# ebu/libear

Hardware: AMD Instinct MI355X
Metric: Msamples/s (higher is better)
Workload: dtype f32 io / f16x2-split MFMA, f32 accumulate

## Files before the change

### include/earhip.h

```cpp
#ifndef EARHIP_H
#define EARHIP_H

#include <stddef.h>
#include <stdint.h>

#ifdef __cplusplus
extern "C" {
#endif

#define EARHIP_VERSION 100

#define EARHIP_OK 0
#define EARHIP_INVALID_ARGUMENT 1
#define EARHIP_INTERNAL_ERROR 2
#define EARHIP_DEVICE_ERROR 3
#define EARHIP_NOT_IMPLEMENTED 4
#define EARHIP_UNKNOWN_LAYOUT 5
#define EARHIP_ADM_ERROR 6

int earhip_version(void);
const char *earhip_last_error(void);
int earhip_device_count(int *count);

typedef struct earhip_ctx earhip_ctx;
// ... 212 lines not shown

int earhip_conversion_to_polar(size_t n, const double *x, const double *y, const double *z,
                               const double *width, const double *height, const double *depth,
                               double *azimuth, double *elevation, double *distance,
                               double *width_out, double *height_out, double *depth_out);
int earhip_conversion_to_cartesian(size_t n, const double *azimuth, const double *elevation,
                                   const double *distance, const double *width,
                                   const double *height, const double *depth, double *x, double *y,
                                   double *z, double *width_out, double *height_out,
                                   double *depth_out);
int earhip_conversion_to_polar_device(earhip_ctx *ctx, size_t n, const double *x, const double *y,
                                      const double *z, const double *width, const double *height,
                                      const double *depth, double *azimuth, double *elevation,
                                      double *distance, double *width_out, double *height_out,
                                      double *depth_out, int *status);
int earhip_conversion_to_cartesian_device(earhip_ctx *ctx, size_t n, const double *azimuth,
                                          const double *elevation, const double *distance,
                                          const double *width, const double *height,
                                          const double *depth, double *x, double *y, double *z,
                                          double *width_out, double *height_out, double *depth_out,
                                          int *status);

typedef struct earhip_render earhip_render;

typedef struct earhip_render_config {
  int n_objects;
  int n_out;
  int block_size;
  int n_buses;
  const float *decorrelators;
  int n_taps;
  int delay;
  int max_blocks;
} earhip_render_config;

int earhip_render_create(earhip_ctx *ctx, const earhip_render_config *cfg,
                         earhip_render **out);
int earhip_render_destroy(earhip_render *r);
int earhip_render_set_object_points(earhip_render *r, int object, int npoints,
                                    const int64_t *times, const float *direct,
                                    const float *diffuse);
int earhip_render_commit(earhip_render *r);
int earhip_render_scratch_regrows(const earhip_render *r, long *count);
int earhip_render_reset(earhip_render *r, int64_t sample_time);
int earhip_render_process_device(earhip_render *r, size_t nblocks,
                                 const float *in_dev, size_t in_stride,
                                 float *out_dev, size_t out_stride);
int earhip_render_process(earhip_render *r, size_t nblocks, const float *const *in,
                          float *const *out);
typedef enum {
  EARHIP_PCM_S16 = 1,
  EARHIP_PCM_S24 = 2,
  EARHIP_PCM_S32 = 3,
  EARHIP_PCM_F32 = 4
} earhip_pcm_format;
int earhip_render_process_frames(earhip_render *r, size_t nblocks, const void *frames,
                                 earhip_pcm_format fmt, int frame_channels, int first_channel,
                                 float *const *out, int out_interleaved);
int earhip_render_process_frames_device(earhip_render *r, size_t nblocks, const void *frames_dev,
                                        earhip_pcm_format fmt, int frame_channels, int first_channel,
                                        float *out_dev, size_t out_stride, int out_interleaved);
typedef struct earhip_pcm_out {
  earhip_pcm_format format;
  int dither;
  uint32_t seed;
} earhip_pcm_out;
int earhip_render_process_frames_pcm(earhip_render *r, size_t nblocks, const void *frames,
                                     earhip_pcm_format fmt, int frame_channels, int first_channel,
                                     void *out_frames, const earhip_pcm_out *out);
int earhip_render_process_frames_pcm_device(earhip_render *r, size_t nblocks, const void *frames_dev,
                                            earhip_pcm_format fmt, int frame_channels,
                                            int first_channel, void *out_dev, size_t out_frame_bytes,
                                            size_t out_first_byte, const earhip_pcm_out *out);
int earhip_render_output_levels(earhip_render *r, float *peak, uint64_t *clipped, int reset);
int earhip_render_enable_timing(earhip_render *r, int enable);
int earhip_render_get_timing(earhip_render *r, double out[6]);
int earhip_render_gain_kernel(const earhip_render *r, int *kind);
int earhip_render_hinge_standby(earhip_render *r, int *standby);
int earhip_render_hinge_robust(earhip_render *r, int *robust);
int earhip_render_wide_form(earhip_render *r, int *wide);
int earhip_render_last_plan(const earhip_render *r, int out[4]);
int earhip_render_last_decor_plan(const earhip_render *r, int out[4]);
int earhip_render_last_list_layout(const earhip_render *r, int *paired);
int earhip_render_last_tail_blocks(const earhip_render *r, int *blocks);
int earhip_render_last_host_chunks(const earhip_render *r, int *chunks);
int earhip_render_scratch_bytes(const earhip_render *r, size_t *bytes);

typedef struct earhip_comm earhip_comm;
int earhip_comm_unique_id(void *id128);
int earhip_comm_create(earhip_ctx *ctx, int rank, int world, const void *id128, earhip_comm **out);
int earhip_comm_destroy(earhip_comm *comm);
int earhip_comm_channel_range(int n_out, int rank, int world, int *padded_rows, int *lo, int *hi);
int earhip_render_exchange_device(earhip_comm *comm, int slot, const float *partial_dev,
                                  float *owned_dev, size_t rows_per_rank, size_t row_stride);
int earhip_comm_gather_device(earhip_comm *comm, int slot, const float *owned_dev, float *full_dev,
                              size_t rows_per_rank, size_t row_stride, int root);
int earhip_comm_wait(earhip_comm *comm, int slot);
int earhip_comm_last_exchange_ms(earhip_comm *comm, int slot, double *ms);
int earhip_comm_info(earhip_comm *comm, int info[4]);
int earhip_comm_link_probe(earhip_comm *comm, size_t bytes, int shift, int reps, double *GBps);

typedef struct earhip_loudness earhip_loudness;
int earhip_loudness_create(earhip_ctx *ctx, int n_channels, int sample_rate, const double *coeffs,
                           size_t max_steps, earhip_loudness **out);
typedef struct earhip_true_peak {
  int phases;
  int taps;
  const double *coeffs;
} earhip_true_peak;
int earhip_loudness_create_tp(earhip_ctx *ctx, int n_channels, int sample_rate, const double *coeffs,
                              size_t max_steps, const earhip_true_peak *tp, earhip_loudness **out);
int earhip_loudness_destroy(earhip_loudness *m);
int earhip_loudness_reset(earhip_loudness *m);
int earhip_loudness_process_device(earhip_loudness *m, size_t nsamples, const float *rows_dev, size_t stride);
int earhip_loudness_process(earhip_loudness *m, size_t nsamples, const float *const *rows);
int earhip_loudness_num_steps(earhip_loudness *m, size_t *steps);
int earhip_loudness_steps(earhip_loudness *m, size_t first, size_t n, double *energy);
int earhip_loudness_result(earhip_loudness *m, const double *weights, double *integrated,
                           double *max_momentary, double *max_short_term);
int earhip_loudness_peaks(earhip_loudness *m, float *true_peak, float *sample_peak);
int earhip_loudness_step_peaks(earhip_loudness *m, size_t first, size_t n, float *true_peak, float *sample_peak);
int earhip_loudness_result_range(earhip_loudness *m, const double *weights, double *lra, double *low,
                                 double *high);
int earhip_loudness_gate(size_t n_steps, int n_channels, const double *energy ,
                         const double *weights, double *integrated, double *max_momentary,
                         double *max_short_term);
int earhip_loudness_layout_weights(const char *layout, double *weights);
int earhip_loudness_range(size_t n_steps, int n_channels, const double *energy ,
                          const double *weights, double *lra, double *low, double *high);
int earhip_render_attach_loudness(earhip_render *r, earhip_loudness *m);

typedef struct earhip_firmix earhip_firmix;
typedef struct earhip_firmix_config {
  int n_in;
  int n_out;
  int block_size;
  int n_taps;
  const float *taps;
  int max_blocks;
} earhip_firmix_config;
int earhip_firmix_create(earhip_ctx *ctx, const earhip_firmix_config *config, earhip_firmix **out);
int earhip_firmix_destroy(earhip_firmix *fm);
int earhip_firmix_reset(earhip_firmix *fm);
int earhip_firmix_info(const earhip_firmix *fm, int info[5]);
int earhip_firmix_process_device(earhip_firmix *fm, size_t nblocks, const float *in_dev, size_t in_stride,
                                 float *out_dev, size_t out_stride);
int earhip_firmix_process(earhip_firmix *fm, size_t nblocks, const float *const *in, float *const *out);
int earhip_firmix_create_sets(earhip_ctx *ctx, const earhip_firmix_config *config, int n_sets, earhip_firmix **out);
int earhip_firmix_load_set(earhip_firmix *fm, int set, const float *taps);
int earhip_firmix_load_set_device(earhip_firmix *fm, int set, const float *taps_dev);
int earhip_firmix_select(earhip_firmix *fm, int set, int fade_blocks);
int earhip_firmix_state(const earhip_firmix *fm, int state[4]);
int earhip_firmix_set_info(const earhip_firmix *fm, int set, int info[2]);
int earhip_render_attach_firmix(earhip_render *r, earhip_firmix *fm, float *sink_dev, size_t sink_stride,
                                size_t sink_capacity);
int earhip_render_firmix_position(earhip_render *r, size_t *samples);

typedef struct earhip_limiter earhip_limiter;
typedef struct earhip_limiter_config {
  int n_channels;
  int sample_rate;
  float ceiling;
  int lookahead;
  int hold;
  int detect;
  const earhip_true_peak *tp;
// ... 173 lines not shown
```

### libear_amd/capi.py

```python
import ctypes as C
import os

import numpy as np

from .build import lib_path

f32p = C.POINTER(C.c_float)
i64p = C.POINTER(C.c_int64)
pp_f32 = C.POINTER(f32p)

OK, INVALID_ARGUMENT, INTERNAL_ERROR, DEVICE_ERROR, NOT_IMPLEMENTED, UNKNOWN_LAYOUT, ADM_ERROR = 0, 1, 2, 3, 4, 5, 6


class EarHipError(Exception):
    def __init__(self, code, msg):
        super().__init__(msg)
        self.code = code


class InvalidArgument(EarHipError, ValueError):
    """maps to ear::invalid_argument"""


class InternalError(EarHipError, RuntimeError):
# ... 1096 lines not shown
        x = np.ascontiguousarray(x)
        _, dtype, cols = pcm_format(out_fmt)
        out = np.empty((x.shape[0], self.N * cols), dtype)
        return self.process_frames_pcm_into(x, out, fmt, first_channel, out_fmt, dither, seed)

    def process_frames_pcm_into(self, x, out, fmt, first_channel=0, out_fmt="s16", dither=False, seed=0):
        code, nblocks, channels = self._frames_shape(x, fmt)
        ocode, dtype, cols = pcm_format(out_fmt)
        assert out.dtype == dtype and out.flags["C_CONTIGUOUS"] and out.shape == (nblocks * self.B, self.N * cols), out.shape
        spec = PcmOut(ocode, int(dither), int(seed) & 0xFFFFFFFF)
        check(load().earhip_render_process_frames_pcm(self.h, C.c_size_t(nblocks), C.c_void_p(x.ctypes.data), C.c_int(code),
                                                      C.c_int(channels), C.c_int(first_channel), C.c_void_p(out.ctypes.data),
                                                      C.byref(spec)))
        return out

    def process_frames_pcm_device(self, nblocks, frames_ptr, fmt, frame_channels, first_channel, out_ptr, out_frame_bytes,
                                  out_first_byte=0, out_fmt="s16", dither=False, seed=0):
        code = pcm_format(fmt)[0] if isinstance(fmt, str) else int(fmt)
        ocode = pcm_format(out_fmt)[0] if isinstance(out_fmt, str) else int(out_fmt)
        spec = PcmOut(ocode, int(dither), int(seed) & 0xFFFFFFFF)
        check(load().earhip_render_process_frames_pcm_device(self.h, C.c_size_t(nblocks), C.c_void_p(frames_ptr), C.c_int(code),
                                                             C.c_int(frame_channels), C.c_int(first_channel), C.c_void_p(out_ptr),
                                                             C.c_size_t(out_frame_bytes), C.c_size_t(out_first_byte),
                                                             C.byref(spec)))

    def output_levels(self, reset=False):
        peak, clipped = np.zeros(self.N, np.float32), np.zeros(self.N, np.uint64)
        check(load().earhip_render_output_levels(self.h, _ptr(peak), C.c_void_p(clipped.ctypes.data), int(bool(reset))))
        return peak, clipped

    def enable_timing(self, on=True):
        check(load().earhip_render_enable_timing(self.h, int(on)))

    def get_timing(self):
        out = (C.c_double * 6)()
        check(load().earhip_render_get_timing(self.h, out))
        return {"gain_mix_ms": out[0], "gain_mix_launches": out[1], "decor_ms": out[2],
                "decor_launches": out[3], "prep_ms": out[4], "prep_launches": out[5]}

    def gain_kernel(self):
        kind = C.c_int(-1)
        check(load().earhip_render_gain_kernel(self.h, C.byref(kind)))
        return kind.value

    def hinge_standby(self):
        flag = C.c_int(0)
        check(load().earhip_render_hinge_standby(self.h, C.byref(flag)))
        return bool(flag.value)

    def hinge_robust(self):
        flag = C.c_int(0)
        check(load().earhip_render_hinge_robust(self.h, C.byref(flag)))
        return bool(flag.value)

    def wide_form(self):
        flag = C.c_int(1)
        check(load().earhip_render_wide_form(self.h, C.byref(flag)))
        return None if flag.value < 0 else bool(flag.value)

    def scratch_bytes(self):
        v = C.c_size_t(0)
        check(load().earhip_render_scratch_bytes(self.h, C.byref(v)))
        return v.value

    def scratch_regrows(self):
        v = C.c_long(0)
        check(load().earhip_render_scratch_regrows(self.h, C.byref(v)))
        return v.value

    def last_tail_blocks(self):
        v = C.c_int(0)
        check(load().earhip_render_last_tail_blocks(self.h, C.byref(v)))
        return v.value

    def last_host_chunks(self):
        v = C.c_int(0)
        check(load().earhip_render_last_host_chunks(self.h, C.byref(v)))
        return v.value

    def last_list_layout(self):
        v = C.c_int(0)
        check(load().earhip_render_last_list_layout(self.h, C.byref(v)))
        return None if v.value < 0 else bool(v.value)

    def last_plan(self):
        out = (C.c_int * 4)()
        check(load().earhip_render_last_plan(self.h, out))
        return {"kernel": out[0], "tile": out[1], "ntiles": out[2], "gsplit": out[3]}

    def last_decor_plan(self):
        out = (C.c_int * 4)()
        check(load().earhip_render_last_decor_plan(self.h, out))
        return {"Bk": out[0], "NP": out[1], "form": out[2], "run": out[3]}

    def attach_loudness(self, meter):
        check(load().earhip_render_attach_loudness(self.h, meter.h if meter is not None else None))
        self._meter = meter

    def attach_fir_matrix(self, fm, sink_ptr=None, sink_stride=0, sink_capacity=0):
        check(load().earhip_render_attach_firmix(self.h, fm.h if fm is not None else None,
                                                 C.c_void_p(sink_ptr) if sink_ptr else None, C.c_size_t(sink_stride),
                                                 C.c_size_t(sink_capacity)))
        self._fir_matrix = fm

    def fir_matrix_position(self):
        v = C.c_size_t(0)
        check(load().earhip_render_firmix_position(self.h, C.byref(v)))
        return v.value

    def attach_limiter(self, lim, sink_ptr=None, sink_stride=0, sink_capacity=0):
        check(load().earhip_render_attach_limiter(self.h, lim.h if lim is not None else None,
                                                  C.c_void_p(sink_ptr) if sink_ptr else None, C.c_size_t(sink_stride),
                                                  C.c_size_t(sink_capacity)))
        self._limiter = lim

    def limiter_position(self):
        v = C.c_size_t(0)
        check(load().earhip_render_limiter_position(self.h, C.byref(v)))
        return v.value

    def close(self):
        if self.h:
            load().earhip_render_destroy(self.h)
            self.h = C.c_void_p()



def _f64(a):
    return np.ascontiguousarray(a, dtype=np.float64)


def loudness_gate(energy, weights):
    w = _f64(weights).reshape(-1)
    e = _f64(energy).reshape(-1, w.size)
    out = [C.c_double(0) for _ in range(3)]
    check(load().earhip_loudness_gate(C.c_size_t(e.shape[0]), C.c_int(w.size), C.c_void_p(e.ctypes.data), C.c_void_p(w.ctypes.data),
                                      *[C.byref(v) for v in out]))
    return tuple(v.value for v in out)


def loudness_range(energy, weights):
    w = _f64(weights).reshape(-1)
    e = _f64(energy).reshape(-1, w.size)
    out = [C.c_double(0) for _ in range(3)]
    check(load().earhip_loudness_range(C.c_size_t(e.shape[0]), C.c_int(w.size), C.c_void_p(e.ctypes.data), C.c_void_p(w.ctypes.data),
                                       *[C.byref(v) for v in out]))
    return tuple(v.value for v in out)


class _TruePeak(C.Structure):
    _fields_ = [("phases", C.c_int), ("taps", C.c_int), ("coeffs", C.c_void_p)]


def loudness_layout_weights(layout):
    n = C.c_int(0)
    check(load().earhip_layout_num_channels(layout.encode(), C.byref(n)))
    w = np.zeros(n.value, np.float64)
    check(load().earhip_loudness_layout_weights(layout.encode(), C.c_void_p(w.ctypes.data)))
    return w


class _BusStage:
    _stem = None

    def reset(self):
        check(getattr(load(), f"earhip_{self._stem}_reset")(self.h))
# ... 442 lines not shown
```

### libear_amd/csrc/api_core.hip

```cpp
#include <cctype>
#include <cerrno>
#include <cmath>
#include <cstdlib>
#include <string>
#include <memory>
#include <mutex>
#include <type_traits>

#include "common.h"
#include "curves.h"
#include "gain_kernels.h"
#include "gain_mfma.h"
#include "gain_h2.h"
#include "gain_h2_t1.h"
#include "gain_p2.h"
#include "gain_hg.h"
#include "gain_f32g.h"

namespace earhip {

static_assert(kSplitTile == 256, "MixLaunch::tile() and tiles_aligned(256, ...) assume the 4-wave tile");

static thread_local std::string g_last_error;
void set_last_error(const std::string &msg) { g_last_error = msg; }

template <int V>
using Int = std::integral_constant<int, V>;
template <int... Vs, typename F>
static void dispatch(int v, F &&f) {
  if (!((v == Vs ? (f(Int<Vs>{}), true) : false) || ...)) fail_internal("no gain kernel instantiation for this launch plan");
}
template <int... Vs, typename F>
static void for_each(F &&f) {
  (f(Int<Vs>{}), ...);
}

template <typename F>
static void for_each_hinge_build(F &&f) {
  for_each<1, 2, 4, 8>([&](auto T) { f(T, Int<4>{}), f(T, Int<8>{}); });
}

struct CallWords {
  unsigned *level_cur = nullptr, *level_next = nullptr;
  unsigned *wide_cur = nullptr, *wide_next = nullptr;
  unsigned *gate = nullptr;
  unsigned *slow_cur = nullptr, *slow_next = nullptr;
  unsigned *obj_level = nullptr;
  bool grew = false;
};

static int grow_call_words(earhip_ctx *ctx, int M, size_t ntiles, size_t tile_cap) {
  int made = 0;
  if (M > 0 && !ctx->level.p) ctx->level.alloc_zero(4, ctx->stream), made++;
  const bool grow_obj = ctx->obj_level_cap < M, grow_tiles = ctx->tile_slow_cap < ntiles;
  if (grow_obj || grow_tiles) EARHIP_HIP(hipStreamSynchronize(ctx->stream));
  if (grow_obj) {
    ctx->obj_level_cap = M + M / 2 + 64;
    ctx->obj_level.alloc_zero(2 * (size_t)ctx->obj_level_cap, ctx->stream);
    made++;
  }
  if (grow_tiles) {
    ctx->tile_slow_cap = std::max<size_t>(tile_cap, 1024);
    ctx->tile_slow.alloc_zero(2 * ctx->tile_slow_cap, ctx->stream);
    ctx->tile_slow_idx = 0;
    made++;
  }
  return made;
}

void reserve_call_words(earhip_ctx *ctx, int M, size_t max_samples) {
  const size_t ntiles = (max_samples + 255) / 256;
  grow_call_words(ctx, M, ntiles, ntiles + ntiles / 4);
}

static CallWords acquire_call_words(earhip_ctx *ctx, const MixLaunch &ml, int M, const float *in_dev, size_t in_stride, int nsamples) {
  CallWords w;
  if (!ml.split_operands()) return w;
  const bool probe = ctx->x_scale_auto && in_stride % 4 == 0 && ((uintptr_t)in_dev & 15) == 0;
  const size_t slow_tiles = ml.kind == GainKernel::Grid ? (size_t)ml.ntiles : 0;
  if (!probe && !slow_tiles) return w;
  if ((probe && (!ctx->level.p || ctx->obj_level_cap < M)) || ctx->tile_slow_cap < slow_tiles) {
    ctx->lazy_allocs += grow_call_words(ctx, probe ? M : 0, slow_tiles, 2 * slow_tiles);
    w.grew = true;
  }
  if (slow_tiles) {
    w.slow_cur = ctx->tile_slow.p + (size_t)ctx->tile_slow_idx * ctx->tile_slow_cap;
    w.slow_next = ctx->tile_slow.p + (size_t)(ctx->tile_slow_idx ^ 1) * ctx->tile_slow_cap;
    ctx->tile_slow_idx ^= 1;
  }
  if (!probe) return w;
  w.level_cur = ctx->level.p + ctx->level_idx;
  w.level_next = ctx->level.p + (ctx->level_idx ^ 1);
  if ((size_t)ml.ntiles * ml.gsplit >= 2 * (size_t)ctx->num_cus) w.wide_cur = ctx->level.p + 2 + ctx->level_idx;
  w.wide_next = ctx->level.p + 2 + (ctx->level_idx ^ 1);
  w.gate = ctx->level.p + 2 + ctx->level_idx;
  ctx->level_idx ^= 1;
  w.obj_level = ctx->obj_level.p;
  const int v = ctx->get(OPT_PROBE_RUNS);
  const int probe_runs = v >= 1 && v <= 64 && (v & (v - 1)) == 0 ? v : 16;
  hipLaunchKernelGGL(k_level_probe, dim3((M + kProbeObjects - 1) / kProbeObjects), dim3(64 * kProbeObjects), 0, ctx->stream, in_dev,
                     in_stride, nsamples, M, w.level_cur, ctx->obj_level.p, ctx->obj_level_cap, probe_runs);
  return w;
}

struct MixCall {
  earhip_ctx *ctx;
  const CurveSet &cs;
  const MixLaunch &ml;
  const ColumnPlan &cp;
  PointStore ps;
  int M, nsamples;
  int64_t t_call;
  const float *in_dev;
  size_t in_stride;
  SegDesc *scratch;
  ScratchLayout lay;
  SlotLists sl;
  PieceLists pl;
  HingeLists hl;
  CallWords w;
  bool hg_robust = false, standby = false;
  GainMixParams P;
  hipStream_t stream() const { return ctx->stream; }
  int64_t t_end() const { return t_call + nsamples; }
  unsigned *gate_word(bool robust) const { return hg_robust == robust ? w.gate : nullptr; }
  unsigned *standby_gate() const { return ml.kind == GainKernel::Hinge ? w.gate : nullptr; }
  int piece_tile() const { return 64 * ml.pw; }
  int piece_tiles() const { return lay.piece_tiles; }
  float x_scale() const { return std::ldexp(1.0f, ctx->x_scale_log2); }
  dim3 tile_grid(int x) const { return dim3(x, ml.gsplit, cp.mnz * cp.mgroups); }
};


static void prep_hinge_lists(const MixCall &c) {
  earhip_ctx *ctx = c.ctx;
  const MixLaunch &ml = c.ml;
  const int M = c.M, nw = ml.tile() / 64;
  if (M > kMaxHingeCached || (nw != 4 && nw != 8)) fail_internal("hinge lists: object count or tile out of range");
  if (!c.ps.kink_row0) fail_internal("hinge kernel: the curve set has no kink rows");
  if (!hinge_addressable(M, c.in_stride, c.nsamples, (size_t)c.ps.kink_row0 + c.ps.rows, c.ps.row)) fail_internal("hinge kernel: buffers beyond its 32-bit offsets");
  if (c.w.gate)
    hipLaunchKernelGGL(k_hinge_gate, dim3((M + 255) / 256), dim3(256), 0, c.stream(), c.w.obj_level, ctx->obj_level_cap, M, c.w.level_cur, c.w.gate,
                       c.w.wide_cur != nullptr, c.hg_robust);
  int tpw = 1;
  const size_t cached_max = std::min((size_t)kMaxHingeCached, ctx->hinge_build_lds / sizeof(HingeCached));
  if ((size_t)M > cached_max) fail_internal("hinge lists: more objects than the builder's LDS holds on this device");
  while (tpw < 8 && ml.ntiles / (2 * tpw) >= ctx->num_cus && (size_t)M * (2 * tpw) <= cached_max) tpw *= 2;
  if (ctx->has(OPT_HBUILD_TPW)) {
    const int v = ctx->get(OPT_HBUILD_TPW);
    if ((v == 1 || v == 2 || v == 4 || v == 8) && (size_t)M * v <= cached_max) tpw = v;
  }
  HingeCached *stage = nullptr;
  if (ctx->get(OPT_BUILD_2K, 0) != 0) {
    stage = c.lay.hinge_staging(c.scratch);
    const dim3 cgrid((ml.ntiles + 63) / 64, (M + kClassifyObjects - 1) / kClassifyObjects);
    dispatch<4, 8>(nw, [&](auto NW) {
      hipLaunchKernelGGL((k_hinge_classify<decltype(NW)::value>), cgrid, dim3(64 * kClassifyObjects), 0, c.stream(), c.ps, M, ml.ntiles, c.t_call,
                         c.t_end(), stage, c.w.obj_level, c.w.level_cur, c.gate_word(false), c.gate_word(true));
    });
    if (!ctx->has(OPT_HBUILD_TPW)) {
      tpw = 1;
      while (tpw < 8 && ml.ntiles / (2 * tpw) >= 2 * ctx->num_cus) tpw *= 2;
    }
  }
  const dim3 bgrid((ml.ntiles + tpw - 1) / tpw);
  const size_t lds = stage ? 0 : sizeof(HingeCached) * (size_t)M * tpw;
  for_each_hinge_build([&](auto T, auto NW) {
    if (tpw == T && nw == NW)
      hipLaunchKernelGGL((k_hinge_build<decltype(T)::value, decltype(NW)::value>), bgrid, dim3(kHingeBuildThreads), lds, c.stream(), c.ps, M, ml.ntiles,
                         c.t_call, c.t_end(), c.hl, c.w.obj_level, c.w.level_cur, c.gate_word(false), c.gate_word(true), (const HingeCached *)stage);
  });
}

static void prep_piece_lists(const MixCall &c) {
  earhip_ctx *ctx = c.ctx;
  const MixLaunch &ml = c.ml;
  const int M = c.M, ptile = c.piece_tile(), pnt = c.piece_tiles();
  if (M > kMaxPieceObjects || ptile > kPieceMaxTile) fail_internal("piece lists: object index or tile out of range");
  int tpw = 1;
  while (tpw < 8 && pnt / (2 * tpw) >= ctx->num_cus) tpw *= 2;
  if (ctx->has(OPT_BUILD_TPW)) {
    const int v = ctx->get(OPT_BUILD_TPW);
    if (v == 1 || v == 2 || v == 4 || v == 8) tpw = v;
  }
  const PieceLists &pl = c.pl;
  PairRec *stage = nullptr;
  if (ctx->has(OPT_BUILD_2K) ? ctx->get(OPT_BUILD_2K) != 0 : ml.paired) {
    stage = c.lay.piece_staging(c.scratch);
    hipLaunchKernelGGL(k_piece_classify, dim3((pnt + 63) / 64, (M + kClassifyObjects - 1) / kClassifyObjects), dim3(64 * kClassifyObjects), 0,
                       c.stream(), c.ps, M, pnt, ptile, c.t_call, c.t_end(), pl.paired, stage, c.w.obj_level, c.w.level_cur, c.standby_gate());
  }
  dispatch<1, 2, 4, 8>(tpw, [&](auto T) {
    hipLaunchKernelGGL(k_piece_build<decltype(T)::value>, dim3((pnt + tpw - 1) / tpw), dim3(kBuildThreads), 0, c.stream(), c.ps, M, pnt, ptile, c.t_call,
                       c.t_end(), pl, c.w.obj_level, c.w.level_cur, c.standby_gate(), ctx->obj_level_cap, c.w.wide_cur, stage);
  });
}

static void prep_descriptors(const MixCall &c) {
  const MixLaunch &ml = c.ml;
  const unsigned objs = (unsigned)(c.M + 15) / 16;
  QuietMark qm;
  if (c.w.obj_level) {
// ... 54 lines not shown
  const int per_cu = ml.tile() == 512 ? 1 : (cp.nct == 1 ? 3 : 2);
  int wgs = std::max(8, (ctx->num_cus * per_cu / std::max(1, ml.gsplit * cp.mnz * cp.mgroups)) & ~7);
  if (ctx->has(OPT_H2_WGS)) wgs = std::max(1, ctx->get(OPT_H2_WGS));
  wgs = std::max(wgs, ((ml.ntiles + 63) / 64 + 7) & ~7);
  if (!h2_persistent(cp.nct, ml.tile() == 512 ? 8 : 4)) wgs = ml.ntiles;
  GainMixParams P = c.P;
  P.tile_runs = ctx->has(OPT_H2_RUNS) ? (ctx->get(OPT_H2_RUNS) != 0) : 0;
  const dim3 grid = c.tile_grid(std::min(ml.ntiles, wgs));
  const float xs = c.x_scale();
  const float *gs = c.cs.column_scales();
  const bool two_launches = ctx->get(OPT_H2_PAIR, 0) != 0;
  auto h2 = [&](auto NCT, auto NW, auto WIDE) {
    hipLaunchKernelGGL((k_gain_mix_h2<decltype(NCT)::value, decltype(NW)::value, decltype(WIDE)::value>), grid, dim3(64 * decltype(NW)::value), 0,
                       c.stream(), P, c.ps.zero_row, xs, gs, w.level_cur, w.level_next, w.slow_cur, w.slow_next, w.wide_cur, w.wide_next);
  };
  auto h2_t1 = [&](auto NCT, auto WIDE) {
    hipLaunchKernelGGL((k_gain_mix_h2_t1<decltype(NCT)::value, 4, decltype(WIDE)::value>), grid, dim3(256), 0, c.stream(), P, c.ps.zero_row, xs, gs,
                       w.level_cur, w.level_next, w.slow_cur, w.slow_next, w.wide_cur, w.wide_next);
  };
  dispatch<1, 2, 3>(cp.nct, [&](auto NCT) {
    if (ml.tile() == 512) {
      if (w.wide_cur && !two_launches) return h2(NCT, Int<8>{}, Int<2>{});
      if (w.wide_cur) h2(NCT, Int<8>{}, Int<0>{});
      h2(NCT, Int<8>{}, Int<1>{});
    } else if (NCT == 1) {
      if (w.wide_cur) h2(Int<1>{}, Int<4>{}, Int<0>{});
      h2(Int<1>{}, Int<4>{}, Int<1>{});
    } else {
      if (w.wide_cur) h2_t1(NCT, std::false_type{});
      h2_t1(NCT, std::true_type{});
    }
  });
}

static void launch_pieces(const MixCall &c) {
  earhip_ctx *ctx = c.ctx;
  const ColumnPlan &cp = c.cp;
  const MixLaunch &ml = c.ml;
  const CallWords &w = c.w;
  const int pnt = c.piece_tiles();
  int wgs = std::max(8, (ctx->num_cus * (ml.pw == 4 ? 2 : 1) / std::max(1, ml.gsplit * cp.mnz * cp.mgroups)) & ~7);
  if (ctx->has(OPT_P2_WGS)) wgs = ctx->get(OPT_P2_WGS) > 0 ? ctx->get(OPT_P2_WGS) : pnt;
  if (!p2_persistent(cp.nct, ml.pw, ml.paired)) wgs = pnt;
  const dim3 grid = c.tile_grid(std::min(pnt, wgs));
  const float xs = c.x_scale();
  const float *gs = c.cs.column_scales();
  dispatch<0, 1>(ml.paired ? 1 : 0, [&](auto PAIRED) {
    dispatch<1, 2, 3>(cp.nct, [&](auto NCT) {
      dispatch<4, 8>(ml.pw == 4 ? 4 : 8, [&](auto NW) {
        constexpr int nw = decltype(NW)::value;
        hipLaunchKernelGGL((k_gain_mix_p2<decltype(NCT)::value, nw, decltype(PAIRED)::value != 0>), grid, dim3(64 * nw), 0, c.stream(), c.P, c.pl, xs, gs,
                           w.level_cur, w.level_next, w.wide_cur, w.wide_next, c.standby_gate(), pnt);
      });
    });
  });
}

static void launch_hinge(const MixCall &c) {
  const CallWords &w = c.w;
  const float xs = c.x_scale();
  const float *gs = c.cs.column_scales();
  dispatch<1, 2, 3>(c.cp.nct, [&](auto NCT) {
    dispatch<4, 8>(c.ml.tile() == 256 ? 4 : 8, [&](auto NW) {
      constexpr int nw = decltype(NW)::value;
      hipLaunchKernelGGL((k_gain_mix_hg<decltype(NCT)::value, nw>), c.tile_grid(c.ml.ntiles), dim3(64 * nw), 0, c.stream(), c.P, c.hl, xs, gs, w.level_cur,
                         w.level_next, w.wide_cur, w.wide_next, c.gate_word(false), c.gate_word(true));
    });
  });
}

static GainMixParams mix_params(const MixCall &c, float *out_dev, size_t out_stride, size_t part_stride, unsigned *record) {
  const float *in_dev = c.in_dev;
  const size_t in_stride = c.in_stride;
  const bool valu = c.ml.kind == GainKernel::Valu;
  GainMixParams P;
  P.mode_word = c.w.gate;
  P.record = c.w.gate ? record : nullptr;
  P.sl = c.sl;
  P.in = in_dev;
  P.in_stride = in_stride;
  P.out = out_dev;
  P.out_stride = out_stride;
  P.part_stride = part_stride;
  P.desc = c.scratch;
  P.ps = c.ps;
  P.t_call = c.t_call;
  P.nsamples = c.nsamples;
  P.ntiles = c.ml.ntiles;
  P.M = c.M;
  P.ncols = c.cs.ncols();
  P.ngroups = valu ? c.cp.ngroups : c.cp.mgroups;
  P.wsplit = c.ml.wsplit;
  P.tiles_per_wg = valu ? 1 : c.ml.tpw;
  P.vec_ok = in_stride % 4 == 0 && out_stride % 4 == 0 && part_stride % 4 == 0 && ((uintptr_t)in_dev & 15) == 0 && ((uintptr_t)out_dev & 15) == 0;
  return P;
}

MixResult launch_gain_mix(earhip_ctx *ctx, const CurveSet &cs, const MixLaunch &ml, bool strict, int64_t t_call, int nsamples,
                          const float *in_dev, size_t in_stride, float *out_dev, size_t out_stride, size_t part_stride, SegDesc *desc,
                          unsigned *record, hipEvent_t *ev) {
  const GainKernel kind = ml.kind;
  MixCall c{ctx, cs, ml, cs.plan(), cs.device(), cs.M(), nsamples, t_call, in_dev, in_stride, desc, scratch_layout(cs, ml, cs.M(), nsamples)};
  if (kind == GainKernel::Slots) c.sl = c.lay.slot_lists(desc);
  if (kind == GainKernel::Pieces || kind == GainKernel::Hinge) c.pl = c.lay.piece_lists(desc, ml.paired);
  if (kind == GainKernel::Hinge) c.hl = c.lay.hinge_lists(desc);
  if (kind == GainKernel::Slots && c.M > kMaxSlotObjects) fail_internal("slot lists address objects with 16 bits");
  if (ev) EARHIP_HIP(hipEventRecord(ev[0], ctx->stream));
  c.w = acquire_call_words(ctx, ml, c.M, in_dev, in_stride, nsamples);
  c.hg_robust = kind == GainKernel::Hinge && ctx->get(OPT_HG_ROBUST, 1) != 0;
  c.standby = kind == GainKernel::Hinge && c.w.gate && !c.hg_robust;
  switch (kind) {
    case GainKernel::Hinge:
      prep_hinge_lists(c);
      if (c.standby) prep_piece_lists(c);
      break;
    case GainKernel::Pieces: prep_piece_lists(c); break;
    case GainKernel::Slots: {
      const bool own_search = (size_t)c.ps.npoints <= (size_t)8 * c.M;
      if (!own_search) prep_descriptors(c);
      prep_slot_lists(c, own_search);
      break;
    }
    default: prep_descriptors(c); break;
  }
  if (ev) EARHIP_HIP(hipEventRecord(ev[1], ctx->stream));
  c.P = mix_params(c, out_dev, out_stride, part_stride, record);
  if (ev) EARHIP_HIP(hipEventRecord(ev[2], ctx->stream));
  switch (kind) {
    case GainKernel::Valu: launch_valu(c, strict); break;
    case GainKernel::Slots: launch_slots(c); break;
    case GainKernel::F32Grid: launch_f32grid(c); break;
    case GainKernel::Grid: launch_grid(c); break;
    case GainKernel::Pieces: launch_pieces(c); break;
    case GainKernel::Hinge:
      launch_hinge(c);
      if (c.standby) launch_pieces(c);
      break;
  }
  if (ev) EARHIP_HIP(hipEventRecord(ev[3], ctx->stream));
  EARHIP_HIP(hipGetLastError());
  MixResult res;
  res.gated = kind == GainKernel::Hinge && c.w.gate;
  res.device_form = c.w.wide_cur != nullptr;
  res.hinge_robust = res.gated && c.hg_robust;
  res.grew = c.w.grew;
  return res;
}

size_t hinge_build_allow_lds(const hipDeviceProp_t &prop) {
  const size_t want = 128 * 1024, dflt = 64 * 1024;
  const size_t device_max = std::max((size_t)prop.sharedMemPerBlock, (size_t)prop.maxSharedMemoryPerMultiProcessor);
  size_t ask = std::min(want, device_max > 4096 ? device_max - 4096 : dflt);
  if (ask <= dflt) return dflt;
  bool ok = true;
  for_each_hinge_build([&](auto T, auto NW) {
    ok = ok && hipFuncSetAttribute(reinterpret_cast<const void *>(&k_hinge_build<decltype(T)::value, decltype(NW)::value>),
                                   hipFuncAttributeMaxDynamicSharedMemorySize, (int)ask) == hipSuccess;
  });
  if (!ok) (void)hipGetLastError();
  return ok ? ask : dflt;
}

struct GainStage {
  earhip_ctx *ctx;
  int n_in, n_out;
  CurveSet curves;
  DevBuf<SegDesc> desc;
  DevBuf<float> parts;
  std::vector<float> rows;
  bool force_ramp;
  GainStage(earhip_ctx *c, int ni, int no, bool ramp = false)
      : ctx(c), n_in(ni), n_out(no), curves(ni, no, 1, ramp), force_ramp(ramp) {}

  void run_device(int64_t t_call, int nsamples, const float *in_dev, size_t in_stride,
                  float *out_dev, size_t out_stride) {
    curves.commit(ctx);
    const bool strict = ctx->strict || n_in == 1 || force_ramp;
    const MixLaunch ml = plan_mix(ctx, curves.plan(), n_in, nsamples, strict, 32, curves.stats(t_call, in_stride, (size_t)nsamples, false));
    if (ml.kind == GainKernel::Hinge) curves.ensure_kinks(ctx);
    desc.reserve(scratch_units(curves, ml, n_in));
    const size_t row_stride = ((size_t)nsamples + 3) & ~(size_t)3;
    if (ml.gsplit > 1) parts.reserve(row_stride * n_out * ml.gsplit);
    launch_gain_mix_summed(ctx, curves, ml, strict, t_call, nsamples, in_dev, in_stride, out_dev, out_stride, parts.p, row_stride, desc.p,
                           nullptr, nullptr);
  }

  void run_host(int64_t t_call, const float *const *in, float *const *out, int64_t r0,
                int64_t r1) {
    const int n = (int)(r1 - r0);
    if (n <= 0) return;
    const size_t stride = ((size_t)n + 3) & ~(size_t)3;
    ctx->pin_in.reserve(stride * n_in);
    ctx->pin_out.reserve(stride * n_out);
    ctx->dev_in.reserve(stride * n_in);
    ctx->dev_out.reserve(stride * n_out);
    for (int c = 0; c < n_in; c++)
      std::memcpy(ctx->pin_in.p + c * stride, in[c] + r0, sizeof(float) * n);
    EARHIP_HIP(hipMemcpyAsync(ctx->dev_in.p, ctx->pin_in.p, sizeof(float) * stride * n_in,
                              hipMemcpyHostToDevice, ctx->stream));
    run_device(t_call, n, ctx->dev_in.p, stride, ctx->dev_out.p, stride);
    EARHIP_HIP(hipMemcpyAsync(ctx->pin_out.p, ctx->dev_out.p, sizeof(float) * stride * n_out,
                              hipMemcpyDeviceToHost, ctx->stream));
    EARHIP_HIP(hipStreamSynchronize(ctx->stream));
    for (int c = 0; c < n_out; c++)
      std::memcpy(out[c] + r0, ctx->pin_out.p + c * stride, sizeof(float) * n);
  }
};

}

using namespace earhip;

static const char *const kOptNames[OPT_COUNT] = {
    "SPL", "MFMA", "XSCALE", "WAVES", "TPW", "NRT", "H2_TILE", "H2_WGS", "H2_RUNS", "P2_TILE", "P2_PAIRS", "P2_WGS", "HINGE", "HG_TILE", "HBUILD_TPW",
    "BUILD_TPW", "K2_WG", "K2_OWN_BLOCK", "RUN", "GSPLIT", "PROBE_RUNS", "BLOCK_GROUPS", "DEBUG_TIMING", "TAILCUT", "HOST_CHUNK_MB", "HOST_THREADS", "HG_ROBUST", "BUILD_2K", "HOST_BIND", "HOST_NT", "HOST_FIRST", "H2_PAIR"};

static int parse_option_value(const std::string &key, const char *text) {
  char *end = nullptr;
  errno = 0;
  const long v = std::strtol(text, &end, 10);
  while (end && *end && std::isspace((unsigned char)*end)) end++;
  if (end == text || (end && *end) || errno == ERANGE || v < -(1L << 30) || v > (1L << 30))
    fail_invalid("option '" + key + "': '" + std::string(text) + "' is not an integer");
  return (int)v;
}

void earhip_ctx::apply_options() {
  spl = 4, use_mfma = 3, x_scale_log2 = 14, x_scale_auto = true, max_waves = 4, tiles_per_wg = 4, tiles_per_wg_forced = false, nrt = 8;
  if (has(OPT_SPL) && (get(OPT_SPL) == 2 || get(OPT_SPL) == 4)) spl = get(OPT_SPL);
  if (has(OPT_MFMA)) use_mfma = get(OPT_MFMA);
  if (has(OPT_XSCALE) && get(OPT_XSCALE) >= -64 && get(OPT_XSCALE) <= 64)
    x_scale_log2 = get(OPT_XSCALE), x_scale_auto = false;
  if (has(OPT_WAVES) && get(OPT_WAVES) >= 1 && get(OPT_WAVES) <= 8) max_waves = get(OPT_WAVES);
  if (has(OPT_TPW) && get(OPT_TPW) >= 1 && get(OPT_TPW) <= 8) tiles_per_wg = get(OPT_TPW), tiles_per_wg_forced = true;
  if (has(OPT_NRT) && (get(OPT_NRT) == 4 || get(OPT_NRT) == 8)) nrt = get(OPT_NRT);
}

struct earhip_gain_interp {
  std::unique_ptr<GainStage> stage;
};

struct PolicyCache {
  std::vector<std::unique_ptr<GainStage>> stages;
  GainStage *get(earhip_ctx *ctx, int n_in, int n_out, bool ramp) {
    for (auto &s : stages)
      if (s->n_in == n_in && s->n_out == n_out && s->force_ramp == ramp) return s.get();
    stages.emplace_back(new GainStage(ctx, n_in, n_out, ramp));
    return stages.back().get();
  }
};
static std::vector<std::pair<earhip_ctx *, std::unique_ptr<PolicyCache>>> g_policy;
static std::mutex g_policy_mutex;
static PolicyCache *policy_cache(earhip_ctx *ctx) {
  std::lock_guard<std::mutex> lock(g_policy_mutex);
  for (auto &p : g_policy)
    if (p.first == ctx) return p.second.get();
  g_policy.emplace_back(ctx, std::unique_ptr<PolicyCache>(new PolicyCache));
  return g_policy.back().second.get();
}

static __global__ void k_clock_probe(unsigned long long *out) {
  out[0] = clock64();
  out[1] = wall_clock64();
}

static __global__ void __launch_bounds__(256) k_read_linear(const f32x4 *in, float *out, size_t n4) {
  f32x4 acc = {0.0f, 0.0f, 0.0f, 0.0f};
  size_t i = (size_t)blockIdx.x * 256 + threadIdx.x;
  const size_t step = (size_t)gridDim.x * 256;
  for (; i + 3 * step < n4; i += 4 * step) {
    const f32x4 a = __builtin_nontemporal_load(in + i), b = __builtin_nontemporal_load(in + i + step);
    const f32x4 c = __builtin_nontemporal_load(in + i + 2 * step), d = __builtin_nontemporal_load(in + i + 3 * step);
    acc += (a + b) + (c + d);
  }
  for (; i < n4; i += step) acc += __builtin_nontemporal_load(in + i);
  if (acc[0] + acc[1] + acc[2] + acc[3] == 123.456f) out[0] = 1.0f;
}
static __global__ void __launch_bounds__(256) k_read_rows(const float *in, float *out, int rows, size_t stride) {
  constexpr int DEPTH = 4;
  const int lane = threadIdx.x & 63, w = threadIdx.x >> 6, li = lane & 15, kg = lane >> 4;
  const float *base = in + (size_t)blockIdx.x * 256 + w * 64 + li * 4;
  auto row = [&](int r) { return base + (size_t)min(r, rows - 1) * stride; };
  f32x4 acc = {0.0f, 0.0f, 0.0f, 0.0f};
  f32x4 ring[DEPTH][8];
#pragma unroll
  for (int d = 0; d < DEPTH; d++)
#pragma unroll
    for (int q = 0; q < 8; q++)
      ring[d][q] = __builtin_nontemporal_load((const f32x4 *)row(d * 32 + kg * 8 + q));
  for (int r0 = 0; r0 < rows; r0 += 32 * DEPTH) {
#pragma unroll
    for (int d = 0; d < DEPTH; d++) {
#pragma unroll
      for (int q = 0; q < 8; q++) acc += ring[d][q];
      const int rn = r0 + 32 * DEPTH + d * 32;
      if (rn < rows)
#pragma unroll
        for (int q = 0; q < 8; q++)
          ring[d][q] = __builtin_nontemporal_load((const f32x4 *)row(rn + kg * 8 + q));
    }
  }
  if (acc[0] + acc[1] + acc[2] + acc[3] == 123.456f) out[0] = 1.0f;
}

extern "C" {

int earhip_debug_read_bandwidth(earhip_ctx *ctx, const float *in_dev, size_t rows, size_t stride,
                                size_t nsamples, int reps, double ms[2]) {
  return guarded([&] {
    require(ctx != nullptr && in_dev != nullptr && ms != nullptr, "NULL argument");
    require(rows >= 1 && rows < ((size_t)1 << 24) && reps >= 1 && reps <= 1000, "rows / reps out of range");
    require(stride % 256 == 0 && nsamples % 256 == 0 && nsamples >= 256 && nsamples <= stride &&
                ((uintptr_t)in_dev & 15) == 0,
            "buffer must be 16-byte aligned with stride and nsamples multiples of 256");
    ctx->use();
    if (!ctx->level.p) ctx->level.alloc_zero(4, ctx->stream);
    float *sink = reinterpret_cast<float *>(ctx->level.p);
    hipEvent_t e[4];
    for (auto &x : e) EARHIP_HIP(hipEventCreate(&x));
    const size_t n4 = rows * stride / 4;
    const unsigned lin_blocks = (unsigned)std::min<size_t>((n4 + 255) / 256, (size_t)ctx->num_cus * 32);
    auto linear = [&] {
      hipLaunchKernelGGL(k_read_linear, dim3(lin_blocks), dim3(256), 0, ctx->stream,
                         reinterpret_cast<const f32x4 *>(in_dev), sink, n4);
    };
    auto pattern = [&] {
      hipLaunchKernelGGL(k_read_rows, dim3((unsigned)(nsamples / 256)), dim3(256), 0, ctx->stream, in_dev, sink,
                         (int)rows, stride);
    };
    linear();
    EARHIP_HIP(hipEventRecord(e[0], ctx->stream));
    for (int i = 0; i < reps; i++) linear();
    EARHIP_HIP(hipEventRecord(e[1], ctx->stream));
    pattern();
    EARHIP_HIP(hipEventRecord(e[2], ctx->stream));
    for (int i = 0; i < reps; i++) pattern();
    EARHIP_HIP(hipEventRecord(e[3], ctx->stream));
    EARHIP_HIP(hipGetLastError());
    EARHIP_HIP(hipEventSynchronize(e[3]));
    float t = 0.0f;
    EARHIP_HIP(hipEventElapsedTime(&t, e[0], e[1]));
    ms[0] = (double)t / reps;
    EARHIP_HIP(hipEventElapsedTime(&t, e[2], e[3]));
    ms[1] = (double)t / reps;
    for (auto &x : e) (void)hipEventDestroy(x);
  });
}

int earhip_debug_copy_bandwidth(earhip_ctx *ctx, void *host, size_t bytes, int reps, double ms[2]) {
  return guarded([&] {
    require(ctx != nullptr && host != nullptr && ms != nullptr, "NULL argument");
    require(bytes >= 4 && reps >= 1 && reps <= 1000, "bytes / reps out of range");
    ctx->use();
    DevBuf<char> dev;
    dev.alloc(bytes);
    hipEvent_t e[2];
    for (auto &x : e) EARHIP_HIP(hipEventCreate(&x));
    for (int dir = 0; dir < 2; dir++) {
      auto copy = [&] {
        if (dir == 0) EARHIP_HIP(hipMemcpyAsync(dev.p, host, bytes, hipMemcpyHostToDevice, ctx->stream));
        else EARHIP_HIP(hipMemcpyAsync(host, dev.p, bytes, hipMemcpyDeviceToHost, ctx->stream));
      };
      copy();
      EARHIP_HIP(hipEventRecord(e[0], ctx->stream));
      for (int i = 0; i < reps; i++) copy();
      EARHIP_HIP(hipEventRecord(e[1], ctx->stream));
      EARHIP_HIP(hipEventSynchronize(e[1]));
      float t = 0.0f;
      EARHIP_HIP(hipEventElapsedTime(&t, e[0], e[1]));
      ms[dir] = (double)t / reps;
    }
    for (auto &x : e) (void)hipEventDestroy(x);
    EARHIP_HIP(hipStreamSynchronize(ctx->stream));
  });
}

int earhip_debug_hg_prof(earhip_ctx *ctx, unsigned long long *out128) {
  return guarded([&] {
    require(ctx != nullptr && out128 != nullptr, "NULL argument");
#ifdef EARHIP_HG_PROF
    ctx->use();
    EARHIP_HIP(hipStreamSynchronize(ctx->stream));
    EARHIP_HIP(hipMemcpyFromSymbol(out128, HIP_SYMBOL(g_hg_prof), sizeof(unsigned long long) * 128));
#else
    fail_invalid("this build has no hinge-kernel phase sums (-DEARHIP_HG_PROF)");
#endif
  });
}

int earhip_debug_build_prof(earhip_ctx *ctx, unsigned long long *out64) {
  return guarded([&] {
    require(ctx != nullptr && out64 != nullptr, "NULL argument");
#ifdef EARHIP_BUILD_PROF
    ctx->use();
    EARHIP_HIP(hipStreamSynchronize(ctx->stream));
    EARHIP_HIP(hipMemcpyFromSymbol(out64, HIP_SYMBOL(g_build_prof), sizeof(unsigned long long) * 64));
#else
    fail_invalid("this build has no list-builder phase stamps (-DEARHIP_BUILD_PROF)");
#endif
// ... 305 lines not shown
```

### libear_amd/csrc/api_render.hip

```cpp
#include <cmath>
#include <cstdlib>
#include <chrono>
#include <memory>
#include <vector>

#include "bus_stage.h"
#include "curves.h"
#include "decor_stage.h"
#include "host_pipeline.h"
#include "pcm_frames.h"

using namespace earhip;

struct CallReport {
  int kind = -1;
  int plan[3] = {0, 0, 0};
  int paired = -1;
  size_t scratch_bytes = 0;
  bool gated = false;
  bool device_form = false;
  bool hg_robust = false;
  int tail_blocks = 0;
};

struct earhip_render {
  earhip_ctx *ctx = nullptr;
  int M = 0, N = 0, B = 0, K = 1, T = 0;
  std::unique_ptr<CurveSet> curves;
  int64_t t = 0;
  CallReport report;
  long scratch_regrows = 0;
  DevBuf<unsigned> rec;

  DevBuf<SegDesc> desc;
  DevBuf<float> bus;
  int max_gsplit = 1;
  DecorStage decor;
  DevBuf<float> d_in, d_out;
  PinBuf<float> p_in, p_out;
  std::unique_ptr<GatherPool> gather;
  StreamPipe pipe;
  int last_host_chunks = 0;
  PinBuf<unsigned char> p_bytes;
  DevBuf<unsigned char> d_bytes;
  DevBuf<float> d_ilv, d_rows, d_rows_out;
  DevBuf<unsigned char> d_pcm;
  PinBuf<unsigned char> p_pcm;
  PcmLevels levels;
  bool timing = false;
  bool last_timed = false;
  int timing_every = 1;
  long timing_calls = 0;
  hipEvent_t ev[6] = {nullptr, nullptr, nullptr, nullptr, nullptr, nullptr};
  struct Pending { hipEvent_t e[6]; bool has_k2; bool continues; };
  std::vector<Pending> pending;
  std::vector<hipEvent_t> pool;
  double acc_ms[3] = {0, 0, 0};
  double acc_n[3] = {0, 0, 0};

  ~earhip_render() {
    for (auto &p : pending)
      for (auto e : p.e)
        if (e) (void)hipEventDestroy(e);
    for (auto e : pool) (void)hipEventDestroy(e);
  }

  unsigned mode_word() {
    ctx->use();
    unsigned word = 0;
    EARHIP_HIP(hipMemcpyAsync(&word, rec.p, sizeof(word), hipMemcpyDeviceToHost, ctx->stream));
    EARHIP_HIP(hipStreamSynchronize(ctx->stream));
    if (!(word & kModeRecorded)) fail_internal("no gain kernel recorded the call's mode word");
    return word;
  }

  hipEvent_t get_event() {
    if (!pool.empty()) {
      hipEvent_t e = pool.back();
      pool.pop_back();
      return e;
    }
    hipEvent_t e;
    EARHIP_HIP(hipEventCreate(&e));
    return e;
  }

  void drain_timing() {
    EARHIP_HIP(hipStreamSynchronize(ctx->stream));
    for (auto &p : pending) {
      float ms = 0;
      const double one = p.continues ? 0.0 : 1.0;
      EARHIP_HIP(hipEventElapsedTime(&ms, p.e[0], p.e[1]));
      acc_ms[2] += ms; acc_n[2] += one;
      EARHIP_HIP(hipEventElapsedTime(&ms, p.e[2], p.e[3]));
      acc_ms[0] += ms; acc_n[0] += one;
      if (p.has_k2) {
        EARHIP_HIP(hipEventElapsedTime(&ms, p.e[4], p.e[5]));
        acc_ms[1] += ms; acc_n[1] += one;
      }
      for (auto e : p.e)
        if (e) pool.push_back(e);
    }
    pending.clear();
  }

  size_t direct_stride(const float *const *ch, int count, size_t n) const {
    if (ctx->host_ranges.empty() || count < 1) return 0;
    const uintptr_t a0 = (uintptr_t)ch[0];
    const uintptr_t step = count > 1 ? (uintptr_t)ch[1] - a0 : sizeof(float) * n;
    if ((a0 & 15) != 0 || step % 16 != 0 || step < sizeof(float) * n || step > ((uintptr_t)1 << 40)) return 0;
    for (int c = 1; c < count; c++)
      if ((uintptr_t)ch[c] - (uintptr_t)ch[c - 1] != step) return 0;
    return ctx->host_reachable(ch[0], step * (count - 1) + sizeof(float) * n) ? (size_t)(step / sizeof(float)) : 0;
  }

  size_t frames_to_device_rows(size_t nblocks, const void *frames_dev, int fmt, int frame_channels, int first_channel, bool with_out) {
    ctx->use();
    const size_t S = (size_t)pcm_sample_bytes(fmt), n = nblocks * (size_t)B, cap = (size_t)T * B;
    if (d_rows.n < cap * M || (with_out && d_rows_out.n < cap * N)) {
      EARHIP_HIP(hipStreamSynchronize(ctx->stream));
      d_rows.reserve(cap * M);
      if (with_out) d_rows_out.reserve(cap * N);
    }
    launch_pcm_to_rows(fmt, frames_dev, (size_t)frame_channels * S, (size_t)first_channel * S, M, n, d_rows.p, n, ctx->stream);
    return n;
  }
  void reserve_pcm_out(size_t bytes, bool pinned) {
    levels.reserve(N, ctx->stream);
    d_pcm.reserve(bytes);
    if (pinned) p_pcm.reserve(bytes);
  }

  HostChunkPlan host_plan(size_t nblocks, bool direct) const {
    return plan_host_chunks(nblocks, B, M, direct, ctx->has(OPT_HOST_CHUNK_MB), ctx->get(OPT_HOST_CHUNK_MB), ctx->get(OPT_HOST_FIRST, 0));
  }
  hipError_t chunk_rows_d2h(float *out0, size_t out_st, size_t at, size_t len) {
    const float *dout = d_out.p + (size_t)N * at;
    if (out_st)
      return hipMemcpy2DAsync(out0 + at, sizeof(float) * out_st, dout, sizeof(float) * len, sizeof(float) * len, N, hipMemcpyDeviceToHost, pipe.out);
    return hipMemcpyAsync(p_out.p + (size_t)N * at, dout, sizeof(float) * len * N, hipMemcpyDeviceToHost, pipe.out);
  }
  void chunk_rows_scatter(float *const *out, size_t at, size_t len) const {
    for (int ch = 0; ch < N; ch++) std::memcpy(out[ch] + at, p_out.p + (size_t)N * at + (size_t)ch * len, sizeof(float) * len);
  }
  void process_short_call(size_t nblocks, float *out0, size_t out_st) {
    const size_t n = nblocks * (size_t)B;
    const bool direct_out = decor.NP <= 1;
    process_device(nblocks, d_in.p, n, out_st ? out0 : direct_out ? p_out.p : d_out.p, out_st ? out_st : n);
    if (!out_st && !direct_out) EARHIP_HIP(hipMemcpyAsync(p_out.p, d_out.p, sizeof(float) * n * N, hipMemcpyDeviceToHost, ctx->stream));
  }
  GatherPool &staging_threads() {
    if (!gather) {
      gather.reset(new GatherPool);
      const int want = ctx->get(OPT_HOST_THREADS, 0);
      gather->start(want >= 1 && want <= 64 ? want : default_staging_threads());
    }
    return *gather;
  }

  MixLaunch plan_call(size_t nblocks, size_t in_stride) {
    const int nsamples = (int)(nblocks * (size_t)B);
    MixLaunch ml = plan_mix(ctx, curves->plan(), M, nsamples, ctx->strict, max_gsplit, curves->stats(t, in_stride, (size_t)nsamples, true));
    const size_t bus_stride = ((size_t)nsamples + 3) & ~(size_t)3;
    while (ml.gsplit > 1 && bus_stride * K * N * ml.gsplit > bus.n) ml.gsplit /= 2;
    return ml;
  }

  size_t last_in_stride = 0;
  void reserve_for_curves() {
    size_t need = 0;
    bool hinge = false;
    const size_t lens[3] = {(size_t)T, (size_t)std::max(1, T / 2), (size_t)1};
    for (size_t nb : lens) {
      const MixLaunch ml = plan_call(nb, last_in_stride ? last_in_stride : nb * (size_t)B);
      need = std::max(need, scratch_units(*curves, ml, M));
      hinge = hinge || ml.kind == GainKernel::Hinge;
    }
    if (hinge) curves->ensure_kinks(ctx);
    if (need > desc.n) {
      EARHIP_HIP(hipStreamSynchronize(ctx->stream));
      desc.reserve(need + need / 4);
    }
  }

  int resident_workgroups(const MixLaunch &ml) const {
    if (!ml.split_operands()) return 0;
    return ctx->num_cus * (ml.tile() >= 512 ? 1 : 2);
  }

  struct BusTap {
    BusStage *stage = nullptr;
    float *sink = nullptr;
    size_t stride = 0, cap = 0, pos = 0;
  };
  enum { TAP_METER, TAP_MATRIX, TAP_LIMITER, TAP_COUNT };
  BusTap taps[TAP_COUNT];
  bool tapped() const {
    for (const BusTap &t : taps)
      if (t.stage) return true;
    return false;
  }
  void attach(int which, BusStage *stage, const char *rows_words, bool writes, float *sink_dev, size_t sink_stride,
              size_t sink_capacity) {
    if (stage) {
      const std::string the = std::string("the ") + stage->noun;
      if (stage->ctx != ctx) fail_invalid(the + " must belong to the renderer's context");
      require(stage->n_in == N, rows_words);
      if (stage->block != 1 && stage->block != B) fail_invalid(the + " must have the renderer's block size");
      if (writes) {
        require(sink_dev != nullptr, "sink_dev must not be NULL");
        require(sink_stride >= sink_capacity, "sink_stride must be >= sink_capacity");
      }
    }
    taps[which] = stage && writes ? BusTap{stage, sink_dev, sink_stride, sink_capacity, 0} : BusTap{stage};
  }
  void check_taps(size_t nblocks) const {
    const size_t n = nblocks * (size_t)B;
    for (const BusTap &t : taps) {
      if (!t.stage) continue;
      t.stage->check_room(n / (size_t)t.stage->block);
      if (t.sink && t.pos + n > t.cap)
        fail_invalid(std::string("the call would pass the ") + t.stage->noun + "'s sink_capacity (nothing was rendered)");
    }
  }
  void feed_taps(size_t nblocks, const float *out_dev, size_t out_stride) {
    const size_t n = nblocks * (size_t)B;
    for (BusTap &t : taps) {
      if (!t.stage) continue;
      t.stage->feed(n / (size_t)t.stage->block, out_dev, out_stride, t.sink ? t.sink + t.pos : nullptr, t.stride);
      if (t.sink) t.pos += n;
    }
  }
  void process_device(size_t nblocks, const float *in_dev, size_t in_stride, float *out_dev, size_t out_stride) {
    if (!tapped()) return render_spans(nblocks, in_dev, in_stride, out_dev, out_stride);
    check_taps(nblocks);
    render_spans(nblocks, in_dev, in_stride, out_dev, out_stride);
    feed_taps(nblocks, out_dev, out_stride);
  }
  void render_spans(size_t nblocks, const float *in_dev, size_t in_stride, float *out_dev, size_t out_stride) {
    MixLaunch whole;
    bool have_plan = false;
    if (!ctx->strict && ctx->get(OPT_TAILCUT, 1) != 0 && nblocks >= 2) {
      last_in_stride = in_stride;
      if (curves->dirty()) {
        curves->commit(ctx);
        reserve_for_curves();
      }
      const MixLaunch ml = whole = plan_call(nblocks, in_stride);
      have_plan = true;
      const int W = resident_workgroups(ml);
      if (W > 0 && ml.gsplit == 1 && ml.ntiles > W) {
        const size_t tile = (size_t)ml.tile();
        const size_t full = (size_t)ml.ntiles / (size_t)W, rest = (size_t)ml.ntiles % (size_t)W;
        const size_t main_samples = full * (size_t)W * tile;
        const size_t eighths = (size_t)std::min(std::max(ctx->get(OPT_TAILCUT, 2), 0), 7);
        if (rest > 0 && rest <= (size_t)W * eighths / 8 && main_samples % (size_t)B == 0) {
          const size_t main_blocks = main_samples / (size_t)B;
          process_span(main_blocks, in_dev, in_stride, out_dev, out_stride, false);
          const CallReport main = report;
          process_span(nblocks - main_blocks, in_dev + main_samples, in_stride, out_dev + main_samples, out_stride, true);
          report = main;
          report.tail_blocks = (int)(nblocks - main_blocks);
          return;
        }
      }
    }
    report.tail_blocks = 0;
    process_span(nblocks, in_dev, in_stride, out_dev, out_stride, false, have_plan ? &whole : nullptr);
  }

  void process_span(size_t nblocks, const float *in_dev, size_t in_stride, float *out_dev,
                    size_t out_stride, bool continues, const MixLaunch *planned = nullptr) {
    const int nsamples = (int)(nblocks * (size_t)B);
    last_in_stride = in_stride;
    if (curves->dirty()) {
      curves->commit(ctx);
      reserve_for_curves();
    }
    const bool strict = ctx->strict;
    MixLaunch ml = planned ? *planned : plan_call(nblocks, in_stride);
    if (ml.kind == GainKernel::Hinge) curves->ensure_kinks(ctx);

    report.kind = (int)ml.kind;
    {
      const size_t need = scratch_units(*curves, ml, M);
      if (need > desc.n) {
        EARHIP_HIP(hipStreamSynchronize(ctx->stream));
        desc.reserve(need + need / 2);
        scratch_regrows++;
      }
      report.scratch_bytes = need * 16;
    }
    const size_t bus_stride = ((size_t)nsamples + 3) & ~(size_t)3;
    const size_t part_stride = bus_stride * K * N;
    if (part_stride * ml.gsplit > bus.n) fail_internal("bus buffer too small for this launch plan");
    report.paired = (ml.kind == GainKernel::Pieces || ml.kind == GainKernel::Hinge) ? (ml.paired ? 1 : 0) : -1;
    report.plan[0] = ml.tile();
    report.plan[1] = ml.ntiles;
    report.plan[2] = ml.gsplit;
    Pending pd;
    hipEvent_t *evp = nullptr;
    const bool timed = timing && (continues ? last_timed : (timing_calls++ % timing_every) == 0);
    last_timed = timed;
    if (timed) {
      for (int i = 0; i < 6; i++) pd.e[i] = get_event();
      pd.has_k2 = K == 2;
      pd.continues = continues;
      evp = pd.e;
    }
    unsigned *const record = rec.p + (continues ? 1 : 0);
    MixResult mix;
    if (K == 1) {
      mix = launch_gain_mix_summed(ctx, *curves, ml, strict, t, nsamples, in_dev, in_stride, out_dev, out_stride, bus.p, bus_stride, desc.p,
                                   record, evp);
    } else {
      mix = launch_gain_mix(ctx, *curves, ml, strict, t, nsamples, in_dev, in_stride, bus.p, bus_stride, part_stride, desc.p, record, evp);
      decor.run(ctx, nblocks, nsamples, bus.p, bus_stride, part_stride, ml.gsplit, out_dev, out_stride, evp);
    }
    if (timed) pending.push_back(pd);
    report.gated = mix.gated, report.device_form = mix.device_form, report.hg_robust = mix.hinge_robust;
    if (mix.grew) scratch_regrows++;
    t += nsamples;
  }
};

extern "C" {

int earhip_render_create(earhip_ctx *ctx, const earhip_render_config *cfg, earhip_render **out) {
  return guarded([&] {
    require(ctx != nullptr && cfg != nullptr && out != nullptr, "NULL argument");
    require(cfg->n_objects >= 1 && cfg->n_out >= 1, "n_objects and n_out must be >= 1");
    require(cfg->n_buses == 1 || cfg->n_buses == 2, "n_buses must be 1 or 2");
    FftShape shape;
    require(cfg->block_size >= 16 && cfg->block_size <= 4096 && fft_make_shape(2 * cfg->block_size, &shape),
            "block_size must be in [16, 4096]");
    require(cfg->max_blocks >= 1, "max_blocks must be >= 1");
    require((int64_t)cfg->max_blocks * cfg->block_size < ((int64_t)1 << 30),
            "max_blocks * block_size too large");
    require(cfg->delay >= 0, "delay must be >= 0");
    if (cfg->n_buses == 2) {
      require(cfg->decorrelators != nullptr && cfg->n_taps >= 1,
              "n_buses == 2 needs decorrelator filters");
      require((cfg->n_taps + cfg->block_size - 1) / cfg->block_size <= 64,
              "decorrelator filters of more than 64 blocks are not supported by the fused render "
              "(use BlockConvolver)");
    } else {
      require(cfg->delay == 0, "delay needs n_buses == 2");
    }
    ctx->use();
    std::unique_ptr<earhip_render> r(new earhip_render);
    r->ctx = ctx;
    r->M = cfg->n_objects;
    r->N = cfg->n_out;
    r->B = cfg->block_size;
    r->K = cfg->n_buses;
    r->T = cfg->max_blocks;
    r->curves.reset(new CurveSet(r->M, r->K * r->N, r->K, false));
    const size_t max_samples = (size_t)r->T * r->B;
    reserve_call_words(ctx, r->M, max_samples);
    r->rec.alloc_zero(2, ctx->stream);
    const size_t min_tile = (size_t)std::min(16 * ctx->nrt, std::min(64 * ctx->spl, 256));
    const size_t max_tiles = (max_samples + min_tile - 1) / min_tile;
    r->desc.alloc((size_t)r->M * ((max_samples + 255) / 256) + 1);
    (void)max_tiles;
    r->max_gsplit = 16;
    if (ctx->has(OPT_GSPLIT)) {
      const int v = ctx->get(OPT_GSPLIT);
      if (v >= 1 && v <= 32) r->max_gsplit = v;
    }
    r->bus.alloc_zero((size_t)r->K * r->N * bus_samples_bound(ctx, max_samples, r->max_gsplit), ctx->stream);
    if (r->K == 2) r->decor.create(ctx, *cfg, r->B);
    EARHIP_HIP(hipStreamSynchronize(ctx->stream));
    *out = r.release();
  });
}

int earhip_render_destroy(earhip_render *r) {
  return guarded([&] {
    if (!r) return;
    (void)hipSetDevice(r->ctx->device);
    (void)hipStreamSynchronize(r->ctx->stream);
    delete r;
  });
}

int earhip_render_set_object_points(earhip_render *r, int object, int npoints,
                                    const int64_t *times, const float *direct,
                                    const float *diffuse) {
  return guarded([&] {
    require(r != nullptr, "render must not be NULL");
    require(npoints >= 1, "interp_points must not be empty");
    require(times != nullptr && direct != nullptr, "times/direct must not be NULL");
    require(r->K == 1 || diffuse != nullptr, "diffuse gains must not be NULL when n_buses == 2");
    const int N = r->N, cols = r->K * N;
    std::vector<float> rows((size_t)npoints * cols);
    for (int k = 0; k < npoints; k++) {
      std::memcpy(&rows[(size_t)k * cols], direct + (size_t)k * N, sizeof(float) * N);
      if (r->K == 2)
        std::memcpy(&rows[(size_t)k * cols + N], diffuse + (size_t)k * N, sizeof(float) * N);
    }
    r->curves->set_object(object, npoints, times, rows.data());
  });
}
// ... 326 lines not shown
    r->ctx->use();
    if (r->timing) r->drain_timing();
    r->timing = enable != 0;
    r->timing_every = enable > 1 ? enable : 1;
    r->timing_calls = 0;
    for (int i = 0; i < 3; i++) r->acc_ms[i] = r->acc_n[i] = 0;
  });
}

int earhip_render_get_timing(earhip_render *r, double out[6]) {
  return guarded([&] {
    require(r != nullptr && out != nullptr, "NULL argument");
    r->ctx->use();
    r->drain_timing();
    out[0] = r->acc_ms[0]; out[1] = r->acc_n[0];
    out[2] = r->acc_ms[1]; out[3] = r->acc_n[1];
    out[4] = r->acc_ms[2]; out[5] = r->acc_n[2];
  });
}

int earhip_render_gain_kernel(const earhip_render *r, int *kind) {
  return guarded([&] {
    require(r != nullptr && kind != nullptr, "NULL argument");
    *kind = r->report.kind;
  });
}

int earhip_render_hinge_standby(earhip_render *r, int *standby) {
  return guarded([&] {
    require(r != nullptr && standby != nullptr, "NULL argument");
    *standby = 0;
    if (r->report.kind != 5 || !r->report.gated || r->report.hg_robust) return;
    *standby = (r->mode_word() & kGateHingeUnsafe) ? 1 : 0;
  });
}

int earhip_render_hinge_robust(earhip_render *r, int *robust) {
  return guarded([&] {
    require(r != nullptr && robust != nullptr, "NULL argument");
    *robust = 0;
    if (r->report.kind != 5 || !r->report.hg_robust) return;
    *robust = hinge_span_exceeded(r->mode_word(), r->M) ? 1 : 0;
  });
}

int earhip_render_wide_form(earhip_render *r, int *wide) {
  return guarded([&] {
    require(r != nullptr && wide != nullptr, "NULL argument");
    *wide = 1;
    if (r->report.kind < 3) *wide = -1;
    if (r->report.kind < 3 || !r->report.device_form) return;
    *wide = (r->mode_word() & 1u) ? 1 : 0;
  });
}

int earhip_render_scratch_bytes(const earhip_render *r, size_t *bytes) {
  return guarded([&] {
    require(r != nullptr && bytes != nullptr, "NULL argument");
    *bytes = r->report.scratch_bytes;
  });
}

int earhip_render_scratch_regrows(const earhip_render *r, long *count) {
  return guarded([&] {
    require(r != nullptr && count != nullptr, "NULL argument");
    *count = r->scratch_regrows;
  });
}

int earhip_render_last_tail_blocks(const earhip_render *r, int *blocks) {
  return guarded([&] {
    require(r != nullptr && blocks != nullptr, "NULL argument");
    *blocks = r->report.tail_blocks;
  });
}

int earhip_render_last_host_chunks(const earhip_render *r, int *chunks) {
  return guarded([&] {
    require(r != nullptr && chunks != nullptr, "NULL argument");
    *chunks = r->last_host_chunks;
  });
}

int earhip_render_last_list_layout(const earhip_render *r, int *paired) {
  return guarded([&] {
    require(r != nullptr && paired != nullptr, "NULL argument");
    *paired = r->report.paired;
  });
}

int earhip_render_last_plan(const earhip_render *r, int out[4]) {
  return guarded([&] {
    require(r != nullptr && out != nullptr, "NULL argument");
    out[0] = r->report.kind;
    for (int i = 0; i < 3; i++) out[1 + i] = r->report.plan[i];
  });
}

int earhip_render_last_decor_plan(const earhip_render *r, int out[4]) {
  return guarded([&] {
    require(r != nullptr && out != nullptr, "NULL argument");
    for (int i = 0; i < 4; i++) out[i] = 0;
    if (r->K != 2) return;
    out[0] = r->decor.Bk;
    out[1] = r->decor.NP;
    out[2] = r->decor.last_form;
    out[3] = r->decor.last_R;
  });
}

}
```

### libear_amd/csrc/common.h

```cpp
#pragma once

#include <hip/hip_runtime.h>

#include <cstdint>
#include <cstdio>
#include <string>
#include <vector>

#include "../../include/earhip.h"

namespace earhip {

struct Error {
  int code;
  std::string msg;
};

void set_last_error(const std::string &msg);

template <typename F>
int guarded(F &&f) {
  try {
    f();
    return EARHIP_OK;
// ... 15 lines not shown
[[noreturn]] inline void fail_internal(const std::string &m) {
  throw Error{EARHIP_INTERNAL_ERROR, "internal error: " + m};
}
inline void require(bool ok, const char *m) {
  if (!ok) fail_invalid(m);
}

#define EARHIP_HIP(expr)                                                        \
  do {                                                                          \
    hipError_t e_ = (expr);                                                     \
    if (e_ != hipSuccess)                                                       \
      throw ::earhip::Error{EARHIP_DEVICE_ERROR,                                \
                            std::string("internal error: HIP: ") +              \
                                hipGetErrorString(e_) + " in " #expr};          \
  } while (0)

inline bool is_pow2(size_t v) { return v && !(v & (v - 1)); }

template <typename T>
struct DevBuf {
  T *p = nullptr;
  size_t n = 0;
  DevBuf() = default;
  DevBuf(const DevBuf &) = delete;
  DevBuf &operator=(const DevBuf &) = delete;
  ~DevBuf() { release(); }
  void release() {
    if (p) (void)hipFree(p);
    p = nullptr;
    n = 0;
  }
  void alloc(size_t count) {
    release();
    if (count == 0) count = 1;
    EARHIP_HIP(hipMalloc((void **)&p, count * sizeof(T)));
    n = count;
  }
  void alloc_zero(size_t count, hipStream_t s) {
    alloc(count);
    EARHIP_HIP(hipMemsetAsync(p, 0, n * sizeof(T), s));
  }
  void reserve(size_t count) {
    if (count > n) alloc(count);
  }
  void upload(const std::vector<T> &v) {
    alloc(v.size());
    if (!v.empty()) EARHIP_HIP(hipMemcpy(p, v.data(), sizeof(T) * v.size(), hipMemcpyHostToDevice));
  }
};

template <typename T>
struct PinBuf {
  T *p = nullptr;
  size_t n = 0;
  PinBuf() = default;
  PinBuf(const PinBuf &) = delete;
  PinBuf &operator=(const PinBuf &) = delete;
  ~PinBuf() {
    if (p) (void)hipHostFree(p);
  }
  void reserve(size_t count) {
    if (count <= n) return;
    if (p) (void)hipHostFree(p);
    p = nullptr;
    n = 0;
    EARHIP_HIP(hipHostMalloc((void **)&p, count * sizeof(T), hipHostMallocDefault));
    n = count;
  }
};

}

struct earhip_vbs;
namespace earhip {
void vbs_orphan(earhip_vbs *v);
}

namespace earhip {
enum Opt {
  OPT_SPL, OPT_MFMA, OPT_XSCALE, OPT_WAVES, OPT_TPW, OPT_NRT,
  OPT_H2_TILE, OPT_H2_WGS, OPT_H2_RUNS, OPT_P2_TILE, OPT_P2_PAIRS, OPT_P2_WGS, OPT_HINGE, OPT_HG_TILE, OPT_HBUILD_TPW, OPT_BUILD_TPW,
  OPT_K2_WG, OPT_K2_OWN_BLOCK, OPT_RUN, OPT_GSPLIT,
  OPT_PROBE_RUNS, OPT_BLOCK_GROUPS, OPT_DEBUG_TIMING, OPT_TAILCUT, OPT_HOST_CHUNK_MB, OPT_HOST_THREADS, OPT_HG_ROBUST, OPT_BUILD_2K,
  OPT_HOST_BIND, OPT_HOST_NT, OPT_HOST_FIRST, OPT_H2_PAIR, OPT_COUNT
};
struct OptVal {
  bool set = false;
  int v = 0;
};
}

struct earhip_ctx {
  earhip::OptVal opt[earhip::OPT_COUNT];
  bool has(earhip::Opt o) const { return opt[o].set; }
  int get(earhip::Opt o, int dflt = 0) const { return opt[o].set ? opt[o].v : dflt; }
  void apply_options();
  int device = 0;
  hipStream_t stream = nullptr;
  bool own_stream = false;
  bool strict = false;
  int spl = 4;
  int use_mfma = 3;
  int x_scale_log2 = 14;
  bool x_scale_auto = true;
  earhip::DevBuf<unsigned> level;
  int level_idx = 0;
  earhip::DevBuf<unsigned> tile_slow;
  size_t tile_slow_cap = 0;
  int tile_slow_idx = 0;
  earhip::DevBuf<unsigned> obj_level;
  int obj_level_cap = 0;
  long lazy_allocs = 0;
  int max_waves = 4;
  int tiles_per_wg = 4;
  bool tiles_per_wg_forced = false;
  int nrt = 8;
  int num_cus = 256;
  size_t hinge_build_lds = 64 * 1024;
  struct HostRange {
    const char *base;
    size_t bytes;
    bool owned;
  };
  std::vector<HostRange> host_ranges;
  std::vector<earhip_vbs *> pinned_adapters;
  bool host_reachable(const void *p, size_t bytes) const {
    const char *c = static_cast<const char *>(p);
    for (const auto &r : host_ranges)
      if (c >= r.base && c + bytes <= r.base + r.bytes) return true;
    return false;
  }
  earhip::PinBuf<float> pin_in, pin_out;
  earhip::DevBuf<float> dev_in, dev_out, dev_pts;
  void use() const { EARHIP_HIP(hipSetDevice(device)); }
};

namespace earhip {
int panner_create(earhip_ctx *ctx, const char *layout, int n_channels, const double *azimuth, const double *elevation,
                  earhip_panner **out, bool with_extent);
struct PanParams;
const PanParams &panner_params(const earhip_panner *p);
std::vector<double> panner_pan_points(earhip_panner *p, size_t npos, const double *xyz, unsigned *missed);
std::vector<double> tdesign_directions(size_t extra_rows = 0);
}
```

### libear_amd/csrc/curves.h

```cpp
#pragma once

#include <chrono>
#include <cmath>
#include <cstdio>
#include <cstdlib>

#include <algorithm>
#include <cstring>
#include <vector>

#include "common.h"
#include "gain_kernels.h"
#include "gain_p2.h"
#include "gain_hg.h"
#include "gain_f32g.h"

namespace earhip {

struct ColumnPlan {
  int nout = 24;
  int ngroups = 1;
  int nz = 1;
  int nct = 1;
  int mgroups = 1;
  int mnz = 1;
  int row = 24;
  static ColumnPlan make(int ncols) {
    ColumnPlan p;
    int groups = (ncols + 23) / 24;
    const int per = (ncols + groups - 1) / groups;
    p.nout = per <= 8 ? 8 : per <= 16 ? 16 : 24;
    groups = (ncols + p.nout - 1) / p.nout;
    p.ngroups = std::min(groups, 8);
    p.nz = (groups + p.ngroups - 1) / p.ngroups;
    int mg = (ncols + 47) / 48;
    p.nct = mg > 1 ? 3 : (ncols + 15) / 16;
    p.mgroups = std::min(mg, 8);
    p.mnz = (mg + p.mgroups - 1) / p.mgroups;
    p.row = std::max(p.nz * p.ngroups * p.nout, p.mnz * p.mgroups * p.nct * 16);
    return p;
  }
};

struct CurveImage {
  ObjHdr *hdr;
  int32_t *off, *cnt;
  int64_t *time;
  uint8_t *flat;
  PointRec *rec;
  float *gain;
};
static __global__ void __launch_bounds__(256)
k_curve_upload(CurveImage src, CurveImage dst, const int32_t *changed, int row) {
  const int m = changed[blockIdx.x];
  const int off = src.off[m], n = src.cnt[m];
  if (threadIdx.x == 0) dst.off[m] = off, dst.cnt[m] = n, dst.hdr[m] = src.hdr[m];
  for (int i = threadIdx.x; i < n; i += 256) {
    dst.time[off + i] = src.time[off + i];
    dst.flat[off + i] = src.flat[off + i];
    dst.rec[off + i] = src.rec[off + i];
  }
  const size_t g0 = (size_t)off * row, gn = (size_t)n * row;
  const float4 *sg = reinterpret_cast<const float4 *>(src.gain + g0);
  float4 *dg = reinterpret_cast<float4 *>(dst.gain + g0);
  for (size_t i = threadIdx.x; i < gn / 4; i += 256) dg[i] = sg[i];
}

struct CurveStats {
  int aligned_tile = 0;
  double ramp_share = 1.0;
  float gain_scale = 0.0f;
  double point_density = 0.0;
  double pair_waste256 = 1.0;
  double pair_waste512 = 1.0;
  double hinge_exact_share = 2.0;
  bool grid512_strict = false;
  double deltas256 = 0.0;
};

class CurveSet {
 public:
  CurveSet(int M, int ncols, int nbus = 1, bool force_ramp = false)
      : M_(M), ncols_(ncols), nbus_(nbus), force_ramp_(force_ramp), plan_(ColumnPlan::make(ncols)), obj_(M) {
    for (int m = 0; m < M; m++) {
      obj_[m].t.assign(1, 0);
      obj_[m].g.assign(plan_.row, 0.0f);
      obj_[m].flat.assign(1, 0);
      obj_[m].dirty = true;
      dirty_list_.push_back(m);
    }
    cmax_.assign(plan_.row, 0.0f);
    obj_cmax_.assign((size_t)M * plan_.row, 0.0f);
    cm_scratch_.assign(plan_.row, 0.0f);
    shrunk_cols_.assign(plan_.row, 0);
    dirty_list_.reserve(M);
    for (auto &p : phases_) p.items.reserve(M);
  }
  ~CurveSet() {
    if (staged_) (void)hipEventDestroy(staged_);
  }
  int M() const { return M_; }
  int ncols() const { return ncols_; }
  const ColumnPlan &plan() const { return plan_; }

  void set_object(int m, int npoints, const int64_t *times, const float *rows,
                  const uint8_t *flat_override = nullptr) {
    if (m < 0 || m >= M_) fail_invalid("object index out of range");
    if (npoints < 1) fail_invalid("interp_points must not be empty");
    if (npoints > kMaxPointsPerObject) fail_invalid("too many interpolation points for one object");
    for (int k = 1; k < npoints; k++) {
      if (times[k] < times[k - 1]) fail_invalid("interpolation points are not sorted");
      if (times[k] - times[k - 1] > (int64_t)0x7fffffff)
        fail_invalid("interpolation ramp longer than 2^31-1 samples is not supported");
    }
    Obj &o = obj_[m];
    const size_t row = (size_t)plan_.row;
    o.t.assign(times, times + npoints);
    o.g.assign((size_t)npoints * row, 0.0f);
    for (int k = 0; k < npoints; k++)
      std::memcpy(&o.g[(size_t)k * row], rows + (size_t)k * ncols_, sizeof(float) * ncols_);
    o.flat.assign(npoints, 0);
    const int bc = ncols_ / nbus_;
    for (int k = 1; k < npoints; k++) {
      if (flat_override) {
        o.flat[k] = flat_override[k];
        continue;
      }
      for (int b = 0; b < nbus_; b++) {
        bool same = true;
        for (int c = b * bc; same && c < (b + 1) * bc; c++)
          same = rows[(size_t)(k - 1) * ncols_ + c] == rows[(size_t)k * ncols_ + c];
        if (same) o.flat[k] |= (uint8_t)(1 << b);
      }
    }
    {
      int w = 1;
      for (int k = 1; k < npoints; k++) {
        const bool repeat = o.t[k] == o.t[w - 1] && std::memcmp(&o.g[(size_t)k * row], &o.g[(size_t)(w - 1) * row], sizeof(float) * row) == 0;
        if (repeat) continue;
        if (w != k) {
          o.t[w] = o.t[k];
          o.flat[w] = o.flat[k];
          std::memmove(&o.g[(size_t)w * row], &o.g[(size_t)k * row], sizeof(float) * row);
        }
        w++;
      }
      o.t.resize(w);
      o.flat.resize(w);
      o.g.resize((size_t)w * row);
    }
    if (!o.dirty) o.dirty = true, dirty_list_.push_back(m);
  }

  void commit(earhip_ctx *ctx) {
    if (dirty_list_.empty()) return;
#ifdef EARHIP_COMMIT_TIMING
    static double acc[6] = {0, 0, 0, 0, 0, 0};
    static long ncalls = 0;
    auto now = [] { return std::chrono::duration<double, std::micro>(std::chrono::steady_clock::now().time_since_epoch()).count(); };
    double tq = now();
    auto lap = [&](int i) { const double t = now(); acc[i] += t - tq; tq = t; };
    struct Print { ~Print() { if (ncalls) fprintf(stderr, "commit timing (us/call over %ld): sync %.2f regions %.2f mirror+stats %.2f finish %.2f upload %.2f tail %.2f\n", ncalls, acc[0]/ncalls, acc[1]/ncalls, acc[2]/ncalls, acc[3]/ncalls, acc[4]/ncalls, acc[5]/ncalls); } };
    static Print printer;
    ncalls++;
#define EARHIP_LAP(i) lap(i)
#else
#define EARHIP_LAP(i)
#endif
    const size_t row = (size_t)plan_.row;
    if (staged_) EARHIP_HIP(hipEventSynchronize(staged_));
    EARHIP_LAP(0);
    bool full_upload = !uploaded_once_;
    for (int m : dirty_list_) {
      Obj &o = obj_[m];
      const int n = (int)o.t.size();
      if (n > o.cap) {
        abandoned_ += (size_t)o.cap;
        o.cap = std::max(16, n + n / 2);
// ... 41 lines not shown
      arena_cap_ = cap;
      full_upload = true;
    }
    if (!h_off_.p) {
      h_off_.reserve(M_), h_cnt_.reserve(M_), h_changed_.reserve(M_), h_gcol_.reserve(row), h_hdr_.reserve(M_);
      d_off_.alloc(M_), d_cnt_.alloc(M_), d_gcol_.alloc(row), d_hdr_.alloc(M_);
    }
    EARHIP_LAP(1);
    const float old_scale = gain_scale();
    bool cmax_shrunk = false;
    for (int m : dirty_list_) {
      Obj &o = obj_[m];
      const int n = (int)o.t.size();
      h_off_.p[m] = o.off;
      h_cnt_.p[m] = n;
      h_hdr_.p[m] = ObjHdr{o.off, n, o.t[0], o.t[n - 1], 0};
      std::memcpy(h_time_.p + o.off, o.t.data(), (size_t)n * sizeof(int64_t));
      std::memcpy(h_flat_.p + o.off, o.flat.data(), (size_t)n);
      std::memcpy(h_gain_.p + (size_t)o.off * row, o.g.data(), (size_t)n * row * sizeof(float));
      for (int k = 0; k < n; k++) {
        PointRec &r = h_rec_.p[o.off + k];
        r.time = o.t[k];
        const int64_t len = k ? o.t[k] - o.t[k - 1] : 0;
        r.scale = len > 0 ? 1.0f / (float)len : 0.0f;
        r.flat = o.flat[k];
      }
      float *cm = obj_cmax_.data() + (size_t)m * row;
      if (o.has_stats) cmax_shrunk = retire(o.st, cm) || cmax_shrunk;
      o.st = stats_of(o, cm);
      admit(o.st, cm);
      o.has_stats = true;
    }
    if (cmax_shrunk) {
      for (size_t c = 0; c < row; c++) {
        if (!shrunk_cols_[c]) continue;
        shrunk_cols_[c] = 0;
        float v = 0.0f;
        for (int m = 0; m < M_; m++) {
          const float a = obj_cmax_[(size_t)m * row + c];
          v = a <= v ? v : a;
        }
        cmax_[c] = v;
      }
    }
    EARHIP_LAP(2);
    finish_stats();
    const float set_scale = gain_scale();
    bool gcol_changed = !uploaded_once_ || set_scale != old_scale;
    for (size_t c = 0; c < row; c++) {
      const float cm = cmax_[c];
      int e;
      std::frexp(cm, &e);
      const float v = (cm >= 1e-30f && cm < 1e30f) ? std::ldexp(1.0f, 14 - e) : (set_scale > 0.0f ? set_scale : 1.0f);
      gcol_changed = gcol_changed || v != h_gcol_.p[c];
      h_gcol_.p[c] = v;
    }
    EARHIP_LAP(3);
    if (gcol_changed) EARHIP_HIP(hipMemcpyAsync(d_gcol_.p, h_gcol_.p, row * sizeof(float), hipMemcpyHostToDevice, ctx->stream));
    if (full_upload || dirty_list_.size() > (size_t)M_ / 4) {
      EARHIP_HIP(hipMemcpyAsync(d_off_.p, h_off_.p, M_ * sizeof(int32_t), hipMemcpyHostToDevice, ctx->stream));
      EARHIP_HIP(hipMemcpyAsync(d_cnt_.p, h_cnt_.p, M_ * sizeof(int32_t), hipMemcpyHostToDevice, ctx->stream));
      EARHIP_HIP(hipMemcpyAsync(d_hdr_.p, h_hdr_.p, M_ * sizeof(ObjHdr), hipMemcpyHostToDevice, ctx->stream));
      EARHIP_HIP(hipMemcpyAsync(d_time_.p, h_time_.p, arena_used_ * sizeof(int64_t), hipMemcpyHostToDevice, ctx->stream));
      EARHIP_HIP(hipMemcpyAsync(d_flat_.p, h_flat_.p, arena_used_, hipMemcpyHostToDevice, ctx->stream));
      EARHIP_HIP(hipMemcpyAsync(d_rec_.p, h_rec_.p, arena_used_ * sizeof(PointRec), hipMemcpyHostToDevice, ctx->stream));
      EARHIP_HIP(hipMemcpyAsync(d_gain_.p, h_gain_.p, arena_used_ * row * sizeof(float), hipMemcpyHostToDevice, ctx->stream));
    } else {
      for (size_t i = 0; i < dirty_list_.size(); i++) h_changed_.p[i] = dirty_list_[i];
      CurveImage src{h_hdr_.p, h_off_.p, h_cnt_.p, h_time_.p, h_flat_.p, h_rec_.p, h_gain_.p};
      CurveImage dst{d_hdr_.p, d_off_.p, d_cnt_.p, d_time_.p, d_flat_.p, d_rec_.p, d_gain_.p};
      hipLaunchKernelGGL(k_curve_upload, dim3((unsigned)dirty_list_.size()), dim3(256), 0, ctx->stream, src, dst, h_changed_.p,
                         (int)row);
      EARHIP_HIP(hipGetLastError());
    }
    EARHIP_LAP(4);
    if (kinks_) {
      const bool all = full_upload || gcol_changed || dirty_list_.size() > (size_t)M_ / 4;
      if (!all)
        for (size_t i = 0; i < dirty_list_.size(); i++) h_changed_.p[i] = dirty_list_[i];
      derive_kinks(ctx, all ? nullptr : h_changed_.p, all ? M_ : (int)dirty_list_.size());
    }
    if (!staged_) EARHIP_HIP(hipEventCreateWithFlags(&staged_, hipEventDisableTiming));
    EARHIP_HIP(hipEventRecord(staged_, ctx->stream));
    for (int m : dirty_list_) obj_[m].dirty = false;
    dirty_list_.clear();
    uploaded_once_ = true;
    EARHIP_LAP(5);
  }
#undef EARHIP_LAP

  void ensure_kinks(earhip_ctx *ctx) {
    if (kinks_) return;
    kinks_ = true;
    const size_t row = (size_t)plan_.row;
    EARHIP_HIP(hipStreamSynchronize(ctx->stream));
    d_gain_.alloc(arena_cap_ * row * 2);
    EARHIP_HIP(hipMemcpyAsync(d_gain_.p, h_gain_.p, arena_used_ * row * sizeof(float), hipMemcpyHostToDevice, ctx->stream));
    derive_kinks(ctx, nullptr, M_);
    if (!staged_) EARHIP_HIP(hipEventCreateWithFlags(&staged_, hipEventDisableTiming));
    EARHIP_HIP(hipEventRecord(staged_, ctx->stream));
  }
  bool has_kinks() const { return kinks_; }
  bool dirty() const { return !dirty_list_.empty(); }

  bool tiles_aligned(int tile, int64_t t_call) const {
    const int64_t d = t_call >= t_ref_ ? t_call - t_ref_ : t_ref_ - t_call;
    return d % tile == 0 && grid_ % (uint64_t)tile == 0;
  }

  int aligned_tile(int64_t t_call) const {
    const int grids[2] = {512, 256};
    for (int gi = 0; gi < 2; gi++) {
      const int64_t G = grids[gi];
      const int si = 1 - gi;
      int off_grid_limit = M_ / 64;
      if (ramp_share() < 0.5) {
        const double deltas = deltas_per_pair(si ? 512 : 256);
        off_grid_limit = (int)(M_ * std::min(1.0 / 64, deltas / 200.0));
      }
      if (tiles_aligned((int)G, t_call)) return (int)G;
      if (grid_off_[gi] <= off_grid_limit && (((t_call - grid_phase_[gi]) % G) + G) % G == 0) return (int)G;
    }
    return 0;
  }

  double deltas_per_pair(int tile) const {
    const int gi = tile >= 512 ? 1 : 0;
    return tot_.tiles[gi] > 0 ? tot_.incid[gi] / tot_.tiles[gi] * moving_share() : 0.0;
  }
  double moving_share() const { return M_ > 0 ? (double)tot_.moving / M_ : 0.0; }
  double point_density_all() const { return point_density() * moving_share(); }
  double ramp_share() const { return tot_.span > 0 ? tot_.ramp / tot_.span : 0.0; }
  double point_density() const { return tot_.span > 0 ? tot_.npts / tot_.span : 0.0; }
  double pair_waste(int tile) const {
    const int gi = tile >= 512 ? 1 : 0;
    return (tot_.incid[gi] - tot_.touched[gi]) / std::max(1.0, tot_.tiles[gi] + tot_.incid[gi]);
  }
  double hinge_exact_share(size_t in_stride, size_t nsamples) const {
    if (force_ramp_ || !hinge_addressable((size_t)M_, in_stride, nsamples, 2 * arena_cap_, (size_t)plan_.row)) return 2.0;
    return tot_.span > 0 ? std::min(1.0, tot_.bad / std::max(1.0, tot_.span / kHingeTile)) : 0.0;
  }

  int piece_cap(int tile, bool paired) const {
    const int gi = tile >= 512 ? 1 : 0;
    const long slots = paired ? (long)((M_ + 63) & ~63) + 2 * tot_.sum_r7[gi] : (long)M_ + tot_.sum_r15[gi];
    return (int)std::min<long>(slots + 128, (long)kPieceCapPerObject * M_ + 128);
  }

  float gain_scale() const {
    if (!(gain_max_ < 1e30f)) return 0.0f;
    if (gain_max_ < 1e-18f) return 1.0f;
    int e;
    std::frexp(gain_max_, &e);
    return std::ldexp(1.0f, 14 - e);
  }

  CurveStats stats(int64_t t_call, size_t in_stride, size_t nsamples, bool grid512) const {
    CurveStats s;
    s.aligned_tile = aligned_tile(t_call);
    s.ramp_share = ramp_share();
    s.gain_scale = gain_scale();
    s.point_density = point_density_all();
    s.pair_waste256 = pair_waste(256);
    s.pair_waste512 = pair_waste(512);
    s.hinge_exact_share = hinge_exact_share(in_stride, nsamples);
    s.grid512_strict = grid512 && tiles_aligned(kF32GridTile, t_call);
    s.deltas256 = deltas_per_pair(256);
    return s;
  }

  const float *column_scales() const { return d_gcol_.p; }

  PointStore device() const {
    PointStore ps;
    ps.hdr = d_hdr_.p;
    ps.off = d_off_.p;
    ps.cnt = d_cnt_.p;
    ps.time = d_time_.p;
    ps.flat = d_flat_.p;
    ps.rec = d_rec_.p;
    ps.gain = d_gain_.p;
    ps.row = plan_.row;
    ps.bus_cols = ncols_ / nbus_;
    ps.nbus = nbus_;
    ps.zero_row = 0;
    ps.npoints = (int)tot_.points;
    ps.rows = (int)arena_used_;
    ps.kink_row0 = kinks_ ? (int)arena_cap_ : 0;
    ps.force_ramp = force_ramp_ ? 1 : 0;
    return ps;
  }

 private:
  void derive_kinks(earhip_ctx *ctx, const int32_t *objects, int count) {
    const size_t row = (size_t)plan_.row;
    uint32_t *kink = reinterpret_cast<uint32_t *>(d_gain_.p + arena_cap_ * row);
    EARHIP_HIP(hipMemsetAsync(kink, 0, 2 * row * sizeof(uint32_t), ctx->stream));
    hipLaunchKernelGGL(k_kink_rows, dim3((unsigned)count), dim3(256), 0, ctx->stream, d_off_.p, d_cnt_.p, d_rec_.p, d_gain_.p, kink,
                       d_gcol_.p, objects, (int)row, nbus_);
    EARHIP_HIP(hipGetLastError());
  }
  struct ObjStats {
    uint64_t gcd = 0;
    int64_t first = 0;
    int64_t phase[2] = {-1, -1};
    double span = 0, ramp = 0, npts = 0, bad = 0, points = 0;
    double incid[2] = {0, 0}, touched[2] = {0, 0}, tiles[2] = {0, 0};
    int maxr[2] = {0, 0};
  };
  struct Obj {
    std::vector<int64_t> t;
    std::vector<float> g;
    std::vector<uint8_t> flat;
    int off = 0, cap = 0;
    bool dirty = false, has_stats = false;
    ObjStats st;
  };

  ObjStats stats_of(const Obj &o, float *cm) const {
    ObjStats s;
    const auto &t = o.t;
    const size_t row = (size_t)plan_.row, n = t.size();
    const int allflat = (1 << nbus_) - 1;
    s.first = t[0];
    s.points = (double)n;
    for (size_t k = 1; k < n && s.gcd != 1; k++) {
      uint64_t a = (uint64_t)(t[k] - t[k - 1]), b = s.gcd;
      while (a) {
        const uint64_t r = b % a;
        b = a;
        a = r;
      }
      s.gcd = b;
    }
    const int64_t grids[2] = {512, 256};
    for (int gi = 0; gi < 2; gi++) {
      const int64_t G = grids[gi];
      const int64_t p0 = ((t[0] % G) + G) % G;
      bool same = s.gcd % (uint64_t)G == 0;
      s.phase[gi] = same ? p0 : -1;
    }
    for (size_t k = 1; k < n; k++) {
      const int64_t len = t[k] - t[k - 1];
      const bool is_ramp = (o.flat[k] & allflat) != allflat;
      s.span += (double)len;
      if (is_ramp) s.ramp += (double)len;
      if (len < kHingeMinLen) s.bad += is_ramp ? 1.0 + (double)len / kHingeTile : 0.5;
    }
    if (n > 1) s.npts = (double)(n - 1);
    for (int gi = 0; gi < 2; gi++) {
      const int64_t T = gi ? 512 : 256;
      auto tile_of = [T](int64_t a) { return a >= 0 ? a / T : -((-a + T - 1) / T); };
      if (n > 1) s.tiles[gi] = (double)(t.back() - t.front()) / (double)T;
      int64_t last_tile = INT64_MIN;
      for (size_t k = 1; k < n; k++) {
        if ((o.flat[k] & allflat) == allflat) continue;
        const int64_t a = t[k] > t[k - 1] ? t[k - 1] : t[k] - 1, b = t[k];
        const int64_t ta = tile_of(a), tb = tile_of(b - 1);
        s.incid[gi] += (double)(tb - ta + 1);
        s.touched[gi] += (double)(tb - ta + 1) - (ta == last_tile ? 1.0 : 0.0);
        last_tile = tb;
      }
    }
    for (int gi = 0; gi < 2; gi++) {
      const int64_t T = gi ? 512 : 256;
      auto is_r = [&](size_t k) { return (o.flat[k] & allflat) != allflat; };
      auto ra = [&](size_t k) { return t[k] > t[k - 1] ? t[k - 1] : t[k] - 1; };
      int best = 0, inside = 0;
      size_t j = 1;
      for (size_t i = 1; i < n; i++) {
        if (!is_r(i)) continue;
        if (j < i) j = i, inside = 0;
        while (j < n && (!is_r(j) || ra(j) < t[i] - 1 + T)) {
          if (is_r(j)) inside++;
          j++;
        }
        best = std::max(best, inside);
        inside--;
      }
      s.maxr[gi] = force_ramp_ ? 1 : best;
    }
    for (size_t c = 0; c < row; c++) cm[c] = 0.0f;
    for (size_t k = 0; k < n; k++) {
      const float *g = o.g.data() + k * row;
      for (size_t c = 0; c < row; c++) {
        const float a = std::fabs(g[c]);
        cm[c] = a <= cm[c] ? cm[c] : a;
      }
    }
    return s;
  }
  bool retire(const ObjStats &s, const float *cm) {
    tot_.span -= s.span, tot_.ramp -= s.ramp, tot_.npts -= s.npts, tot_.bad -= s.bad, tot_.points -= s.points;
    tot_.moving -= s.npts > 0 ? 1 : 0;
    for (int gi = 0; gi < 2; gi++) {
      tot_.incid[gi] -= s.incid[gi], tot_.touched[gi] -= s.touched[gi], tot_.tiles[gi] -= s.tiles[gi];
      tot_.sum_r15[gi] -= std::min(s.maxr[gi], kPieceMaxPerObject), tot_.sum_r7[gi] -= std::min(s.maxr[gi], kPairMaxPerObject);
      if (s.phase[gi] >= 0) phases_[gi].add(s.phase[gi], -1);
// ... 20 lines not shown
  void finish_stats() {
    if (grid_stale_) {
      t_ref_ = obj_[0].st.first;
      uint64_t g = 0;
      auto fold = [&g](uint64_t a) {
        uint64_t b = g;
        while (a) {
          const uint64_t r = b % a;
          b = a;
          a = r;
        }
        g = b;
      };
      for (int m = 0; m < M_ && g != 1; m++) {
        const ObjStats &s = obj_[m].st;
        fold(s.gcd);
        fold((uint64_t)(s.first >= t_ref_ ? s.first - t_ref_ : t_ref_ - s.first));
      }
      grid_ = g;
      grid_stale_ = false;
    }
    for (int gi = 0; gi < 2; gi++) {
      int64_t best = 0;
      int best_n = 0;
      for (const auto &kv : phases_[gi].items)
        if (kv.second > best_n) best_n = kv.second, best = kv.first;
      grid_phase_[gi] = best;
      grid_off_[gi] = M_ - best_n;
    }
    float gmax = 0.0f;
    for (float v : cmax_) gmax = v <= gmax ? gmax : v;
    gain_max_ = gmax;
  }

  int M_, ncols_, nbus_;
  bool force_ramp_;
  ColumnPlan plan_;
  std::vector<Obj> obj_;
  std::vector<int> dirty_list_;
  bool uploaded_once_ = false;
  size_t arena_used_ = 2, arena_cap_ = 0, abandoned_ = 0;
  struct Totals {
    double span = 0, ramp = 0, npts = 0, bad = 0, points = 0;
    long moving = 0;
    double incid[2] = {0, 0}, touched[2] = {0, 0}, tiles[2] = {0, 0};
    long sum_r15[2] = {0, 0}, sum_r7[2] = {0, 0};
  } tot_;
  struct PhaseCounts {
    std::vector<std::pair<int64_t, int>> items;
    void add(int64_t phase, int d) {
      for (size_t i = 0; i < items.size(); i++)
        if (items[i].first == phase) {
          items[i].second += d;
          if (items[i].second <= 0) items[i] = items.back(), items.pop_back();
          return;
        }
      if (d > 0) items.emplace_back(phase, d);
    }
  } phases_[2];
  std::vector<float> obj_cmax_;
  std::vector<float> cm_scratch_;
  std::vector<uint8_t> shrunk_cols_;
  bool grid_stale_ = true;
  int64_t t_ref_ = 0;
  uint64_t grid_ = 0;
  int64_t grid_phase_[2] = {0, 0};
  int grid_off_[2] = {0, 0};
  std::vector<float> cmax_;
  float gain_max_ = 0;
  DevBuf<int32_t> d_off_, d_cnt_;
  DevBuf<ObjHdr> d_hdr_;
  PinBuf<ObjHdr> h_hdr_;
  DevBuf<int64_t> d_time_;
  DevBuf<uint8_t> d_flat_;
  DevBuf<PointRec> d_rec_;
  DevBuf<float> d_gcol_, d_gain_;
  bool kinks_ = false;
  PinBuf<float> h_gcol_, h_gain_;
  PinBuf<int32_t> h_off_, h_cnt_, h_changed_;
  PinBuf<int64_t> h_time_;
  PinBuf<uint8_t> h_flat_;
  PinBuf<PointRec> h_rec_;
  hipEvent_t staged_ = nullptr;
};

enum class GainKernel : int {
  Valu = 0,
  Slots = 1,
  F32Grid = 2,
  Grid = 3,
  Pieces = 4,
  Hinge = 5
};

struct MixLaunch {
  GainKernel kind = GainKernel::Valu;
  bool wide = false;
  int pw = 2;
  bool paired = false;
  int hinge_tile = 512;
  int spl;
  int nrt;
  int ntiles, wsplit, gsplit;
  int tpw = 1;
  bool split_operands() const { return kind == GainKernel::Grid || kind == GainKernel::Pieces || kind == GainKernel::Hinge; }
  int tile() const {
    switch (kind) {
      case GainKernel::Valu: return 64 * spl;
      case GainKernel::Slots: return 16 * nrt;
      case GainKernel::F32Grid: return kF32GridTile;
      case GainKernel::Grid: return wide ? 512 : 256;
      case GainKernel::Pieces: return 64 * pw;
      case GainKernel::Hinge: return hinge_tile;
    }
    return 0;
  }
};

inline MixLaunch plan_mix(const earhip_ctx *ctx, const ColumnPlan &cp, int M, int nsamples, bool strict, int max_gsplit,
                          const CurveStats &st) {
  const int aligned_tile = st.aligned_tile;
  const double ramp_share = st.ramp_share, point_density = st.point_density, pair_waste256 = st.pair_waste256,
               pair_waste512 = st.pair_waste512, hinge_exact_share = st.hinge_exact_share, deltas256 = st.deltas256;
  const float gain_scale = st.gain_scale;
  const bool aligned = aligned_tile >= 256;
  MixLaunch L;
  const bool mfma = !strict && ctx->use_mfma;
  bool split = mfma && M >= 32 && gain_scale > 0.0f && ctx->use_mfma != 5 && ctx->use_mfma != 6 &&
               (ctx->use_mfma == 4 || (ctx->use_mfma == 3 && aligned));
  auto object_splits = [&](int ntiles) {
    int g = 1;
    const int nz = cp.mnz * cp.mgroups;
    while (g < max_gsplit && ntiles * nz * g < 2 * ctx->num_cus && M / (g * 2) >= 64) g *= 2;
    return g;
  };
  if (split && !aligned && M / object_splits((nsamples + 255) / 256) > 1024) split = false;
  const int forced = ctx->get(OPT_H2_TILE);
  bool pieces = mfma && !split && M >= 32 && M <= kMaxPieceObjects && gain_scale > 0.0f &&
                (ctx->use_mfma == 3 || ctx->use_mfma == 5 || ctx->use_mfma == 6);
  bool hinge = false;
  if (pieces) {
    const int ptile = ctx->get(OPT_P2_TILE);
    const double kPairWaste = 0.06;
    const double kMostlyRamping = cp.nct == 3 && M <= 1024 ? 0.7 : 0.5;
    const bool paired_by_rule = pair_waste256 < kPairWaste && ramp_share < kMostlyRamping;
    L.paired = paired_by_rule;
    if (ctx->has(OPT_P2_PAIRS)) L.paired = ctx->get(OPT_P2_PAIRS) != 0;
    const bool long_call = nsamples / 512 >= 2 * ctx->num_cus;
    L.pw = ptile == 512 ? 8 : ptile == 256 ? 4 : (L.paired && long_call && pair_waste512 < kPairWaste) ? 8 : 4;
    const double kHingeExact = 0.005, kHingeRamps = 0.5;
    const int hinge_max = (int)std::min((size_t)kMaxHingeCached, ctx->hinge_build_lds / 16);
    hinge = M <= hinge_max && hinge_exact_share <= kHingeExact && ramp_share >= kHingeRamps && !(paired_by_rule && L.paired);
    if (ctx->has(OPT_HINGE)) hinge = ctx->get(OPT_HINGE) != 0 && M <= hinge_max && hinge_exact_share <= 1.0;
    if (ctx->use_mfma == 6) hinge = M <= hinge_max && hinge_exact_share <= 1.0;
    if (ctx->use_mfma == 5) hinge = false;
    if (hinge && !ctx->has(OPT_HINGE) && ctx->use_mfma == 3 && cp.nct == 3 && deltas256 > 0.0 && point_density > 0.0) {
      const double hinge_est = 0.56 + 0.077 * (point_density * 512.0), lists_est = 0.151 + 0.238 * (1.0 + deltas256);
      if (lists_est < 0.97 * hinge_est) hinge = false;
    }
    if (hinge) {
      if (ctx->has(OPT_HG_TILE)) L.hinge_tile = ctx->get(OPT_HG_TILE) == 256 ? 256 : 512;
      pieces = false, L.paired = false, L.pw = 4;
    }
  }
  L.wide = split && aligned_tile >= 512 && forced != 256 && (forced == 512 || nsamples / 512 >= 2 * ctx->num_cus);
  const bool f32grid = mfma && !split && !pieces && !hinge && ctx->use_mfma == 1 && st.grid512_strict && gain_scale > 0.0f &&
// ... 42 lines not shown
void reserve_call_words(earhip_ctx *ctx, int M, size_t max_samples);

struct ScratchLayout {
  struct Region {
    size_t at = 0, units = 0;
  };
  Region desc;
  Region slots;
  Region pieces;
  Region piece_stage;
  Region hinge;
  Region hinge_stage;
  size_t total = 0;
  int M = 0, ntiles = 0, piece_tiles = 0, piece_slots = 0;

  SlotLists slot_lists(SegDesc *base) const {
    SlotLists sl;
    sl.slots = reinterpret_cast<Slot *>(base + slots.at);
    sl.count = reinterpret_cast<int *>(sl.slots + (size_t)kTileSlots * M * ntiles);
    sl.ovf = sl.count + (size_t)4 * ntiles;
    sl.M = M;
    return sl;
  }
  PieceLists piece_lists(SegDesc *base, bool paired) const {
    PieceLists pl;
    pl.pieces = reinterpret_cast<Piece *>(base + pieces.at);
    pl.M = M;
    pl.paired = paired ? 1 : 0;
    pl.slots = piece_slots;
    pl.count = reinterpret_cast<int *>(pl.pieces + (size_t)pl.cap() * piece_tiles);
    pl.ovf = pl.count + (size_t)8 * piece_tiles;
    return pl;
  }
  PairRec *piece_staging(SegDesc *base) const { return reinterpret_cast<PairRec *>(base + piece_stage.at); }
  HingeLists hinge_lists(SegDesc *base) const { return earhip::hinge_lists(base + hinge.at, M, ntiles); }
  HingeCached *hinge_staging(SegDesc *base) const { return reinterpret_cast<HingeCached *>(base + hinge_stage.at); }
};
static_assert(sizeof(Slot) == 16 && sizeof(Piece) == 16 && sizeof(PairRec) == 16 && sizeof(HingeCached) == 16 && sizeof(SegDesc) == 16,
              "the scratch buffer is laid out in 16-byte units");

inline ScratchLayout scratch_layout(GainKernel kind, size_t M, size_t ntiles, size_t piece_tiles, size_t piece_slots) {
  ScratchLayout L;
  L.M = (int)M, L.ntiles = (int)ntiles, L.piece_tiles = (int)piece_tiles, L.piece_slots = (int)piece_slots;
  auto behind = [](const ScratchLayout::Region &r, size_t units) { return ScratchLayout::Region{r.at + r.units, units}; };
  switch (kind) {
    case GainKernel::Valu:
    case GainKernel::F32Grid:
    case GainKernel::Grid:
      L.desc = {0, M * ntiles + 1};
      L.total = L.desc.units;
      break;
    case GainKernel::Slots:
      L.desc = {0, M * ntiles};
      L.slots = behind(L.desc, desc_units(M, ntiles) - M * ntiles);
      L.total = L.slots.at + L.slots.units;
      break;
    case GainKernel::Hinge:
      L.hinge = {0, hinge_units(M, ntiles)};
      L.hinge_stage = behind(L.hinge, M * ntiles);
      [[fallthrough]];
    case GainKernel::Pieces:
      L.pieces = {0, piece_units(M, piece_tiles, piece_slots)};
      L.piece_stage = behind(L.pieces, M * piece_tiles);
      L.total = std::max(L.hinge_stage.at + L.hinge_stage.units, L.piece_stage.at + L.piece_stage.units);
      break;
  }
  return L;
}

inline ScratchLayout scratch_layout(const CurveSet &cs, const MixLaunch &ml, int M, int nsamples = 0) {
  const int ptile = 64 * ml.pw;
  const size_t ptiles = nsamples > 0 ? (size_t)(nsamples + ptile - 1) / ptile
                                     : (size_t)ml.ntiles * (ml.kind == GainKernel::Hinge ? (size_t)std::max(1, ml.tile() / ptile) : 1);
  const bool lists = ml.kind == GainKernel::Pieces || ml.kind == GainKernel::Hinge;
  return scratch_layout(ml.kind, (size_t)M, (size_t)ml.ntiles, lists ? ptiles : 0, lists ? (size_t)cs.piece_cap(ptile, ml.paired) : 0);
}
inline size_t scratch_units(const CurveSet &cs, const MixLaunch &ml, int M) { return scratch_layout(cs, ml, M).total; }

struct MixResult {
  bool gated = false;
  bool device_form = false;
  bool hinge_robust = false;
  bool grew = false;
};

MixResult launch_gain_mix(earhip_ctx *ctx, const CurveSet &cs, const MixLaunch &ml, bool strict,
                          int64_t t_call, int nsamples, const float *in_dev, size_t in_stride,
                          float *out_dev, size_t out_stride, size_t part_stride, SegDesc *desc, unsigned *record,
                          hipEvent_t *ev );

inline MixResult launch_gain_mix_summed(earhip_ctx *ctx, const CurveSet &cs, const MixLaunch &ml, bool strict, int64_t t_call, int nsamples,
                                        const float *in_dev, size_t in_stride, float *out_dev, size_t out_stride, float *parts,
                                        size_t row_stride, SegDesc *desc, unsigned *record, hipEvent_t *ev) {
  if (ml.gsplit == 1) return launch_gain_mix(ctx, cs, ml, strict, t_call, nsamples, in_dev, in_stride, out_dev, out_stride, 0, desc, record, ev);
  const int ncols = cs.ncols();
  const size_t part_stride = row_stride * ncols;
  const MixResult res = launch_gain_mix(ctx, cs, ml, strict, t_call, nsamples, in_dev, in_stride, parts, row_stride, part_stride, desc, record, ev);
  hipLaunchKernelGGL(k_sum_parts, dim3((nsamples + 255) / 256, ncols), dim3(256), 0, ctx->stream, parts, part_stride, ml.gsplit, row_stride,
                     ncols, nsamples, out_dev, out_stride);
  EARHIP_HIP(hipGetLastError());
  return res;
}

}
```

### libear_amd/csrc/gain_h2.h

```cpp
#pragma once

#include <hip/hip_runtime.h>

#include <type_traits>

#include "gain_kernels.h"
#include "gain_mfma.h"
#include "gain_split.h"

namespace earhip {

typedef const SegDesc __attribute__((address_space(4))) *ConstDesc;
template <int NQ>
struct ChunkDesc {
  SegDesc d[NQ];
};
template <int NQ>
struct ChunkCoef {
  float p0[NQ], scale[NQ];
};
template <int NQ>
__device__ __forceinline__ ChunkDesc<NQ> load_desc(const SegDesc *dtile, int m0) {
  ConstDesc dp = (ConstDesc)(dtile + m0);
  ChunkDesc<NQ> D;
#pragma unroll
  for (int q = 0; q < NQ; q++) {
    D.d[q].row = dp[q].row;
    D.d[q].d0 = dp[q].d0;
    D.d[q].scale = dp[q].scale;
    D.d[q].info = dp[q].info;
  }
  return D;
}
template <int NQ, int TILE>
__device__ __forceinline__ void load_gains(const ChunkDesc<NQ> &R, int m0, int m_new, int zero_row, const float *__restrict__ gain,
                                           unsigned rowlen, unsigned bcol_e, ChunkCoef<NQ> &D, float (&S)[NQ], float (&E)[NQ]) {
#pragma unroll
  for (int q = 0; q < NQ; q++) {
    const SegDesc d = R.d[q];
    const bool valid = m0 + q >= m_new && !(d.info & (kSegMulti | kSegQuiet));
    const unsigned rs = (unsigned)(valid ? d.row : zero_row);
    const unsigned re = (valid && (d.info & kSegRamp)) ? (unsigned)d.row + 1u : rs;
    D.p0[q] = d.scale != 0.0f ? (float)(d.d0 + TILE / 2) * d.scale : 0.0f;
    D.scale[q] = d.scale;
    const float *rps = gain + (size_t)rs * rowlen, *rpe = gain + (size_t)re * rowlen;
    S[q] = rps[bcol_e];
    E[q] = rpe[bcol_e];
  }
}
template <int NQ, bool WIDE>
__device__ __forceinline__ void store_b(const ChunkCoef<NQ> &D, const float (&S)[NQ], const float (&E)[NQ], float g_scale, u32x4 *f,
                                        int w, int part) {
  uint32_t h[NQ / 2], l[NQ / 2], hs[NQ / 2];
#pragma unroll
  for (int i = 0; i < NQ / 2; i++) {
    float v[2];
#pragma unroll
    for (int j = 0; j < 2; j++) {
      const int q = 2 * i + j;
      v[j] = (part == 0 ? __builtin_fmaf(1.0f - D.p0[q], S[q], D.p0[q] * E[q]) : D.scale[q] * (E[q] - S[q])) *
             g_scale;
    }
    const uint32_t H = pack_f16(v[0], v[1]);
    h[i] = H;
    l[i] = pack_f16(sub_f16_lo(v[0], H), sub_f16_hi(v[1], H));
    hs[i] = WIDE ? scale_f16x2_down(H) : 0u;
  }
  if constexpr (NQ == 8) {
    f[0] = u32x4{h[0], h[1], h[2], h[3]};
    f[64] = u32x4{l[0], l[1], l[2], l[3]};
    if constexpr (WIDE) f[128] = u32x4{hs[0], hs[1], hs[2], hs[3]};
  } else {
    typedef uint32_t u32x2 __attribute__((ext_vector_type(2)));
    u32x2 *g = reinterpret_cast<u32x2 *>(f) + (w & 1);
    g[0] = u32x2{h[0], h[1]};
    g[128] = u32x2{l[0], l[1]};
    if constexpr (WIDE) g[256] = u32x2{hs[0], hs[1]};
  }
}
template <int NCT, bool WIDE, typename RequestX, typename Convert>
__device__ __forceinline__ void chunk_mfmas(const u32x4 (*bf)[64], int lane, const u32x4 (&ah)[kSplitRowTiles],
                                            const u32x4 (&al)[kSplitRowTiles], f32x4 (&tot0)[kSplitRowTiles][NCT],
                                            f32x4 (&tot1)[kSplitRowTiles][NCT], RequestX request_x, Convert convert) {
  constexpr int NRT = kSplitRowTiles;
  constexpr int XB = 2 * NCT >= 4 ? 4 : 2 * NCT;
  constexpr int NBLK = 2 * NCT;
  u32x4 b[2][2], b2;
  auto load_b = [&](int blk, u32x4 (&bb)[2]) {
#pragma unroll
    for (int q = 0; q < 2; q++) bb[q] = bf[((blk & 1) * NCT + (blk >> 1)) * 3 + q][lane];
  };
  load_b(0, b[0]);
  __builtin_amdgcn_sched_group_barrier(0x100, 2, 0);
#pragma unroll
  for (int blk = 0; blk < NBLK; blk++) {
    u32x4(&bc)[2] = b[blk & 1];
    const int ct = blk >> 1;
    if constexpr (WIDE) b2 = bf[((blk & 1) * NCT + (blk >> 1)) * 3 + 2][lane];
    if (blk + 1 < NBLK) load_b(blk + 1, b[(blk + 1) & 1]);
    f32x4(&tt)[NRT][NCT] = (blk & 1) == 0 ? tot0 : tot1;
    if constexpr (WIDE) {
#pragma unroll
      for (int r = 0; r < NRT; r++) tt[r][ct] = mfma_f16(ah[r], bc[1], tt[r][ct]);
#pragma unroll
      for (int r = 0; r < NRT; r++) tt[r][ct] = mfma_f16(al[r], b2, tt[r][ct]);
    } else {
#pragma unroll
      for (int r = 0; r < NRT; r++) tt[r][ct] = mfma_f16(al[r], bc[0], tt[r][ct]);
#pragma unroll
      for (int r = 0; r < NRT; r++) tt[r][ct] = mfma_f16(ah[r], bc[1], tt[r][ct]);
    }
#pragma unroll
    for (int r = 0; r < NRT; r++) tt[r][ct] = mfma_f16(ah[r], bc[0], tt[r][ct]);
    if (blk < XB) request_x(blk * (8 / XB), 8 / XB);
    const bool conv0 = blk == NBLK - 2, conv1 = blk == NBLK - 1;
    if (conv0) convert(0);
    if (conv1) convert(1);
    if constexpr (WIDE) {
      if (blk + 1 < NBLK) __builtin_amdgcn_sched_group_barrier(0x100, 3, 0);
      else __builtin_amdgcn_sched_group_barrier(0x100, 1, 0);
    } else {
      if (blk + 1 < NBLK) __builtin_amdgcn_sched_group_barrier(0x100, 2, 0);
    }
    if (conv0 || conv1) {
#pragma unroll
      for (int k = 0; k < 12; k++) {
        __builtin_amdgcn_sched_group_barrier(0x008, 1, 0);
        __builtin_amdgcn_sched_group_barrier(0x002, 5, 0);
      }
    } else if (blk < XB) {
#pragma unroll
      for (int k = 0; k < 8 / XB; k++) {
        __builtin_amdgcn_sched_group_barrier(0x008, 12 / (8 / XB), 0);
        __builtin_amdgcn_sched_group_barrier(0x002, 2, 0);
        __builtin_amdgcn_sched_group_barrier(0x020, 1, 0);
      }
    } else {
      __builtin_amdgcn_sched_group_barrier(0x008, 12, 0);
    }
  }
}


constexpr bool h2_persistent(int nct, int nw) { return nw == 8 || nct == 1; }
template <int NCT, int NW, int FORM>
__global__ void __launch_bounds__(64 * NW, NCT == 1 && NW == 8 ? 2 : (NW == 4 ? 2 : 1))
k_gain_mix_h2(GainMixParams P, int zero_row, float x_scale, const float *__restrict__ gcol, const unsigned *level_cur,
              unsigned *level_next, const unsigned *slow_cur, unsigned *slow_next, const unsigned *wide_cur, unsigned *wide_next) {
  if (FORM != 2 && wide_cur && ((*wide_cur & 1u) != 0u) != (FORM == 1)) return;
  constexpr int NRT = 4, TS = 16 * NRT, CH = kSplitChunk;
  constexpr int NQ = CH / NW;
  constexpr int NFRAG = 2 * NCT * 3;
  __shared__ u32x4 bfrag[2][NFRAG + 6][64];
  constexpr int OP = kSplitOutPitch;
  __shared__ __attribute__((aligned(16))) float otile[NW][16 * OP];
  __shared__ float inv_gcol[16 * NCT];
  __shared__ unsigned long long redo_tiles[NW];
  auto body = [&](auto wide_tag) __attribute__((always_inline)) {
  constexpr bool WIDE = decltype(wide_tag)::value;
  if (threadIdx.x < 16 * NCT) inv_gcol[threadIdx.x] = 1.0f / gcol[blockIdx.z * 16 * NCT + threadIdx.x];
  __syncthreads();
  const int lane = threadIdx.x & 63;
  const int w = __builtin_amdgcn_readfirstlane(threadIdx.x >> 6);
  const int li = lane & 15, kg = lane >> 4;
  const int ntl = P.ntiles, gx = gridDim.x;
  const bool runs = P.tile_runs != 0;
  const int run_first = (int)(((int64_t)ntl * blockIdx.x) / gx), run_end = (int)(((int64_t)ntl * (blockIdx.x + 1)) / gx);
  const int vb0 = runs ? run_first : (int)blockIdx.x, vstep = runs ? 1 : gx;
  const int vb_last = runs ? max(run_end - 1, run_first) : ntl - 1;
  const int my_tiles = runs ? run_end - run_first : (ntl - (int)blockIdx.x + gx - 1) / gx;
  auto tile_at = [&](int vb) { return runs ? min(vb, ntl - 1) : xcd_tile(vb, ntl); };
  if (blockIdx.x == 0 && blockIdx.y == 0 && blockIdx.z == 0 && threadIdx.x == 0) {
    if (wide_next) *wide_next = 0u;
    record_mode(P, wide_cur != nullptr);
  }
  if (level_cur) {
    x_scale = probed_input_scale(level_cur, x_scale);
    if (blockIdx.x == 0 && blockIdx.y == 0 && blockIdx.z == 0 && threadIdx.x == 0) *level_next = 0;
  }
  const int nparts = gridDim.y;
  const int part = blockIdx.y;
  const int m_lo = (int)(((int64_t)P.M * part) / nparts);
  const int m_hi = (int)(((int64_t)P.M * (part + 1)) / nparts);
  const int col0 = blockIdx.z * 16 * NCT;
  const float *__restrict__ gain = P.ps.gain;
  const unsigned rowlen = (unsigned)P.ps.row;
  auto tile_first = [&](int t) { return t * (TS * NW) + w * TS; };
  auto tile_length = [&](int t) { return max(0, min(TS, P.nsamples - tile_first(t))); };
  auto opaque_lane = [&]() __attribute__((always_inline)) {
    int l = lane;
    asm volatile("" : "+v"(l));
    return l;
  };

  f32x4 tot0[NRT][NCT], tot1[NRT][NCT];
  auto clear_totals = [&]() {
#pragma unroll
    for (int r = 0; r < NRT; r++)
#pragma unroll
      for (int c = 0; c < NCT; c++) tot0[r][c] = tot1[r][c] = f32x4{0.0f, 0.0f, 0.0f, 0.0f};
  };
  clear_totals();

  auto single_object = [&](int t, int m, float sx, bool sg, int khint = -1) __attribute__((always_inline)) {
    const int tile_s0 = tile_first(t), tile_len = tile_length(t);
    if (tile_len <= 0) return;
    const int64_t tile_t0 = P.t_call + tile_s0, tile_t1 = tile_t0 + tile_len;
    const int ol = opaque_lane(), li = ol & 15, kg = ol >> 4;
    float gsc[NCT];
#pragma unroll
    for (int c = 0; c < NCT; c++) gsc[c] = sg ? gcol[col0 + c * 16 + li] : 1.0f;
    const int base = P.ps.off[m], n = P.ps.cnt[m];
    const float *row = P.in + (size_t)m * P.in_stride + tile_s0;
    int k;
    if (khint >= 0) {
      k = min(khint, n);
      while (k < n && P.ps.time[base + k] <= tile_t0) k++;
    } else {
      k = upper_bound_time(P.ps.time + base, n, tile_t0);
    }
    exact_segments<NCT>(P.ps, base, n, k, row, tile_t0, tile_t1, tile_len, li, kg, gsc, sx, col0, tot0);
  };

  const int nobj = m_hi - m_lo;
  const int nch = (P.vec_ok && nobj >= CH) ? (nobj + CH - 1) / CH : 0;
  auto flush_tile = [&](int t, float inv_x, bool col_scaled) __attribute__((always_inline)) {
    const int tile_s0 = tile_first(t), tile_len = tile_length(t);
    if (tile_len > 0) {
      const int ol = opaque_lane(), li = ol & 15, kg = ol >> 4;
      const float wf0 = (float)(w * TS + kg * 16 - (TS * NW) / 2);
      float inv_gc[NCT];
#pragma unroll
      for (int c = 0; c < NCT; c++) inv_gc[c] = col_scaled ? inv_gcol[c * 16 + li] : 1.0f;
      float *op = P.out + (size_t)blockIdx.y * P.part_stride + tile_s0;
      write_tile<NCT>(tot0, tot1, wf0, inv_x, inv_gc, otile[w], op, P.out_stride, col0, P.ncols, li, kg, tile_len, P.vec_ok);
    }
    clear_totals();
  };

  if (lane == 0) redo_tiles[w] = 0ull;
  if (nch > 0) {
    const int nvec = (P.nsamples + 3) & ~3;
    const unsigned xrow = (unsigned)(kg * 8) * (unsigned)P.in_stride * 4u;
    const int xsl = w * TS + li * NRT;
    struct Stage {
      int tile, c;
    };
    int left = my_tiles * nch;
    int vb_c = vb0;
    auto next_stage = [&](const Stage &s) __attribute__((always_inline)) {
      Stage n;
      const bool wrap = s.c + 1 == nch;
      n.c = wrap ? 0 : s.c + 1;
      if (wrap) vb_c = min(vb_c + vstep, vb_last);
      n.tile = wrap ? tile_at(vb_c) : s.tile;
      return n;
    };
    const unsigned bcol_e = (unsigned)(col0 + min(lane, 16 * NCT - 1));
    const float g_scale = gcol[bcol_e];
    const int blane = (w * NQ / 8) * 16 + (lane & 15);
    const int bfr = lane < 16 * NCT ? (lane >> 4) * 3 : NFRAG;
    const int bfr1 = lane < 16 * NCT ? NCT * 3 : 3;
    auto chunk_base = [&](int c) { return min(m_lo + c * CH, m_hi - CH); };

    auto load_x_part = [&](const Stage &st, bool live, f32x4 (&x)[8], int q0, int n) {
      const int ts0 = st.tile * (TS * NW);
      const char *bp = reinterpret_cast<const char *>(P.in + (live ? (size_t)chunk_base(st.c) * P.in_stride + ts0 : 0));
      const size_t rstride = live ? P.in_stride * sizeof(float) : 0;
      const unsigned xo = live ? xrow + 4u * (unsigned)min(xsl, nvec - 4 - ts0) : 0u;
#pragma unroll
      for (int q = 0; q < 8; q++)
        if (q >= q0 && q < q0 + n)
          x[q] = __builtin_nontemporal_load(reinterpret_cast<const f32x4 *>(bp + (size_t)q * rstride + xo));
    };
    auto load_x = [&](const Stage &st, bool live, f32x4 (&x)[8]) { load_x_part(st, live, x, 0, 8); };
    auto stage_desc = [&](const Stage &st) { return load_desc<NQ>(P.desc + (size_t)st.tile * P.M, chunk_base(st.c) + w * NQ); };
    auto chunk_gains = [&](const ChunkDesc<NQ> &R, int cc, ChunkCoef<NQ> &D, float (&S)[NQ], float (&E)[NQ]) {
      load_gains<NQ, TS * NW>(R, chunk_base(cc) + w * NQ, m_lo + cc * CH, zero_row, gain, rowlen, bcol_e, D, S, E);
    };
    auto convert = [&](const ChunkCoef<NQ> &D, const float (&S)[NQ], const float (&E)[NQ], int buf, int part) {
      store_b<NQ, WIDE>(D, S, E, g_scale, &bfrag[buf][bfr][blane] + (part ? bfr1 * 64 : 0), w, part);
    };

    f32x4 X0[8], X1[8];
    ChunkDesc<NQ> L;
    Stage sa, sb, sc;
    sa.tile = tile_at(vb_c);
    sa.c = 0;
    sb = next_stage(sa);
    sc = next_stage(sb);
    int ka = 0;
    {
      float S[NQ], E[NQ];
      ChunkCoef<NQ> D;
      L = stage_desc(sa);
      chunk_gains(L, 0, D, S, E);
      load_x(sa, true, X0);
      load_x(sb, left > 1, X1);
      convert(D, S, E, 0, 0);
      convert(D, S, E, 0, 1);
      L = stage_desc(sb);
    }
    auto chunk = [&](int buf, f32x4 (&xc)[8]) __attribute__((always_inline)) {
      __syncthreads();
      float S[NQ], E[NQ];
      ChunkCoef<NQ> D;
      chunk_gains(L, sb.c, D, S, E);
      L = stage_desc(sc);
      __builtin_amdgcn_sched_barrier(0);

      u32x4 ah[NRT], al[NRT];
      split_inputs<WIDE>(xc, x_scale, ah, al);
      __builtin_amdgcn_sched_barrier(0);
      chunk_mfmas<NCT, WIDE>(bfrag[buf], lane, ah, al, tot0, tot1,
                             [&](int q0, int n) __attribute__((always_inline)) { load_x_part(sc, left > 2, xc, q0, n); },
                             [&](int part) __attribute__((always_inline)) { convert(D, S, E, buf ^ 1, part); });
    };
    auto tile_end = [&](int t) __attribute__((always_inline)) {
      {
        typedef const unsigned __attribute__((address_space(4))) *ConstWord;
        const bool any_slow = !slow_cur || ((ConstWord)slow_cur)[t] != 0u;
        if (slow_next && blockIdx.y == 0 && blockIdx.z == 0 && threadIdx.x == 0) slow_next[t] = 0u;
        for (int b0 = 0; any_slow && b0 < nobj; b0 += 64) {
          const int ol = opaque_lane();
          const SegDesc db = (P.desc + (size_t)t * P.M)[min(m_lo + b0 + ol, m_hi - 1)];
          unsigned long long multi = __ballot((db.info & (kSegMulti | kSegQuiet)) && b0 + ol < nobj);
          while (multi) {
            const int j = __builtin_ctzll(multi);
            multi &= multi - 1;
            single_object(t, m_lo + b0 + j, x_scale, true, seg_k(__shfl(db.info, j)));
          }
        }
        if (__ballot(totals_not_finite<NCT>(tot0, tot1))) {
          if (lane == 0) redo_tiles[w] |= 1ull << ka;
          clear_totals();
        } else {
          flush_tile(t, 1.0f / x_scale, true);
        }
        ka++;
      }
    };
    auto advance = [&]() __attribute__((always_inline)) {
      if (sa.c == nch - 1) tile_end(sa.tile);
      sa = sb;
      sb = sc;
      sc = next_stage(sc);
      left--;
    };
#pragma unroll 1
    while (left > 0) {
      chunk(0, X0);
      advance();
      if (left <= 0) break;
      chunk(1, X1);
      advance();
    }
  }
  for (int k = 0; k < my_tiles; k++) {
    if (nch > 0 && !((redo_tiles[w] >> (k & 63)) & 1ull)) continue;
    const int t = tile_at(vb0 + k * vstep);
    if (nch == 0 && slow_next && blockIdx.y == 0 && blockIdx.z == 0 && threadIdx.x == 0) slow_next[t] = 0u;
    for (int m = m_lo; m < m_hi; m++) single_object(t, m, 1.0f, false);
    flush_tile(t, 1.0f, false);
  }
  };
  if constexpr (FORM == 2) {
    if (!wide_cur || (*wide_cur & 1u) != 0u) body(std::true_type{});
    else body(std::false_type{});
  } else {
    body(std::integral_constant<bool, FORM == 1>{});
  }
}

}
```

### libear_amd/csrc/gain_h2_t1.h

```cpp
#pragma once

#include "gain_h2.h"

namespace earhip {

template <int NCT, int NW, bool WIDE>
__global__ void __launch_bounds__(64 * NW, 2)
k_gain_mix_h2_t1(GainMixParams P, int zero_row, float x_scale, const float *__restrict__ gcol, const unsigned *level_cur,
              unsigned *level_next, const unsigned *slow_cur, unsigned *slow_next, const unsigned *wide_cur, unsigned *wide_next) {
  if (wide_cur && ((*wide_cur & 1u) != 0u) != WIDE) return;
  constexpr int NRT = 4, TS = 16 * NRT, CH = kSplitChunk;
  constexpr int NQ = CH / NW;
  constexpr int NFRAG = 2 * NCT * 3;
  __shared__ u32x4 bfrag[2][NFRAG + 6][64];
  constexpr int OP = kSplitOutPitch;
  __shared__ __attribute__((aligned(16))) float otile[NW][16 * OP];
  __shared__ float inv_gcol[16 * NCT];
  if (threadIdx.x < 16 * NCT) inv_gcol[threadIdx.x] = 1.0f / gcol[blockIdx.z * 16 * NCT + threadIdx.x];
  __syncthreads();
  const int lane = threadIdx.x & 63;
  const int w = __builtin_amdgcn_readfirstlane(threadIdx.x >> 6);
  const int li = lane & 15, kg = lane >> 4;
  const int wgtile = xcd_tile(blockIdx.x, gridDim.x);
  if (blockIdx.x == 0 && blockIdx.y == 0 && blockIdx.z == 0 && threadIdx.x == 0) {
    if (wide_next) *wide_next = 0u;
    record_mode(P, wide_cur != nullptr);
  }
  if (level_cur) {
    x_scale = probed_input_scale(level_cur, x_scale);
    if (blockIdx.x == 0 && blockIdx.y == 0 && blockIdx.z == 0 && threadIdx.x == 0) *level_next = 0;
  }
  const bool any_slow = !slow_cur || slow_cur[wgtile] != 0u;
  if (slow_next && blockIdx.y == 0 && blockIdx.z == 0 && threadIdx.x == 0) slow_next[wgtile] = 0u;
  const int nparts = gridDim.y;
  const int part = blockIdx.y;
  const int m_lo = (int)(((int64_t)P.M * part) / nparts);
  const int m_hi = (int)(((int64_t)P.M * (part + 1)) / nparts);
  const int col0 = blockIdx.z * 16 * NCT;
  const int tile_s0 = wgtile * (TS * NW) + w * TS;
  const int tile_len = max(0, min(TS, P.nsamples - tile_s0));
  const int64_t tile_t0 = P.t_call + tile_s0;
  const int64_t tile_t1 = tile_t0 + tile_len;
  const SegDesc *__restrict__ dtile = P.desc + (size_t)wgtile * P.M;
  const float *__restrict__ gain = P.ps.gain;
  const unsigned rowlen = (unsigned)P.ps.row;

  f32x4 tot0[NRT][NCT], tot1[NRT][NCT];
  auto clear_totals = [&]() {
#pragma unroll
    for (int r = 0; r < NRT; r++)
#pragma unroll
      for (int c = 0; c < NCT; c++) tot0[r][c] = tot1[r][c] = f32x4{0.0f, 0.0f, 0.0f, 0.0f};
  };
  clear_totals();

  auto single_object = [&](int m, float sx, bool sg, int khint = -1) {
    if (tile_len <= 0) return;
    float gsc[NCT];
#pragma unroll
    for (int c = 0; c < NCT; c++) gsc[c] = sg ? gcol[col0 + c * 16 + li] : 1.0f;
    const int base = P.ps.off[m], n = P.ps.cnt[m];
    const float *row = P.in + (size_t)m * P.in_stride + tile_s0;
    int k;
    if (khint >= 0) {
      k = min(khint, n);
      while (k < n && P.ps.time[base + k] <= tile_t0) k++;
    } else {
      k = upper_bound_time(P.ps.time + base, n, tile_t0);
    }
    exact_segments<NCT>(P.ps, base, n, k, row, tile_t0, tile_t1, tile_len, li, kg, gsc, sx, col0, tot0);
  };

  const int nobj = m_hi - m_lo;
  const int nch = (P.vec_ok && nobj >= CH) ? (nobj + CH - 1) / CH : 0;
  float inv_x = 1.0f / x_scale;
  bool col_scaled = true;

  if (nch > 0) {
    const int nvec = (P.nsamples + 3) & ~3;
    const unsigned xs = (unsigned)min(tile_s0 + li * NRT, nvec - 4);
    const unsigned xlane = ((unsigned)(kg * 8) * (unsigned)P.in_stride + xs) * 4u;
    const unsigned bcol_e = (unsigned)(col0 + min(lane, 16 * NCT - 1));
    const float g_scale = gcol[bcol_e];
    const int blane = (w * NQ / 8) * 16 + (lane & 15);
    const int bfr = lane < 16 * NCT ? (lane >> 4) * 3 : NFRAG;
    const int bfr1 = lane < 16 * NCT ? NCT * 3 : 3;
    auto chunk_base = [&](int c) { return min(m_lo + c * CH, m_hi - CH); };

    auto load_x_part = [&](int c, f32x4 (&x)[8], int q0, int n) {
      const bool live = c < nch;
      const char *bp = reinterpret_cast<const char *>(P.in + (live ? (size_t)chunk_base(c) * P.in_stride : 0));
      const size_t rstride = live ? P.in_stride * sizeof(float) : 0;
      const unsigned xo = live ? xlane : 0u;
#pragma unroll
      for (int q = 0; q < 8; q++)
        if (q >= q0 && q < q0 + n)
          x[q] = __builtin_nontemporal_load(reinterpret_cast<const f32x4 *>(bp + (size_t)q * rstride + xo));
    };
    auto load_x = [&](int c, f32x4 (&x)[8]) { load_x_part(c, x, 0, 8); };
    auto chunk_desc = [&](int c) { return load_desc<NQ>(dtile, chunk_base(min(c, nch - 1)) + w * NQ); };
    auto chunk_gains = [&](const ChunkDesc<NQ> &R, int c, ChunkCoef<NQ> &D, float (&S)[NQ], float (&E)[NQ]) {
      const int cc = min(c, nch - 1);
      load_gains<NQ, TS * NW>(R, chunk_base(cc) + w * NQ, m_lo + cc * CH, zero_row, gain, rowlen, bcol_e, D, S, E);
    };
    auto convert = [&](const ChunkCoef<NQ> &D, const float (&S)[NQ], const float (&E)[NQ], int buf, int part) {
      store_b<NQ, WIDE>(D, S, E, g_scale, &bfrag[buf][bfr][blane] + (part ? bfr1 * 64 : 0), w, part);
    };

    f32x4 X0[8], X1[8];
    ChunkDesc<NQ> L;
    {
      float S[NQ], E[NQ];
      ChunkCoef<NQ> D;
      L = chunk_desc(0);
      chunk_gains(L, 0, D, S, E);
      load_x(0, X0);
      load_x(1, X1);
      convert(D, S, E, 0, 0);
      convert(D, S, E, 0, 1);
      L = chunk_desc(1);
    }
    auto chunk = [&](int c, int buf, f32x4 (&xc)[8]) {
      __syncthreads();
      float S[NQ], E[NQ];
      ChunkCoef<NQ> D;
      chunk_gains(L, c + 1, D, S, E);
      L = chunk_desc(c + 2);
      __builtin_amdgcn_sched_barrier(0);

      u32x4 ah[NRT], al[NRT];
      split_inputs<WIDE>(xc, x_scale, ah, al);
      __builtin_amdgcn_sched_barrier(0);
      chunk_mfmas<NCT, WIDE>(bfrag[buf], lane, ah, al, tot0, tot1,
                             [&](int q0, int n) __attribute__((always_inline)) { load_x_part(c + 2, xc, q0, n); },
                             [&](int part) __attribute__((always_inline)) { convert(D, S, E, buf ^ 1, part); });
    };
#pragma unroll 1
    for (int c = 0; c < nch; c += 2) {
      chunk(c, 0, X0);
      if (c + 1 < nch) chunk(c + 1, 1, X1);
    }

    for (int b0 = 0; any_slow && b0 < nobj; b0 += 64) {
      const SegDesc db = dtile[min(m_lo + b0 + lane, m_hi - 1)];
      unsigned long long multi = __ballot((db.info & (kSegMulti | kSegQuiet)) && b0 + lane < nobj);
      while (multi) {
        const int j = __builtin_ctzll(multi);
        multi &= multi - 1;
        single_object(m_lo + b0 + j, x_scale, true, seg_k(__shfl(db.info, j)));
      }
    }
    if (__ballot(totals_not_finite<NCT>(tot0, tot1))) {
      clear_totals();
      inv_x = 1.0f;
      col_scaled = false;
      for (int m = m_lo; m < m_hi; m++) single_object(m, 1.0f, false);
    }
  } else {
    inv_x = 1.0f;
    col_scaled = false;
    for (int m = m_lo; m < m_hi; m++) single_object(m, 1.0f, false);
  }

  if (tile_len <= 0) return;
  const float wf0 = (float)(w * TS + kg * 16 - (TS * NW) / 2);
  float inv_gc[NCT];
#pragma unroll
  for (int c = 0; c < NCT; c++) inv_gc[c] = col_scaled ? inv_gcol[c * 16 + li] : 1.0f;
  float *op = P.out + (size_t)blockIdx.y * P.part_stride + tile_s0;
  write_tile<NCT>(tot0, tot1, wf0, inv_x, inv_gc, otile[w], op, P.out_stride, col0, P.ncols, li, kg, tile_len, P.vec_ok);
}

}
```

### libear_amd/csrc/gain_kernels.h

```cpp
#pragma once

#include <hip/hip_runtime.h>

#include <cstdint>

#include "search.h"

namespace earhip {

struct PointRec {
  int64_t time;
  float scale;
  uint32_t flat;
};
static_assert(sizeof(PointRec) == 16, "PointRec is loaded as one dwordx4");

struct ObjHdr {
  int32_t off, cnt;
  int64_t first, last;
  int64_t reserved;
};
static_assert(sizeof(ObjHdr) == 32, "an object's header is two dwordx4 loads");
struct PointStore {
  const ObjHdr *hdr;
// ... 23 lines not shown

constexpr int kSegRamp = 1;
constexpr int kSegMulti = 2;
constexpr int kSegQuiet = (int)0x80000000u;
constexpr int kMaxPointsPerObject = (1 << 18) - 1;
static_assert((((unsigned)kMaxPointsPerObject << 13) & (unsigned)kSegQuiet) == 0u, "the segment index must not reach the quiet flag");
__host__ __device__ __forceinline__ int seg_r1(int info) { return (info >> 4) & 0x1ff; }
__host__ __device__ __forceinline__ int seg_k(int info) { return (info >> 13) & 0x3ffff; }


__device__ __forceinline__ int xcd_tile(int b, int n) {
  const int per = n >> 3;
  if (b >= per * 8) return b;
  return (b & 7) * per + (b >> 3);
}

__device__ __forceinline__ SegDesc describe_segment(const PointStore &ps, int base,
                                                    int n, int k, int64_t t0,
                                                    int64_t t_end) {
  SegDesc d;
  if (ps.force_ramp) k = 1;
  const int allflat = (1 << ps.nbus) - 1;
  const int fb = (k > 0 && k < n) ? (ps.flat[base + k] & allflat) : allflat;
  const bool ramp = ps.force_ramp || fb != allflat;
  const bool multi = !ps.force_ramp && k < n && ps.time[base + k] < t_end;
  const int r1 = min((int)((multi ? ps.time[base + k] : t_end) - t0), 511);
  d.info = (k << 13) | (r1 << 4) | (fb << 2) | (multi ? kSegMulti : 0) | (ramp ? kSegRamp : 0);
  if (ramp) {
    const int64_t start = ps.time[base + k - 1], end = ps.time[base + k];
    d.row = base + k - 1;
    d.d0 = (int32_t)(t0 - start);
    d.scale = 1.0f / (float)(end - start);
  } else {
    d.row = base + (k == n ? k - 1 : k);
    d.d0 = 0;
    d.scale = 0.0f;
  }
  return d;
}

__device__ __forceinline__ SegDesc describe_segment_rec(const PointStore &ps, int base, int n, int k, int64_t t0,
                                                        int64_t t_end) {
  if (ps.force_ramp) return describe_segment(ps, base, n, k, t0, t_end);
  const int allflat = (1 << ps.nbus) - 1;
  PointRec r, q;
  r.time = t_end;
  r.scale = 0.0f;
  r.flat = (uint32_t)allflat;
  q = r;
  if (k < n) r = ps.rec[base + k];
  if (k > 0) q = ps.rec[base + k - 1];
  const int fb = (k > 0 && k < n) ? ((int)r.flat & allflat) : allflat;
  const bool ramp = fb != allflat;
  const bool multi = k < n && r.time < t_end;
  const int r1 = min((int)((multi ? r.time : t_end) - t0), 511);
  SegDesc d;
  d.info = (k << 13) | (r1 << 4) | (fb << 2) | (multi ? kSegMulti : 0) | (ramp ? kSegRamp : 0);
  if (ramp) {
    d.row = base + k - 1;
    d.d0 = (int32_t)(t0 - q.time);
    d.scale = r.scale;
  } else {
    d.row = base + (k == n ? k - 1 : k);
    d.d0 = 0;
    d.scale = 0.0f;
  }
  return d;
}

struct LevelProbe {
  const float *in = nullptr;
  size_t in_stride = 0;
  int nsamples = 0;
  int every = 1;
  unsigned *level = nullptr;
  unsigned *obj_level = nullptr;
};
constexpr int kQuietBinades = 20;
constexpr int kPlainBinades = 8;
__host__ __device__ __forceinline__ bool level_is_quiet(unsigned obj_level, unsigned call_level) {
  return obj_level != 0u && call_level != 0u && (int)(obj_level >> 23) < (int)(call_level >> 23) - kQuietBinades;
}
constexpr int kProbeInstants = 64, kProbeObjects = 16;
static __global__ void __launch_bounds__(64 * kProbeObjects)
k_level_probe(const float *in, size_t in_stride, int nsamples, int M, unsigned *level, unsigned *obj_level, int cap, int nruns) {
  __shared__ unsigned wmax[kProbeObjects];
  const int lane = threadIdx.x & 63, wv = threadIdx.x >> 6, m = blockIdx.x * kProbeObjects + wv;
  const int nvec = nsamples >> 2, ninst = min(kProbeInstants, nvec);
  unsigned v = 0u;
  if (m < M && lane < ninst) {
    const unsigned sh = (unsigned)__builtin_ctz((unsigned)nruns), per = 64u >> sh;
    const unsigned nrun = max((unsigned)ninst / per, 1u), g = min((unsigned)lane / per, nrun - 1u), sub = (unsigned)lane & (per - 1u);
    const unsigned stretch = (unsigned)nvec / nrun;
    const unsigned h = ((unsigned)m * 2654435761u) ^ (g * 40503u);
    const unsigned room = stretch > per ? stretch - per + 1u : 1u;
    const int at = (int)min(g * stretch + __umulhi(h, room) + sub, (unsigned)nvec - 1u);
    const float4 px = *reinterpret_cast<const float4 *>(in + (size_t)m * in_stride + 4 * (size_t)at);
    v = max(max(__float_as_uint(px.x) & 0x7fffffffu, __float_as_uint(px.y) & 0x7fffffffu),
            max(__float_as_uint(px.z) & 0x7fffffffu, __float_as_uint(px.w) & 0x7fffffffu));
  }
  unsigned hi_v = v, lo_v = v ? v : 0xffffffffu;
#pragma unroll
  for (int d = 32; d >= 1; d >>= 1) {
    hi_v = max(hi_v, (unsigned)__shfl_xor((int)hi_v, d));
    lo_v = min(lo_v, (unsigned)__shfl_xor((int)lo_v, d));
  }
  if (lane == 0) {
    wmax[wv] = hi_v;
    if (m < M) {
      obj_level[m] = hi_v;
      obj_level[cap + m] = lo_v == 0xffffffffu ? 0u : lo_v;
    }
  }
  __syncthreads();
  if (threadIdx.x == 0) {
    unsigned he = 0u;
#pragma unroll
    for (int i = 0; i < kProbeObjects; i++) he = max(he, wmax[i]);
    he &= 0x7f800000u;
    if (he != 0 && he > __atomic_load_n(level, __ATOMIC_RELAXED)) atomicMax(level, he);
  }
}

constexpr int kHingeSpreadBinades = 16;
constexpr unsigned kGateHingeUnsafe = 2u;
constexpr int kGateQuietShift = 8;
__host__ __device__ __forceinline__ bool hinge_span_exceeded(unsigned word, int M) {
  const int limit = M / 64 > 4 ? M / 64 : 4;
  return (word & kGateHingeUnsafe) != 0u || (int)(word >> kGateQuietShift) > limit;
}
static __global__ void __launch_bounds__(256)
k_hinge_gate(const unsigned *obj_level, int cap, int M, const unsigned *level_cur, unsigned *gate, bool wide, bool count_quiet) {
  const int m = blockIdx.x * 256 + threadIdx.x;
  bool unsafe = false, quiet = false;
  if (m < M) {
    const unsigned hi = obj_level[m], lo = obj_level[cap + m], call = *level_cur;
    const bool exact_anyway = hi != 0u && call != 0u && (int)(hi >> 23) < (int)(call >> 23) - kHingeSpreadBinades;
    unsafe = !exact_anyway && lo != 0u && call != 0u && (int)(lo >> 23) < (int)(call >> 23) - kHingeSpreadBinades;
    quiet = exact_anyway;
  }
  if (__syncthreads_or(unsafe ? 1 : 0) && threadIdx.x == 0) atomicOr(gate, kGateHingeUnsafe);
  if (count_quiet) {
    const int nq = __syncthreads_count(quiet ? 1 : 0);
    if (nq > 0 && threadIdx.x == 0) atomicAdd(gate, (unsigned)nq << kGateQuietShift);
  }
  if (wide) {
    bool wd = false;
    if (m < M) {
      const unsigned lo = obj_level[cap + m], call = *level_cur;
      wd = lo != 0u && call != 0u && (int)(lo >> 23) < (int)(call >> 23) - kPlainBinades;
    }
    if (__syncthreads_or(wd ? 1 : 0) && threadIdx.x == 0) atomicOr(gate, 1u);
  }
}

struct QuietMark {
  const unsigned *obj_level = nullptr;
  int cap = 0;
  const unsigned *level = nullptr;
  unsigned *wide = nullptr;
};
template <int kPrepRun>
static __global__ void __launch_bounds__(256)
k_seg_prep(PointStore ps, int M, int ntiles, int tile_samples, int64_t t_call, int64_t t_call_end,
           SegDesc *desc, QuietMark qm, unsigned *tile_slow = nullptr) {
  __shared__ SegDesc sh[16 * kPrepRun][17];
  const int ti = threadIdx.x & 15, oi = threadIdx.x >> 4;
  const int tile0 = (blockIdx.x * 16 + ti) * kPrepRun, m = blockIdx.y * 16 + oi;
  bool quiet = false;
  if (qm.obj_level && m < M) {
    const unsigned call = *qm.level, lv = qm.obj_level[m], lo = qm.obj_level[qm.cap + m];
    quiet = level_is_quiet(lv, call);
    if (qm.wide && blockIdx.x == 0 && ti == 0 && lo != 0u && call != 0u && (int)(lo >> 23) < (int)(call >> 23) - kPlainBinades)
      atomicOr(qm.wide, 1u);
  }
  if (tile0 < ntiles && m < M) {
    const ObjHdr hd = ps.hdr[m];
    const int base = hd.off, n = hd.cnt;
    int k = 0;
#pragma unroll
    for (int j = 0; j < kPrepRun; j++) {
      const int tile = tile0 + j;
      if (tile >= ntiles) break;
      const int64_t t0 = t_call + (int64_t)tile * tile_samples;
      int64_t t_end = t0 + tile_samples;
      if (t_end > t_call_end) t_end = t_call_end;
      if (j == 0) {
        k = upper_bound_rec_window(ps.rec + base, n, hd.first, hd.last, t0);
      } else {
        while (k < n && ps.rec[base + k].time <= t0) k++;
      }
      SegDesc d = describe_segment_rec(ps, base, n, k, t0, t_end);
      if (quiet) d.info |= kSegQuiet;
      sh[ti * kPrepRun + j][oi] = d;
      if (tile_slow && (quiet || (d.info & kSegMulti))) atomicOr(&tile_slow[tile], 1u);
    }
  }
  __syncthreads();
#pragma unroll
  for (int j = 0; j < kPrepRun; j++) {
    const int to = (threadIdx.x >> 4) + 16 * j, oo = threadIdx.x & 15;
    const int tile_o = blockIdx.x * 16 * kPrepRun + to, m_o = blockIdx.y * 16 + oo;
    if (tile_o < ntiles && m_o < M) desc[(size_t)tile_o * M + m_o] = sh[to][oo];
  }
}

struct Slot {
  uint32_t mr;
  int32_t row;
  float alpha, beta;
};
static_assert(sizeof(Slot) == 16, "Slot is loaded as one dwordx4");
constexpr int kMaxSlotObjects = 1 << 16;
constexpr int kPlainSlots = 2;
constexpr int kMaskedSlots = 6;
constexpr int kTileSlots = kPlainSlots + kMaskedSlots;
struct SlotLists {
  Slot *slots;
  int *count;
  int *ovf;
  int M;
};
__host__ __device__ inline size_t desc_units(size_t M, size_t ntiles) {
  return (1 + kTileSlots) * M * ntiles + (16 * ntiles + 4 * M * ntiles + 15) / 16 + 1;
}

static __global__ void __launch_bounds__(256)
k_slot_list(PointStore ps, int M, int tile_samples, int64_t t_call, int64_t t_call_end,
            const SegDesc *desc, SlotLists sl) {
  __shared__ unsigned wsum[4];
  __shared__ int base_p, base_m, base_o, written_m, any_over;
  const int tile = blockIdx.x, tid = threadIdx.x, lane = tid & 63, wv = tid >> 6;
  const int64_t t0 = t_call + (int64_t)tile * tile_samples;
  int64_t t_end = t0 + tile_samples;
  if (t_end > t_call_end) t_end = t_call_end;
  Slot *plain = sl.slots + (size_t)tile * kTileSlots * M;
  Slot *masked = plain + kPlainSlots * (size_t)M;
  int *ovf = sl.ovf + (size_t)tile * M;
  if (tid == 0) {
    base_p = 0;
    base_m = 0;
    base_o = 0;
    written_m = 0;
  }
  __syncthreads();
  auto walk = [&](int m, SegDesc dk, Slot *op, Slot *om, int &cp, int &cm, SegDesc (&nx)[2], bool fill) {
    int base = 0, n = 0;
    if (dk.info & kSegMulti) {
      base = ps.off[m];
      n = ps.cnt[m];
    }
    int k = seg_k(dk.info), cur = 0, step = 0;
    cp = 0;
    cm = 0;
    for (;;) {
      const int r1 = seg_r1(dk.info);
      if (r1 > cur) {
        const bool ramp = dk.info & kSegRamp;
        const bool whole = cur == 0 && r1 == tile_samples;
        Slot a;
        a.mr = (uint32_t)m | ((uint32_t)cur << 16) | ((uint32_t)(r1 - 1) << 24);
        a.row = dk.row;
        const float p0 = (float)dk.d0 * dk.scale;
        a.alpha = ramp ? 1.0f - p0 : 1.0f;
        a.beta = ramp ? -dk.scale : 0.0f;
        Slot *o = whole ? op : om;
        int &c = whole ? cp : cm;
        if (o) o[c] = a;
        c++;
        if (ramp) {
          Slot b = a;
          b.row = dk.row + 1;
          b.alpha = p0;
          b.beta = dk.scale;
          if (o) o[c] = b;
          c++;
        }
        cur = r1;
      }
      if (!(dk.info & kSegMulti)) break;
      k++;
      if (step < 2 && !fill) {
        dk = nx[step];
      } else {
        dk = describe_segment(ps, base, n, k, t0, t_end);
        if (step < 2) nx[step] = dk;
// ... 10 lines not shown
    if (lane == 63) wsum[wv] = v;
    __syncthreads();
    unsigned pre = 0, tot = 0;
#pragma unroll
    for (int w = 0; w < 4; w++) {
      const unsigned x = wsum[w];
      if (w < wv) pre += x;
      tot += x;
    }
    __syncthreads();
    total = tot;
    return v + pre;
  };
  for (int mb = 0; mb < M; mb += 256) {
    const int m = mb + tid;
    SegDesc d, nx[2];
    d.info = 0;
    int cp = 0, cm = 0;
    if (m < M) {
      if (desc) {
        d = desc[(size_t)tile * M + m];
      } else {
        const int base = ps.off[m], n = ps.cnt[m];
        d = describe_segment(ps, base, n, upper_bound_time_window(ps.time + base, n, t0), t0, t_end);
      }
      walk(m, d, nullptr, nullptr, cp, cm, nx, true);
    }
    unsigned last;
    const unsigned incl = block_scan((unsigned)cp | ((unsigned)cm << 10), last);
    const int off_p = base_p + (int)(incl & 1023u) - cp;
    const int off_m = base_m + (int)(incl >> 10) - cm;
    const bool over = cm > 0 && off_m + cm > kMaskedSlots * M;
    if (tid == 0) any_over = 0;
    __syncthreads();
    if (over) any_over = 1;
    __syncthreads();
    unsigned oincl = 0, olast = 0;
    if (any_over) oincl = block_scan(over ? 1u : 0u, olast);
    if (m < M) {
      if (over) {
        ovf[base_o + (int)oincl - 1] = m;
      } else if (cp + cm > 0) {
        int a, b;
        walk(m, d, plain + off_p, masked + off_m, a, b, nx, false);
        if (cm > 0) atomicMax(&written_m, off_m + cm);
      }
    }
    __syncthreads();
    if (tid == 0) {
      base_p += (int)(last & 1023u);
      base_m += (int)(last >> 10);
      base_o += (int)olast;
    }
    __syncthreads();
  }
  if (tid == 0) {
    sl.count[tile * 4 + 0] = base_p;
    sl.count[tile * 4 + 1] = written_m;
    sl.count[tile * 4 + 2] = base_o;
  }
}

struct GainMixParams {
  const float *in;
  size_t in_stride;
  float *out;
  size_t out_stride;
  size_t part_stride;
  const SegDesc *desc;
  PointStore ps;
  int64_t t_call;
  int nsamples;
  int ntiles;
  int M;
  int ncols;
  int ngroups;
  int wsplit;
  int tiles_per_wg;
  int vec_ok;
  SlotLists sl;
  int tile_runs = 0;
  const unsigned *mode_word = nullptr;
  unsigned *record = nullptr;
};
constexpr unsigned kModeRecorded = 4u;
__device__ __forceinline__ void record_mode(const GainMixParams &P, bool device_form) {
  if (P.record) *P.record = (P.mode_word ? *P.mode_word : 0u) | (device_form ? 0u : 1u) | kModeRecorded;
}

template <int NOUT, int SPL, bool STRICT, bool PARTIAL>
__device__ __forceinline__ void accumulate_piece(float (&acc)[NOUT][SPL], const float (&xs)[SPL], const bool (&on)[SPL],
                                                 const SegDesc d, const float *__restrict__ rows,
                                                 int rowlen, int lane, int col0, int bus_cols) {
  const bool ramp = d.info & kSegRamp;
  const float *__restrict__ S = rows;
  const float *__restrict__ E = rows + (ramp ? rowlen : 0);
  float p[SPL], q[SPL];
#pragma unroll
  for (int i = 0; i < SPL; i++) {
    p[i] = (float)(d.d0 + lane * SPL + i) * d.scale;
    q[i] = 1.0f - p[i];
  }
  if (STRICT) {
#pragma unroll
    for (int j = 0; j < NOUT; j++) {
      const float s = S[j], e = E[j];
      const bool cflat = !ramp || ((d.info >> (2 + (col0 + j >= bus_cols ? 1 : 0))) & 1);
#pragma unroll
      for (int i = 0; i < SPL; i++) {
        const float g = cflat ? e : q[i] * s + p[i] * e;
        const float v = acc[j][i] + xs[i] * g;
        acc[j][i] = !PARTIAL || on[i] ? v : acc[j][i];
      }
    }
  } else {
    float a[SPL], b[SPL];
#pragma unroll
    for (int i = 0; i < SPL; i++) {
      a[i] = ramp ? xs[i] * q[i] : xs[i];
      b[i] = xs[i] * p[i];
    }
#pragma unroll
    for (int j = 0; j < NOUT; j++) {
      const float s = S[j];
#pragma unroll
      for (int i = 0; i < SPL; i++) acc[j][i] = __builtin_fmaf(a[i], s, acc[j][i]);
    }
    if (ramp) {
#pragma unroll
      for (int j = 0; j < NOUT; j++) {
        const float e = E[j];
#pragma unroll
        for (int i = 0; i < SPL; i++) acc[j][i] = __builtin_fmaf(b[i], e, acc[j][i]);
      }
    }
  }
}

template <int NOUT, int SPL, bool STRICT>
__global__ void __launch_bounds__(512) k_gain_mix(GainMixParams P) {
  constexpr int TS = 64 * SPL;
  typedef float vec_t __attribute__((ext_vector_type(SPL)));
  extern __shared__ __attribute__((aligned(16))) float lds[];
  const int lane = threadIdx.x & 63;
  const int wave = __builtin_amdgcn_readfirstlane(threadIdx.x >> 6);
  const int g = wave % P.ngroups;
  const int ws = wave / P.ngroups;
  const int tile = blockIdx.x;
  const int nparts = P.wsplit * gridDim.y;
  const int part = blockIdx.y * P.wsplit + ws;
  const int m_lo = (int)(((int64_t)P.M * part) / nparts);
  const int m_hi = (int)(((int64_t)P.M * (part + 1)) / nparts);
  const int col0 = (blockIdx.z * P.ngroups + g) * NOUT;

  const int s0 = tile * TS + lane * SPL;
  const int64_t tile_t0 = P.t_call + (int64_t)tile * TS;
  int64_t tile_t1 = tile_t0 + TS;
  if (tile_t1 > P.t_call + P.nsamples) tile_t1 = P.t_call + P.nsamples;
  const bool full = P.vec_ok && s0 + SPL - 1 < P.nsamples;

  float acc[NOUT][SPL];
#pragma unroll
  for (int j = 0; j < NOUT; j++)
#pragma unroll
    for (int i = 0; i < SPL; i++) acc[j][i] = 0.0f;

// ... 111 lines not shown
```

Before: 1.160 million.

## Precompute per-tile segment descriptor tables across calls for grid gain kernel

Adds a persistent per-tile segment descriptor table, built once from the curve points and updated incrementally for changed objects, so grid-kernel calls index into it instead of running the per-call descriptor prep kernel. Per-call quiet state is moved out of the descriptors into a separate per-object mark array. The level probe now fills that array in its last block, using a ticket counter, and sets an any-quiet mode bit. Gain kernels are specialised to OR in these marks only when some object is quiet. This removes a per-call kernel launch and its descriptor writes, at the cost of extra device memory, table rebuilds when curves change, and more complex cross-kernel synchronisation.

```diff
diff --git a/include/earhip.h b/include/earhip.h
--- a/include/earhip.h
+++ b/include/earhip.h
@@ -318,6 +318,7 @@
 int earhip_render_last_plan(const earhip_render *r, int out[4]);
 int earhip_render_last_decor_plan(const earhip_render *r, int out[4]);
 int earhip_render_last_list_layout(const earhip_render *r, int *paired);
+int earhip_render_last_desc_source(const earhip_render *r, int *src);
 int earhip_render_last_tail_blocks(const earhip_render *r, int *blocks);
 int earhip_render_last_host_chunks(const earhip_render *r, int *chunks);
 int earhip_render_scratch_bytes(const earhip_render *r, size_t *bytes);
diff --git a/libear_amd/capi.py b/libear_amd/capi.py
--- a/libear_amd/capi.py
+++ b/libear_amd/capi.py
@@ -1202,6 +1202,11 @@
         v = C.c_int(0)
         check(load().earhip_render_last_list_layout(self.h, C.byref(v)))
         return None if v.value < 0 else bool(v.value)
+
+    def last_desc_source(self):
+        v = C.c_int(0)
+        check(load().earhip_render_last_desc_source(self.h, C.byref(v)))
+        return v.value
 
     def last_plan(self):
         out = (C.c_int * 4)()
diff --git a/libear_amd/csrc/api_core.hip b/libear_amd/csrc/api_core.hip
--- a/libear_amd/csrc/api_core.hip
+++ b/libear_amd/csrc/api_core.hip
@@ -46,17 +46,18 @@
   unsigned *gate = nullptr;
   unsigned *slow_cur = nullptr, *slow_next = nullptr;
   unsigned *obj_level = nullptr;
+  const unsigned *qmark = nullptr;
   bool grew = false;
 };
 
 static int grow_call_words(earhip_ctx *ctx, int M, size_t ntiles, size_t tile_cap) {
   int made = 0;
-  if (M > 0 && !ctx->level.p) ctx->level.alloc_zero(4, ctx->stream), made++;
+  if (M > 0 && !ctx->level.p) ctx->level.alloc_zero(8, ctx->stream), made++;
   const bool grow_obj = ctx->obj_level_cap < M, grow_tiles = ctx->tile_slow_cap < ntiles;
   if (grow_obj || grow_tiles) EARHIP_HIP(hipStreamSynchronize(ctx->stream));
   if (grow_obj) {
     ctx->obj_level_cap = M + M / 2 + 64;
-    ctx->obj_level.alloc_zero(2 * (size_t)ctx->obj_level_cap, ctx->stream);
+    ctx->obj_level.alloc_zero(3 * (size_t)ctx->obj_level_cap, ctx->stream);
     made++;
   }
   if (grow_tiles) {
@@ -73,16 +74,19 @@
   grow_call_words(ctx, M, ntiles, ntiles + ntiles / 4);
 }
 
-static CallWords acquire_call_words(earhip_ctx *ctx, const MixLaunch &ml, int M, const float *in_dev, size_t in_stride, int nsamples) {
+static CallWords acquire_call_words(earhip_ctx *ctx, const MixLaunch &ml, int M, const float *in_dev, size_t in_stride, int nsamples,
+                                    const unsigned *tab_multi) {
   CallWords w;
   if (!ml.split_operands()) return w;
   const bool probe = ctx->x_scale_auto && in_stride % 4 == 0 && ((uintptr_t)in_dev & 15) == 0;
-  const size_t slow_tiles = ml.kind == GainKernel::Grid ? (size_t)ml.ntiles : 0;
-  if (!probe && !slow_tiles) return w;
+  const bool grid = ml.kind == GainKernel::Grid;
+  const size_t slow_tiles = grid && !tab_multi ? (size_t)ml.ntiles : 0;
+  if (!probe && !grid) return w;
   if ((probe && (!ctx->level.p || ctx->obj_level_cap < M)) || ctx->tile_slow_cap < slow_tiles) {
     ctx->lazy_allocs += grow_call_words(ctx, probe ? M : 0, slow_tiles, 2 * slow_tiles);
     w.grew = true;
   }
+  if (tab_multi) w.slow_cur = const_cast<unsigned *>(tab_multi);
   if (slow_tiles) {
     w.slow_cur = ctx->tile_slow.p + (size_t)ctx->tile_slow_idx * ctx->tile_slow_cap;
     w.slow_next = ctx->tile_slow.p + (size_t)(ctx->tile_slow_idx ^ 1) * ctx->tile_slow_cap;
@@ -98,8 +102,16 @@
   w.obj_level = ctx->obj_level.p;
   const int v = ctx->get(OPT_PROBE_RUNS);
   const int probe_runs = v >= 1 && v <= 64 && (v & (v - 1)) == 0 ? v : 16;
+  QuietOut qo;
+  if (tab_multi) {
+    qo.mark = ctx->obj_level.p + 2 * (size_t)ctx->obj_level_cap;
+    qo.mode = w.gate;
+    qo.ticket = ctx->level.p + 4;
+    qo.wide = w.wide_cur != nullptr;
+    w.qmark = qo.mark;
+  }
   hipLaunchKernelGGL(k_level_probe, dim3((M + kProbeObjects - 1) / kProbeObjects), dim3(64 * kProbeObjects), 0, ctx->stream, in_dev,
-                     in_stride, nsamples, M, w.level_cur, ctx->obj_level.p, ctx->obj_level_cap, probe_runs);
+                     in_stride, nsamples, M, w.level_cur, ctx->obj_level.p, ctx->obj_level_cap, probe_runs, qo);
   return w;
 }
 
@@ -118,6 +130,7 @@
   SlotLists sl;
   PieceLists pl;
   HingeLists hl;
+  DescTableView tab;
   CallWords w;
   bool hg_robust = false, standby = false;
   GainMixParams P;
@@ -338,7 +351,8 @@
   P.out = out_dev;
   P.out_stride = out_stride;
   P.part_stride = part_stride;
-  P.desc = c.scratch;
+  P.desc = c.tab.desc ? c.tab.desc : c.scratch;
+  P.qmark = c.w.qmark;
   P.ps = c.ps;
   P.t_call = c.t_call;
   P.nsamples = c.nsamples;
@@ -362,7 +376,8 @@
   if (kind == GainKernel::Hinge) c.hl = c.lay.hinge_lists(desc);
   if (kind == GainKernel::Slots && c.M > kMaxSlotObjects) fail_internal("slot lists address objects with 16 bits");
   if (ev) EARHIP_HIP(hipEventRecord(ev[0], ctx->stream));
-  c.w = acquire_call_words(ctx, ml, c.M, in_dev, in_stride, nsamples);
+  if (kind == GainKernel::Grid && ctx->get(OPT_DESC_TABLE, 1) != 0) c.tab = cs.desc_table(ml.tile(), t_call, nsamples);
+  c.w = acquire_call_words(ctx, ml, c.M, in_dev, in_stride, nsamples, c.tab.multi);
   c.hg_robust = kind == GainKernel::Hinge && ctx->get(OPT_HG_ROBUST, 1) != 0;
   c.standby = kind == GainKernel::Hinge && c.w.gate && !c.hg_robust;
   switch (kind) {
@@ -377,7 +392,9 @@
       prep_slot_lists(c, own_search);
       break;
     }
-    default: prep_descriptors(c); break;
+    default:
+      if (!c.tab.desc) prep_descriptors(c);
+      break;
   }
   if (ev) EARHIP_HIP(hipEventRecord(ev[1], ctx->stream));
   c.P = mix_params(c, out_dev, out_stride, part_stride, record);
@@ -400,6 +417,7 @@
   res.device_form = c.w.wide_cur != nullptr;
   res.hinge_robust = res.gated && c.hg_robust;
   res.grew = c.w.grew;
+  res.desc_table = c.tab.desc != nullptr;
   return res;
 }
 
@@ -469,7 +487,7 @@
 
 static const char *const kOptNames[OPT_COUNT] = {
     "SPL", "MFMA", "XSCALE", "WAVES", "TPW", "NRT", "H2_TILE", "H2_WGS", "H2_RUNS", "P2_TILE", "P2_PAIRS", "P2_WGS", "HINGE", "HG_TILE", "HBUILD_TPW",
-    "BUILD_TPW", "K2_WG", "K2_OWN_BLOCK", "RUN", "GSPLIT", "PROBE_RUNS", "BLOCK_GROUPS", "DEBUG_TIMING", "TAILCUT", "HOST_CHUNK_MB", "HOST_THREADS", "HG_ROBUST", "BUILD_2K", "HOST_BIND", "HOST_NT", "HOST_FIRST", "H2_PAIR"};
+    "BUILD_TPW", "K2_WG", "K2_OWN_BLOCK", "RUN", "GSPLIT", "PROBE_RUNS", "BLOCK_GROUPS", "DEBUG_TIMING", "TAILCUT", "HOST_CHUNK_MB", "HOST_THREADS", "HG_ROBUST", "BUILD_2K", "HOST_BIND", "HOST_NT", "HOST_FIRST", "H2_PAIR", "DESC_TABLE"};
 
 static int parse_option_value(const std::string &key, const char *text) {
   char *end = nullptr;
@@ -570,7 +588,7 @@
                 ((uintptr_t)in_dev & 15) == 0,
             "buffer must be 16-byte aligned with stride and nsamples multiples of 256");
     ctx->use();
-    if (!ctx->level.p) ctx->level.alloc_zero(4, ctx->stream);
+    if (!ctx->level.p) ctx->level.alloc_zero(8, ctx->stream);
     float *sink = reinterpret_cast<float *>(ctx->level.p);
     hipEvent_t e[4];
     for (auto &x : e) EARHIP_HIP(hipEventCreate(&x));
diff --git a/libear_amd/csrc/api_render.hip b/libear_amd/csrc/api_render.hip
--- a/libear_amd/csrc/api_render.hip
+++ b/libear_amd/csrc/api_render.hip
@@ -21,6 +21,7 @@
   bool device_form = false;
   bool hg_robust = false;
   int tail_blocks = 0;
+  bool desc_table = false;
 };
 
 struct earhip_render {
@@ -167,15 +168,23 @@
   }
 
   size_t last_in_stride = 0;
+  size_t desc_table_units(int tile) const { return kDescTableCalls * ((size_t)M * (((size_t)T * B + tile - 1) / tile) + 1); }
+  void sync_desc_tables(const bool (&want)[2]) {
+    const size_t units[2] = {desc_table_units(256), desc_table_units(512)};
+    curves->sync_desc_tables(ctx, want, units);
+  }
   void reserve_for_curves() {
     size_t need = 0;
     bool hinge = false;
+    bool table[2] = {false, false};
     const size_t lens[3] = {(size_t)T, (size_t)std::max(1, T / 2), (size_t)1};
     for (size_t nb : lens) {
       const MixLaunch ml = plan_call(nb, last_in_stride ? last_in_stride : nb * (size_t)B);
       need = std::max(need, scratch_units(*curves, ml, M));
       hinge = hinge || ml.kind == GainKernel::Hinge;
-    }
+      if (ml.kind == GainKernel::Grid && ctx->get(OPT_DESC_TABLE, 1) != 0) table[ml.tile() >= 512 ? 1 : 0] = true;
+    }
+    sync_desc_tables(table);
     if (hinge) curves->ensure_kinks(ctx);
     if (need > desc.n) {
       EARHIP_HIP(hipStreamSynchronize(ctx->stream));
@@ -282,6 +291,11 @@
     if (ml.kind == GainKernel::Hinge) curves->ensure_kinks(ctx);
 
     report.kind = (int)ml.kind;
+    if (ml.kind == GainKernel::Grid && ctx->get(OPT_DESC_TABLE, 1) != 0 && curves->desc_table_pending(ml.tile())) {
+      bool table[2] = {ml.tile() < 512, ml.tile() >= 512};
+      sync_desc_tables(table);
+      scratch_regrows++;
+    }
     {
       const size_t need = scratch_units(*curves, ml, M);
       if (need > desc.n) {
@@ -319,6 +333,7 @@
     }
     if (timed) pending.push_back(pd);
     report.gated = mix.gated, report.device_form = mix.device_form, report.hg_robust = mix.hinge_robust;
+    report.desc_table = mix.desc_table;
     if (mix.grew) scratch_regrows++;
     t += nsamples;
   }
@@ -811,6 +826,13 @@
   });
 }
 
+int earhip_render_last_desc_source(const earhip_render *r, int *src) {
+  return guarded([&] {
+    require(r != nullptr && src != nullptr, "NULL argument");
+    *src = r->report.desc_table ? 1 : 0;
+  });
+}
+
 int earhip_render_last_list_layout(const earhip_render *r, int *paired) {
   return guarded([&] {
     require(r != nullptr && paired != nullptr, "NULL argument");
diff --git a/libear_amd/csrc/common.h b/libear_amd/csrc/common.h
--- a/libear_amd/csrc/common.h
+++ b/libear_amd/csrc/common.h
@@ -121,7 +121,7 @@
   OPT_H2_TILE, OPT_H2_WGS, OPT_H2_RUNS, OPT_P2_TILE, OPT_P2_PAIRS, OPT_P2_WGS, OPT_HINGE, OPT_HG_TILE, OPT_HBUILD_TPW, OPT_BUILD_TPW,
   OPT_K2_WG, OPT_K2_OWN_BLOCK, OPT_RUN, OPT_GSPLIT,
   OPT_PROBE_RUNS, OPT_BLOCK_GROUPS, OPT_DEBUG_TIMING, OPT_TAILCUT, OPT_HOST_CHUNK_MB, OPT_HOST_THREADS, OPT_HG_ROBUST, OPT_BUILD_2K,
-  OPT_HOST_BIND, OPT_HOST_NT, OPT_HOST_FIRST, OPT_H2_PAIR, OPT_COUNT
+  OPT_HOST_BIND, OPT_HOST_NT, OPT_HOST_FIRST, OPT_H2_PAIR, OPT_DESC_TABLE, OPT_COUNT
 };
 struct OptVal {
   bool set = false;
diff --git a/libear_amd/csrc/curves.h b/libear_amd/csrc/curves.h
--- a/libear_amd/csrc/curves.h
+++ b/libear_amd/csrc/curves.h
@@ -10,6 +10,7 @@
 #include <vector>
 
 #include "common.h"
+#include "desc_table.h"
 #include "gain_kernels.h"
 #include "gain_p2.h"
 #include "gain_hg.h"
@@ -78,6 +79,11 @@
   double deltas256 = 0.0;
 };
 
+struct DescTableView {
+  const SegDesc *desc = nullptr;
+  const unsigned *multi = nullptr;
+};
+
 class CurveSet {
  public:
   CurveSet(int M, int ncols, int nbus = 1, bool force_ramp = false)
@@ -94,6 +100,7 @@
     cm_scratch_.assign(plan_.row, 0.0f);
     shrunk_cols_.assign(plan_.row, 0);
     dirty_list_.reserve(M);
+    tab_changed_.reserve(M);
     for (auto &p : phases_) p.items.reserve(M);
   }
   ~CurveSet() {
@@ -301,6 +308,10 @@
     }
     if (!staged_) EARHIP_HIP(hipEventCreateWithFlags(&staged_, hipEventDisableTiming));
     EARHIP_HIP(hipEventRecord(staged_, ctx->stream));
+    tab_synced_ = false;
+    if (tab_[0].tried || tab_[1].tried)
+      for (int m : dirty_list_)
+        if (!obj_[m].tab_stale) obj_[m].tab_stale = true, tab_changed_.push_back(m);
     for (int m : dirty_list_) obj_[m].dirty = false;
     dirty_list_.clear();
     uploaded_once_ = true;
@@ -320,6 +331,71 @@
     EARHIP_HIP(hipEventRecord(staged_, ctx->stream));
   }
   bool has_kinks() const { return kinks_; }
+
+  void sync_desc_tables(earhip_ctx *ctx, const bool (&want)[2], const size_t (&max_units)[2]) {
+    if (!dirty_list_.empty()) fail_internal("descriptor tables: uncommitted curves");
+    int64_t first = obj_[0].t.front(), last = obj_[0].t.back();
+    for (int m = 1; m < M_; m++) first = std::min(first, obj_[m].t.front()), last = std::max(last, obj_[m].t.back());
+    const PointStore ps = device();
+    bool list_staged = false;
+    for (int gi = 0; gi < 2; gi++) {
+      DescTable &T = tab_[gi];
+      if (!want[gi] && !T.tried) continue;
+      if (want[gi]) T.max_units = max_units[gi];
+      const int tile = gi ? 512 : 256;
+      DescTableRange range;
+      if (!force_ramp_) range = desc_table_range(true, first, last, tile, (size_t)M_, T.max_units);
+      if (range.n >= ((int64_t)1 << 30)) range = DescTableRange{};
+      const bool all = !T.tried || !(range == T.range) || tab_changed_.size() > (size_t)M_ / 4;
+      T.tried = true;
+      T.range = range;
+      if (range.n == 0 || (!all && tab_changed_.empty())) continue;
+      const size_t units = (size_t)range.n * M_;
+      if (units > T.desc.n || (size_t)range.n > T.multi.n) {
+        EARHIP_HIP(hipStreamSynchronize(ctx->stream));
+        const size_t cap = std::max(units, std::min(T.max_units, units + units / 2));
+        T.desc.alloc(cap);
+        T.multi.alloc(cap / M_ + 1);
+      }
+      const int nt = (int)range.n, run = nt >= 2048 ? 4 : 2;
+      const int32_t *objects = nullptr;
+      int count = M_;
+      if (all) {
+        EARHIP_HIP(hipMemsetAsync(T.multi.p, 0, (size_t)nt * sizeof(unsigned), ctx->stream));
+      } else {
+        if (!list_staged) {
+          if (staged_) EARHIP_HIP(hipEventSynchronize(staged_));
+          h_tab_changed_.reserve(M_);
+          for (size_t i = 0; i < tab_changed_.size(); i++) h_tab_changed_.p[i] = tab_changed_[i];
+          list_staged = true;
+        }
+        objects = h_tab_changed_.p;
+        count = (int)tab_changed_.size();
+      }
+      const dim3 grid((nt + 16 * run - 1) / (16 * run), (count + 15) / 16);
+      if (run == 4)
+        hipLaunchKernelGGL(k_desc_table<4>, grid, dim3(256), 0, ctx->stream, ps, M_, objects, count, nt, tile, range.lo, T.desc.p, T.multi.p, all);
+      else
+        hipLaunchKernelGGL(k_desc_table<2>, grid, dim3(256), 0, ctx->stream, ps, M_, objects, count, nt, tile, range.lo, T.desc.p, T.multi.p, all);
+      EARHIP_HIP(hipGetLastError());
+    }
+    for (int m : tab_changed_) obj_[m].tab_stale = false;
+    tab_changed_.clear();
+    tab_synced_ = true;
+    if (list_staged) EARHIP_HIP(hipEventRecord(staged_, ctx->stream));
+  }
+  bool desc_table_pending(int tile) const { return !force_ramp_ && (!tab_[tile >= 512 ? 1 : 0].tried || !tab_synced_); }
+  DescTableView desc_table(int tile, int64_t t_call, int nsamples) const {
+    DescTableView v;
+    const int gi = tile >= 512 ? 1 : 0;
+    const DescTable &T = tab_[gi];
+    if (!tab_synced_ || !dirty_list_.empty()) return v;
+    if (!desc_table_usable(T.range, gi ? 512 : 256, true, force_ramp_, t_call, nsamples, tile)) return v;
+    const int64_t i0 = desc_table_index(T.range, t_call, tile);
+    v.desc = T.desc.p + (size_t)i0 * M_;
+    v.multi = T.multi.p + i0;
+    return v;
+  }
   bool dirty() const { return !dirty_list_.empty(); }
 
   bool tiles_aligned(int tile, int64_t t_call) const {
@@ -433,6 +509,7 @@
     std::vector<uint8_t> flat;
     int off = 0, cap = 0;
     bool dirty = false, has_stats = false;
+    bool tab_stale = false;
     ObjStats st;
   };
 
@@ -619,6 +696,16 @@
   PinBuf<uint8_t> h_flat_;
   PinBuf<PointRec> h_rec_;
   hipEvent_t staged_ = nullptr;
+  struct DescTable {
+    DevBuf<SegDesc> desc;
+    DevBuf<unsigned> multi;
+    DescTableRange range;
+    size_t max_units = 0;
+    bool tried = false;
+  } tab_[2];
+  std::vector<int> tab_changed_;
+  PinBuf<int32_t> h_tab_changed_;
+  bool tab_synced_ = false;
 };
 
 enum class GainKernel : int {
@@ -827,6 +914,7 @@
   bool device_form = false;
   bool hinge_robust = false;
   bool grew = false;
+  bool desc_table = false;
 };
 
 MixResult launch_gain_mix(earhip_ctx *ctx, const CurveSet &cs, const MixLaunch &ml, bool strict,
diff --git a/libear_amd/csrc/desc_table.h b/libear_amd/csrc/desc_table.h
--- /dev/null
+++ b/libear_amd/csrc/desc_table.h
@@ -0,0 +1,41 @@
+#pragma once
+
+#include <cstddef>
+#include <cstdint>
+
+namespace earhip {
+
+inline int64_t floor_div(int64_t a, int64_t b) { return a >= 0 ? a / b : -((-a + b - 1) / b); }
+
+constexpr size_t kDescTableCalls = 2;
+
+struct DescTableRange {
+  int64_t lo = 0;
+  int64_t n = 0;
+  bool operator==(const DescTableRange &o) const { return lo == o.lo && n == o.n; }
+};
+
+inline DescTableRange desc_table_range(bool have_points, int64_t first, int64_t last, int tile, size_t M, size_t max_units) {
+  DescTableRange r;
+  if (!have_points || tile <= 0 || M == 0 || last < first) return r;
+  if (first < INT64_MIN / 2 || last > INT64_MAX / 2) return r;
+  const int64_t lo = floor_div(first, tile) - 1;
+  const int64_t hi = floor_div(last + tile - 1, tile) + 1;
+  const int64_t n = hi - lo;
+  if (n <= 0 || (uint64_t)n > max_units / M) return r;
+  r.lo = lo;
+  r.n = n;
+  return r;
+}
+
+inline int64_t desc_table_index(const DescTableRange &r, int64_t t_call, int tile) { return floor_div(t_call, tile) - r.lo; }
+
+inline bool desc_table_usable(const DescTableRange &r, int table_tile, bool grid_kind, bool force_ramp, int64_t t_call, int64_t nsamples,
+                              int tile) {
+  if (r.n <= 0 || !grid_kind || force_ramp || tile <= 0 || tile != table_tile || nsamples <= 0) return false;
+  if (t_call % tile != 0 || nsamples % tile != 0) return false;
+  const int64_t i0 = desc_table_index(r, t_call, tile), nt = nsamples / tile;
+  return i0 >= 0 && nt <= r.n && i0 <= r.n - nt;
+}
+
+}
diff --git a/libear_amd/csrc/gain_h2.h b/libear_amd/csrc/gain_h2.h
--- a/libear_amd/csrc/gain_h2.h
+++ b/libear_amd/csrc/gain_h2.h
@@ -19,16 +19,19 @@
 struct ChunkCoef {
   float p0[NQ], scale[NQ];
 };
-template <int NQ>
-__device__ __forceinline__ ChunkDesc<NQ> load_desc(const SegDesc *dtile, int m0) {
+typedef const unsigned __attribute__((address_space(4))) *ConstWord;
+template <int NQ, bool MARKS>
+__device__ __forceinline__ ChunkDesc<NQ> load_desc(const SegDesc *dtile, const unsigned *qmark, int m0) {
   ConstDesc dp = (ConstDesc)(dtile + m0);
+  ConstWord qp = (ConstWord)(qmark + (MARKS ? m0 : 0));
   ChunkDesc<NQ> D;
 #pragma unroll
   for (int q = 0; q < NQ; q++) {
     D.d[q].row = dp[q].row;
     D.d[q].d0 = dp[q].d0;
     D.d[q].scale = dp[q].scale;
-    D.d[q].info = dp[q].info;
+    if constexpr (MARKS) D.d[q].info = dp[q].info | (int)qp[q];
+    else D.d[q].info = dp[q].info;
   }
   return D;
 }
@@ -156,8 +159,8 @@
   __shared__ __attribute__((aligned(16))) float otile[NW][16 * OP];
   __shared__ float inv_gcol[16 * NCT];
   __shared__ unsigned long long redo_tiles[NW];
-  auto body = [&](auto wide_tag) __attribute__((always_inline)) {
-  constexpr bool WIDE = decltype(wide_tag)::value;
+  auto body = [&](auto wide_tag, auto marks_tag) __attribute__((always_inline)) {
+  constexpr bool WIDE = decltype(wide_tag)::value, MARKS = decltype(marks_tag)::value;
   if (threadIdx.x < 16 * NCT) inv_gcol[threadIdx.x] = 1.0f / gcol[blockIdx.z * 16 * NCT + threadIdx.x];
   __syncthreads();
   const int lane = threadIdx.x & 63;
@@ -274,7 +277,7 @@
           x[q] = __builtin_nontemporal_load(reinterpret_cast<const f32x4 *>(bp + (size_t)q * rstride + xo));
     };
     auto load_x = [&](const Stage &st, bool live, f32x4 (&x)[8]) { load_x_part(st, live, x, 0, 8); };
-    auto stage_desc = [&](const Stage &st) { return load_desc<NQ>(P.desc + (size_t)st.tile * P.M, chunk_base(st.c) + w * NQ); };
+    auto stage_desc = [&](const Stage &st) { return load_desc<NQ, MARKS>(P.desc + (size_t)st.tile * P.M, P.qmark, chunk_base(st.c) + w * NQ); };
     auto chunk_gains = [&](const ChunkDesc<NQ> &R, int cc, ChunkCoef<NQ> &D, float (&S)[NQ], float (&E)[NQ]) {
       load_gains<NQ, TS * NW>(R, chunk_base(cc) + w * NQ, m_lo + cc * CH, zero_row, gain, rowlen, bcol_e, D, S, E);
     };
@@ -318,12 +321,12 @@
     };
     auto tile_end = [&](int t) __attribute__((always_inline)) {
       {
-        typedef const unsigned __attribute__((address_space(4))) *ConstWord;
-        const bool any_slow = !slow_cur || ((ConstWord)slow_cur)[t] != 0u;
+        const bool any_slow = MARKS || !slow_cur || ((ConstWord)slow_cur)[t] != 0u;
         if (slow_next && blockIdx.y == 0 && blockIdx.z == 0 && threadIdx.x == 0) slow_next[t] = 0u;
         for (int b0 = 0; any_slow && b0 < nobj; b0 += 64) {
           const int ol = opaque_lane();
-          const SegDesc db = (P.desc + (size_t)t * P.M)[min(m_lo + b0 + ol, m_hi - 1)];
+          SegDesc db = (P.desc + (size_t)t * P.M)[min(m_lo + b0 + ol, m_hi - 1)];
+          if constexpr (MARKS) db.info |= (int)P.qmark[min(m_lo + b0 + ol, m_hi - 1)];
           unsigned long long multi = __ballot((db.info & (kSegMulti | kSegQuiet)) && b0 + ol < nobj);
           while (multi) {
             const int j = __builtin_ctzll(multi);
@@ -364,12 +367,17 @@
     flush_tile(t, 1.0f, false);
   }
   };
+  const bool marks = P.qmark && P.mode_word && (*P.mode_word & kModeAnyQuiet) != 0u;
+  auto run = [&](auto wide_tag) __attribute__((always_inline)) {
+    if (marks) body(wide_tag, std::true_type{});
+    else body(wide_tag, std::false_type{});
+  };
   if constexpr (FORM == 2) {
-    if (!wide_cur || (*wide_cur & 1u) != 0u) body(std::true_type{});
-    else body(std::false_type{});
+    if (!wide_cur || (*wide_cur & 1u) != 0u) run(std::true_type{});
+    else run(std::false_type{});
   } else {
-    body(std::integral_constant<bool, FORM == 1>{});
-  }
-}
-
-}
+    run(std::integral_constant<bool, FORM == 1>{});
+  }
+}
+
+}
diff --git a/libear_amd/csrc/gain_h2_t1.h b/libear_amd/csrc/gain_h2_t1.h
--- a/libear_amd/csrc/gain_h2_t1.h
+++ b/libear_amd/csrc/gain_h2_t1.h
@@ -16,6 +16,8 @@
   constexpr int OP = kSplitOutPitch;
   __shared__ __attribute__((aligned(16))) float otile[NW][16 * OP];
   __shared__ float inv_gcol[16 * NCT];
+  auto body = [&](auto marks_tag) __attribute__((always_inline)) {
+  constexpr bool MARKS = decltype(marks_tag)::value;
   if (threadIdx.x < 16 * NCT) inv_gcol[threadIdx.x] = 1.0f / gcol[blockIdx.z * 16 * NCT + threadIdx.x];
   __syncthreads();
   const int lane = threadIdx.x & 63;
@@ -30,7 +32,7 @@
     x_scale = probed_input_scale(level_cur, x_scale);
     if (blockIdx.x == 0 && blockIdx.y == 0 && blockIdx.z == 0 && threadIdx.x == 0) *level_next = 0;
   }
-  const bool any_slow = !slow_cur || slow_cur[wgtile] != 0u;
+  const bool any_slow = MARKS || !slow_cur || slow_cur[wgtile] != 0u;
   if (slow_next && blockIdx.y == 0 && blockIdx.z == 0 && threadIdx.x == 0) slow_next[wgtile] = 0u;
   const int nparts = gridDim.y;
   const int part = blockIdx.y;
@@ -98,7 +100,7 @@
           x[q] = __builtin_nontemporal_load(reinterpret_cast<const f32x4 *>(bp + (size_t)q * rstride + xo));
     };
     auto load_x = [&](int c, f32x4 (&x)[8]) { load_x_part(c, x, 0, 8); };
-    auto chunk_desc = [&](int c) { return load_desc<NQ>(dtile, chunk_base(min(c, nch - 1)) + w * NQ); };
+    auto chunk_desc = [&](int c) { return load_desc<NQ, MARKS>(dtile, P.qmark, chunk_base(min(c, nch - 1)) + w * NQ); };
     auto chunk_gains = [&](const ChunkDesc<NQ> &R, int c, ChunkCoef<NQ> &D, float (&S)[NQ], float (&E)[NQ]) {
       const int cc = min(c, nch - 1);
       load_gains<NQ, TS * NW>(R, chunk_base(cc) + w * NQ, m_lo + cc * CH, zero_row, gain, rowlen, bcol_e, D, S, E);
@@ -142,7 +144,8 @@
     }
 
     for (int b0 = 0; any_slow && b0 < nobj; b0 += 64) {
-      const SegDesc db = dtile[min(m_lo + b0 + lane, m_hi - 1)];
+      SegDesc db = dtile[min(m_lo + b0 + lane, m_hi - 1)];
+      if constexpr (MARKS) db.info |= (int)P.qmark[min(m_lo + b0 + lane, m_hi - 1)];
       unsigned long long multi = __ballot((db.info & (kSegMulti | kSegQuiet)) && b0 + lane < nobj);
       while (multi) {
         const int j = __builtin_ctzll(multi);
@@ -169,6 +172,9 @@
   for (int c = 0; c < NCT; c++) inv_gc[c] = col_scaled ? inv_gcol[c * 16 + li] : 1.0f;
   float *op = P.out + (size_t)blockIdx.y * P.part_stride + tile_s0;
   write_tile<NCT>(tot0, tot1, wf0, inv_x, inv_gc, otile[w], op, P.out_stride, col0, P.ncols, li, kg, tile_len, P.vec_ok);
+  };
+  if (P.qmark && P.mode_word && (*P.mode_word & kModeAnyQuiet) != 0u) body(std::true_type{});
+  else body(std::false_type{});
 }
 
 }
diff --git a/libear_amd/csrc/gain_kernels.h b/libear_amd/csrc/gain_kernels.h
--- a/libear_amd/csrc/gain_kernels.h
+++ b/libear_amd/csrc/gain_kernels.h
@@ -129,9 +129,18 @@
   return obj_level != 0u && call_level != 0u && (int)(obj_level >> 23) < (int)(call_level >> 23) - kQuietBinades;
 }
 constexpr int kProbeInstants = 64, kProbeObjects = 16;
+struct QuietOut {
+  unsigned *mark = nullptr;
+  unsigned *mode = nullptr;
+  unsigned *ticket = nullptr;
+  int wide = 0;
+};
+constexpr unsigned kModeAnyQuiet = 8u;
 static __global__ void __launch_bounds__(64 * kProbeObjects)
-k_level_probe(const float *in, size_t in_stride, int nsamples, int M, unsigned *level, unsigned *obj_level, int cap, int nruns) {
+k_level_probe(const float *in, size_t in_stride, int nsamples, int M, unsigned *level, unsigned *obj_level, int cap, int nruns,
+              QuietOut qo) {
   __shared__ unsigned wmax[kProbeObjects];
+  __shared__ unsigned last_here;
   const int lane = threadIdx.x & 63, wv = threadIdx.x >> 6, m = blockIdx.x * kProbeObjects + wv;
   const int nvec = nsamples >> 2, ninst = min(kProbeInstants, nvec);
   unsigned v = 0u;
@@ -155,8 +164,9 @@
   if (lane == 0) {
     wmax[wv] = hi_v;
     if (m < M) {
-      obj_level[m] = hi_v;
-      obj_level[cap + m] = lo_v == 0xffffffffu ? 0u : lo_v;
+      __hip_atomic_store(obj_level + m, hi_v, __ATOMIC_RELAXED, __HIP_MEMORY_SCOPE_AGENT);
+      __hip_atomic_store(obj_level + cap + m, lo_v == 0xffffffffu ? 0u : lo_v, __ATOMIC_RELAXED, __HIP_MEMORY_SCOPE_AGENT);
+      if (qo.mark) asm volatile("s_waitcnt vmcnt(0)" ::: "memory");
     }
   }
   __syncthreads();
@@ -166,6 +176,29 @@
     for (int i = 0; i < kProbeObjects; i++) he = max(he, wmax[i]);
     he &= 0x7f800000u;
     if (he != 0 && he > __atomic_load_n(level, __ATOMIC_RELAXED)) atomicMax(level, he);
+  }
+  if (!qo.mark) return;
+  if (threadIdx.x == 0) {
+    asm volatile("s_waitcnt vmcnt(0)" ::: "memory");
+    last_here = __hip_atomic_fetch_add(qo.ticket, 1u, __ATOMIC_RELAXED, __HIP_MEMORY_SCOPE_AGENT) == gridDim.x - 1u ? 1u : 0u;
+  }
+  __syncthreads();
+  if (!last_here) return;
+  const unsigned call = __hip_atomic_load(level, __ATOMIC_RELAXED, __HIP_MEMORY_SCOPE_AGENT);
+  bool some_quiet = false, some_low = false;
+  for (int k = threadIdx.x; k < M; k += 64 * kProbeObjects) {
+    const unsigned hi = __hip_atomic_load(obj_level + k, __ATOMIC_RELAXED, __HIP_MEMORY_SCOPE_AGENT);
+    const unsigned lo = __hip_atomic_load(obj_level + cap + k, __ATOMIC_RELAXED, __HIP_MEMORY_SCOPE_AGENT);
+    const bool quiet = level_is_quiet(hi, call);
+    qo.mark[k] = quiet ? (unsigned)kSegQuiet : 0u;
+    some_quiet = some_quiet || quiet;
+    some_low = some_low || (lo != 0u && call != 0u && (int)(lo >> 23) < (int)(call >> 23) - kPlainBinades);
+  }
+  const int any_quiet = __syncthreads_or(some_quiet ? 1 : 0), any_low = __syncthreads_or(some_low ? 1 : 0);
+  if (threadIdx.x == 0) {
+    const unsigned bits = (any_quiet ? kModeAnyQuiet : 0u) | (qo.wide && any_low ? 1u : 0u);
+    if (bits) atomicOr(qo.mode, bits);
+    __hip_atomic_store(qo.ticket, 0u, __ATOMIC_RELAXED, __HIP_MEMORY_SCOPE_AGENT);
   }
 }
 
@@ -249,6 +282,48 @@
     const int to = (threadIdx.x >> 4) + 16 * j, oo = threadIdx.x & 15;
     const int tile_o = blockIdx.x * 16 * kPrepRun + to, m_o = blockIdx.y * 16 + oo;
     if (tile_o < ntiles && m_o < M) desc[(size_t)tile_o * M + m_o] = sh[to][oo];
+  }
+}
+
+template <int kPrepRun>
+static __global__ void __launch_bounds__(256)
+k_desc_table(PointStore ps, int M, const int32_t *objects, int count, int ntiles, int tile_samples, int64_t tile_lo, SegDesc *tab,
+             unsigned *multi, bool fresh) {
+  __shared__ SegDesc sh[16 * kPrepRun][17];
+  const int ti = threadIdx.x & 15, oi = threadIdx.x >> 4;
+  const int tile0 = (blockIdx.x * 16 + ti) * kPrepRun, idx = blockIdx.y * 16 + oi;
+  if (tile0 < ntiles && idx < count) {
+    const int m = objects ? objects[idx] : idx;
+    const ObjHdr hd = ps.hdr[m];
+    const int base = hd.off, n = hd.cnt;
+    int k = 0;
+#pragma unroll
+    for (int j = 0; j < kPrepRun; j++) {
+      const int tile = tile0 + j;
+      if (tile >= ntiles) break;
+      const int64_t t0 = (tile_lo + tile) * tile_samples;
+      if (j == 0) {
+        k = upper_bound_rec_window(ps.rec + base, n, hd.first, hd.last, t0);
+      } else {
+        while (k < n && ps.rec[base + k].time <= t0) k++;
+      }
+      sh[ti * kPrepRun + j][oi] = describe_segment_rec(ps, base, n, k, t0, t0 + tile_samples);
+    }
+  }
+  __syncthreads();
+#pragma unroll
+  for (int j = 0; j < kPrepRun; j++) {
+    const int to = (threadIdx.x >> 4) + 16 * j, oo = threadIdx.x & 15;
+    const int tile_o = blockIdx.x * 16 * kPrepRun + to, idx_o = blockIdx.y * 16 + oo;
+    if (tile_o < ntiles && idx_o < count) {
+      const int m_o = objects ? objects[idx_o] : idx_o;
+      const size_t at = (size_t)tile_o * M + m_o;
+      const SegDesc d = sh[to][oo];
+      int delta = (d.info & kSegMulti) ? 1 : 0;
+      if (!fresh) delta -= (tab[at].info & kSegMulti) ? 1 : 0;
+      tab[at] = d;
+      if (delta != 0) atomicAdd(&multi[tile_o], (unsigned)delta);
+    }
   }
 }
 
@@ -425,6 +500,7 @@
   int tile_runs = 0;
   const unsigned *mode_word = nullptr;
   unsigned *record = nullptr;
+  const unsigned *qmark = nullptr;
 };
 constexpr unsigned kModeRecorded = 4u;
 __device__ __forceinline__ void record_mode(const GainMixParams &P, bool device_form) {
```

New measurement: 1.177 million, median of 4. 1.01x the previous value.
